# flash4242/Promptable-Counterfactual-GAN

Hardware: AMD Instinct MI355X
Metric: images/sec (G+D step) MNIST-28 cDCGAN bs512 @1/2/4/8 MI355X; % MFMA roofline (higher is better)
Workload: dtype f32

## Files before the change

include/pcgan_hip.h:

```cpp
#ifndef PCGAN_HIP_H
#define PCGAN_HIP_H

#include <stddef.h>
#include <stdint.h>

#ifdef __cplusplus
extern "C" {
#endif

typedef void* pcg_stream_t;

typedef enum pcg_status {
  PCG_OK = 0,
  PCG_ERR_INVALID = -1,
  PCG_ERR_WORKSPACE = -2,
  PCG_ERR_LAUNCH = -3,
  PCG_ERR_UNSUPPORTED = -4
} pcg_status;

typedef enum pcg_act {
  PCG_ACT_NONE = 0,
  PCG_ACT_RELU = 1,
  PCG_ACT_LRELU = 2,
  PCG_ACT_TANH = 3,
// ... 408 lines not shown
  int32_t B;
  const float* const* w_stored;
  const float* a1; const float* a2; const float* a3; const float* a4;
  float* dx;
} pcg_house_cls_bwd_args;
int pcg_house_classifier_fwd(const pcg_house_cls_fwd_args* args, const pcg_sn_bwd_batch* rider , pcg_stream_t stream);
int pcg_house_classifier_bwd(const pcg_house_cls_bwd_args* args, const pcg_sn_fwd_batch* rider , pcg_stream_t stream);

typedef struct pcg_house_cf_eval_args {
  int64_t N; int32_t T, group, clamp_cls, mask_rows;
  const float* g_flat; int32_t nG;
  const float* bn_mean[10]; const float* bn_var[10];
  float bn_eps, tau, res_scale;
  int32_t col_src[17];
  const float* norm_vals;
  const float* const* c_w_kmajor; const float* const* c_bias;
  const float* x; const int64_t* y;
  const int64_t* target; const float* mask; const float* noise;
  float* cont; float* logits; int32_t* chosen;
  float* masked; float* x_cf; float* x_cf_raw;
  float* logits_cf; float* logits_x;
  int64_t* pred_cf; int64_t* pred_x;
  float* gain;
  float* tile_sums; float* class_sums; float* class_counts;
} pcg_house_cf_eval_args;
int pcg_house_cf_eval(const pcg_house_g_desc* desc, const pcg_house_cf_eval_args* args, pcg_stream_t stream);

enum { PCG_MASK_SHARED = 0,
       PCG_MASK_PER_ROW = 1,
       PCG_MASK_PER_QUERY = 2 };

typedef struct pcg_patch_mask_bits_args {
  const uint64_t* bits;
  float* mask;
  int32_t n, H, W, ps;
} pcg_patch_mask_bits_args;
int pcg_patch_mask_bits(const pcg_patch_mask_bits_args* args, pcg_stream_t stream);

typedef struct pcg_mnist_cf_entry_args {
  const float* x;
  const float* table;
  const float* mask;
  const int64_t* target;
  float* out;
  int32_t B, T, HW, K, mask_mode, q0, nq;
} pcg_mnist_cf_entry_args;
int pcg_mnist_cf_entry(const pcg_mnist_cf_entry_args* args, pcg_stream_t stream);

typedef struct pcg_mnist_cf_tail_args {
  const float* c;
  const float* x;
  const float* mask;
  float* x_cf;
  float* raw; float* masked;
  float* sums;
  float scale;
  int32_t B, T, HW, mask_mode, q0, nq;
} pcg_mnist_cf_tail_args;
int pcg_mnist_cf_tail(const pcg_mnist_cf_tail_args* args, pcg_stream_t stream);

#define PCG_MNIST_CF_GROUP_SUMS 8
typedef struct pcg_mnist_cf_score_args {
  const float* logits_cf;
  const float* logits_orig;
  const int64_t* target;
  const int64_t* y_true;
  const float* tail_sums;
  int64_t* pred; float* conf; float* p_target; float* p_true; float* p_orig_true; float* flip;
  float* group_sums;
  int32_t B, T, K, ld, group_rows, q0, nq;
} pcg_mnist_cf_score_args;
int pcg_mnist_cf_score(const pcg_mnist_cf_score_args* args, pcg_stream_t stream);

int pcg_house_losses(const float* d_real, const float* d_fake, const float* d_fake_g, int64_t n, const float* g_cls, const float* am,
                     const float* pen, float lambda_cls, float w_reg, float lambda_mask, float w_reg_log, float* out5, pcg_stream_t stream);

typedef struct pcg_house_res_fwd_args {
  const float* cont; int32_t ncont;
  const float* samples; const int32_t* seg_dev; int32_t T;
  const float* norm; const float* x; const float* mask;
  const int32_t* col_src;
  int32_t D, B;
  float* res; float* masked; float* x_cf; float* partial512; int32_t* ticket; float* pen_out; float* am_out;
} pcg_house_res_fwd_args;
typedef struct pcg_house_res_bwd_args {
  const float* res; const float* masked; const float* mask; const float* gx_a; const float* gx_b;
  float w_pen, w_am;
  int32_t ncont; const int32_t* cont_idx_dev; const int32_t* seg_dev; int32_t S, T;
  const int32_t* cat_idx_dev; const float* norm;
  int32_t D, B;
  float* dcont; float* dsamples;
} pcg_house_res_bwd_args;
typedef struct pcg_house_loss_args {
  const float* d_real; const float* d_fake; const float* d_fake_g; int32_t n;
  const float* g_cls;
  const float* am; const float* pen;
  float lambda_cls, w_reg, lambda_mask, w_reg_log;
  const float* ce_row_loss;
  int32_t n_ce;
  float* out6;
} pcg_house_loss_args;
typedef struct pcg_house_diag_args {
  const float* logits_cf; const float* logits_orig;
  const int64_t* src_rows;
  const int64_t* target_y; const float* masked;
  int32_t B, nc, D;
  float eps;
  float* out4;
  double* acc;
} pcg_house_diag_args;
int pcg_house_residual_fwd(const pcg_house_res_fwd_args* args, const pcg_sn_fwd_batch* rider , pcg_stream_t stream);
int pcg_house_residual_bwd(const pcg_house_res_bwd_args* args, const pcg_house_loss_args* losses ,
                           const pcg_house_diag_args* diag , pcg_stream_t stream);
int pcg_house_diag(const pcg_house_diag_args* args, pcg_stream_t stream);
int pcg_house_draws(int64_t* target_y, int32_t B, int32_t num_classes, const int64_t* y, uint64_t offset_target, float* mask, int32_t D,
                    const int32_t* zero_cols, int32_t n_zero_cols, uint64_t offset_mask, float* noise, int32_t T, uint64_t offset_noise,
                    uint64_t seed, float* onehot_target, float* onehot_y, pcg_stream_t stream);
int pcg_house_draws_counter(int64_t* target_y, int32_t B, int32_t num_classes, const int64_t* y, float* mask, int32_t D,
                            const int32_t* zero_cols, int32_t n_zero_cols, float* noise, int32_t T, uint64_t seed, float* onehot_target,
                            float* onehot_y, uint64_t* counter, pcg_stream_t stream);
int pcg_house_batch_draws_counter(int64_t* target_y, int32_t B, int32_t num_classes, const float* X, const int64_t* Y,
                                  const int64_t* perm, int64_t n_perm, int64_t n_rows, float* x_out, int64_t* y_out,
                                  int64_t* src_out , float* mask, int32_t D, const int32_t* zero_cols, int32_t n_zero_cols,
                                  float* noise, int32_t T, uint64_t seed, float* onehot_target , float* onehot_y ,
                                  uint64_t* counter, pcg_stream_t stream);

int pcg_dp_barrier(pcg_stream_t stream);
int32_t pcg_dp_rccl_version(void);

#define PCG_DP_UNIQUE_ID_BYTES 128
int pcg_dp_unique_id(void* id_out );
int pcg_dp_init(const void* id , int32_t rank, int32_t world);
int32_t pcg_dp_world(void);
int32_t pcg_dp_rank(void);
pcg_stream_t pcg_dp_side_stream(void);
int pcg_dp_allreduce(float* buf, int64_t n, pcg_stream_t stream);
int pcg_dp_allreduce_begin(float* buf, int64_t n, int32_t slot, pcg_stream_t producer_stream);
int pcg_dp_record(int32_t slot);
int pcg_dp_allreduce_wait(int32_t slot, pcg_stream_t consumer_stream);
int pcg_dp_allreduce_sum_f64(double* buf, int64_t n, pcg_stream_t stream);
int pcg_dp_broadcast(void* buf, int64_t nbytes, int32_t root, pcg_stream_t stream);
int pcg_dp_sync_batchnorm(int32_t enable);
int pcg_dp_shutdown(void);

int pcg_tune_set(const char* name, int32_t value);

int pcg_conv_plan_describe(const pcg_conv_geom* g, int32_t op, int32_t assume_scratch, char* out, size_t out_bytes);
size_t pcg_conv_scratch_parts_bytes(void);
size_t pcg_conv_scratch_arrivals_bytes(void);
int pcg_conv_set_scratch(pcg_stream_t stream, void* parts, size_t parts_bytes, void* arrivals, size_t arrivals_bytes);
int pcg_conv_reset_scratch(pcg_stream_t stream);
size_t pcg_conv_pixtab_bytes(const pcg_conv_geom* g);
int pcg_conv_pixtab_register(const pcg_conv_geom* g, void* host_out, size_t bytes, const void* device_table);
int pcg_debug_stamp_buffer(void* buf, int64_t bytes);

typedef struct pcg_moons_cf_desc {
  int32_t hidden, clf_hidden, B, N;
  int32_t nG, nD, nC, nG_adam, nD_adam;
  int32_t g_off[14], d_off[8], c_off[6];
  double lr_G, lr_D, beta1, beta2, adam_eps;
  float bn_eps, bn_momentum, sn_eps, slope;
  float lambda_cls, lambda_l1, lambda_l2, lambda_mask;
} pcg_moons_cf_desc;

typedef struct pcg_moons_cf_train_args {
  const float* X; const int64_t* Y;
  const int64_t* rows;
  const int64_t* target_y;
  const float* mask;
  float* g_flat; float* d_flat; const float* c_flat;
  float* g_exp_avg; float* g_exp_avg_sq; int64_t* g_step;
  float* d_exp_avg; float* d_exp_avg_sq; int64_t* d_step;
  float* bn_mean[3]; float* bn_var[3]; int64_t* bn_nbt[3];
  float* sn_u[4]; float* sn_v[4];
  float* logs;
  float* scratch; size_t scratch_bytes;
} pcg_moons_cf_train_args;

size_t pcg_moons_cf_scratch_bytes(const pcg_moons_cf_desc* desc, int32_t forward);
int pcg_moons_cf_train_steps(const pcg_moons_cf_desc* desc, const pcg_moons_cf_train_args* args, int32_t n_steps, pcg_stream_t stream);

typedef struct pcg_moons_cf_fwd_args {
  int32_t which, train, B;
  const float* x; const float* onehot; const float* mask;
  float* params;
  float* bn_mean[3]; float* bn_var[3]; int64_t* bn_nbt[3];
  float* sn_u[4]; float* sn_v[4];
  float* out0; float* out1;
  float* scratch; size_t scratch_bytes;
} pcg_moons_cf_fwd_args;
int pcg_moons_cf_forward(const pcg_moons_cf_desc* desc, const pcg_moons_cf_fwd_args* args, pcg_stream_t stream);

typedef struct pcg_moons_cf_eval_args {
  int64_t N; int32_t M, T, group;
  const float* x; const int64_t* y;
  const float* masks;
  const int64_t* target; const float* row_mask;
  const float* g_flat; const float* c_flat;
  const float* bn_mean[3]; const float* bn_var[3];
  float* raw; float* masked; float* x_cf;
  float* logits_cf; float* logits_x;
  int64_t* pred_cf; int64_t* pred_x;
  float* gain;
  float* sums;
} pcg_moons_cf_eval_args;
int pcg_moons_cf_eval(const pcg_moons_cf_desc* desc, const pcg_moons_cf_eval_args* args, pcg_stream_t stream);

typedef struct {
  const float* gamma;
  const float* beta;
  float* running_mean;
  float* running_var;
  int64_t* num_batches_tracked;
  float* save_mean;
  float* save_invstd;
  float* xhat;
  float eps;
  float momentum;
  int32_t training;
} pcg_dense_bn;
typedef struct {
  const float* xhat;
  const float* gamma;
  const float* invstd;
  float* dgamma;
  float* dbeta;
  int32_t accumulate;
} pcg_dense_bn_bwd;
int pcg_dense_rows_fwd(const float* x, const float* W, const float* bias , int32_t R, int32_t I, int32_t O,
                       const pcg_dense_bn* bn , int act, float slope, float* y, pcg_stream_t stream);
int pcg_dense_rows_dgrad(const float* dz, const float* W, int32_t R, int32_t O, int32_t I, int below_act, float below_slope,
                         const float* y_below , const pcg_dense_bn_bwd* bn , float* dx,
                         pcg_stream_t stream);
int pcg_dense_rows_wgrad(const float* dz, const float* x, int32_t R, int32_t O, int32_t I, float* dW, float* db ,
                         int accumulate, pcg_stream_t stream);

typedef struct pcg_moons_gan_desc {
  int32_t hidden, z_dim, label_dim, B, N;
  int32_t nG, nD, nG_adam, nD_adam;
  int32_t g_off[4], d_off[4];
  double lr_G, lr_D, beta1, beta2, adam_eps;
} pcg_moons_gan_desc;

typedef struct pcg_moons_gan_train_args {
  const float* X; const int64_t* Y;
  const int64_t* rows;
  const float* z;
  const int64_t* labels;
  float* g_flat; float* d_flat;
  float* g_exp_avg; float* g_exp_avg_sq; int64_t* g_step;
  float* d_exp_avg; float* d_exp_avg_sq; int64_t* d_step;
  float* logs;
  float* scratch; size_t scratch_bytes;
} pcg_moons_gan_train_args;

size_t pcg_moons_gan_scratch_bytes(const pcg_moons_gan_desc* desc);
int pcg_moons_gan_train_steps(const pcg_moons_gan_desc* desc, const pcg_moons_gan_train_args* args, int32_t n_steps, pcg_stream_t stream);

typedef struct pcg_moons_gan_fwd_args {
  int32_t which; int64_t R;
  const float* x; const float* onehot; const float* params;
  float* out;
} pcg_moons_gan_fwd_args;
int pcg_moons_gan_forward(const pcg_moons_gan_desc* desc, const pcg_moons_gan_fwd_args* args, pcg_stream_t stream);

int32_t pcg_calib_mfma_blocks(int32_t rounds);
size_t pcg_calib_mfma_workspace_bytes(int32_t rounds);
int pcg_calib_mfma(int32_t iters, int32_t rounds, void* workspace, size_t workspace_bytes, double* flop_out ,
                   uint64_t** stamps_out , pcg_stream_t stream);
int pcg_calib_copy(const void* src, void* dst, int64_t nbytes, pcg_stream_t stream);

#ifdef __cplusplus
}
#endif
#endif
```

promptable-counterfactual-gan_amd/_lib.py:

```python
import ctypes
import os

import torch

_HERE = os.path.dirname(os.path.abspath(__file__))
LIB_PATH = os.environ.get("PCG_LIB") or os.path.join(_HERE, "libpcgan_hip.so")

PCG_OK = 0
ACT_NONE, ACT_RELU, ACT_LRELU, ACT_TANH, ACT_SIGMOID = 0, 1, 2, 3, 4


class PcgError(RuntimeError):
    pass


class ConvGeom(ctypes.Structure):

    _fields_ = [(n, ctypes.c_int32) for n in ("B", "IH", "IW", "Cin", "OH", "OW", "Cout", "KH", "KW", "stride", "pad")]

    def key(self):
        return tuple(getattr(self, n) for n, _ in self._fields_)


_I, _P = ctypes.c_int32, ctypes.c_void_p
# ... 45 lines not shown


class MoonsCfFwdArgs(ctypes.Structure):
    _fields_ = ([(n, _I) for n in ("which", "train", "B")] + [(n, _P) for n in ("x", "onehot", "mask", "params")] +
                [("bn_mean", _P * 3), ("bn_var", _P * 3), ("bn_nbt", _P * 3), ("sn_u", _P * 4), ("sn_v", _P * 4)] +
                [("out0", _P), ("out1", _P), ("scratch", _P), ("scratch_bytes", ctypes.c_size_t)])


class MoonsCfEvalArgs(ctypes.Structure):
    _fields_ = ([("N", ctypes.c_int64), ("M", _I), ("T", _I), ("group", _I)] +
                [(n, _P) for n in ("x", "y", "masks", "target", "row_mask", "g_flat", "c_flat")] + [("bn_mean", _P * 3), ("bn_var", _P * 3)] +
                [(n, _P) for n in ("raw", "masked", "x_cf", "logits_cf", "logits_x", "pred_cf", "pred_x", "gain", "sums")])


class HouseCfEvalArgs(ctypes.Structure):
    _fields_ = ([("N", ctypes.c_int64)] + [(n, _I) for n in ("T", "group", "clamp_cls", "mask_rows")] + [("g_flat", _P), ("nG", _I)] +
                [("bn_mean", _P * 10), ("bn_var", _P * 10)] + [(n, ctypes.c_float) for n in ("bn_eps", "tau", "res_scale")] +
                [("col_src", _I * 17), ("norm_vals", _P), ("c_w_kmajor", ctypes.POINTER(ctypes.c_void_p)), ("c_bias", ctypes.POINTER(ctypes.c_void_p))] +
                [(n, _P) for n in ("x", "y", "target", "mask", "noise", "cont", "logits", "chosen", "masked", "x_cf", "x_cf_raw", "logits_cf",
                                   "logits_x", "pred_cf", "pred_x", "gain", "tile_sums", "class_sums", "class_counts")])


class PatchMaskBitsArgs(ctypes.Structure):
    _fields_ = [("bits", _P), ("mask", _P)] + [(n, _I) for n in ("n", "H", "W", "ps")]


class MnistCfEntryArgs(ctypes.Structure):
    _fields_ = [(n, _P) for n in ("x", "table", "mask", "target", "out")] + [(n, _I) for n in ("B", "T", "HW", "K", "mask_mode", "q0", "nq")]


class MnistCfTailArgs(ctypes.Structure):
    _fields_ = ([(n, _P) for n in ("c", "x", "mask", "x_cf", "raw", "masked", "sums")] + [("scale", ctypes.c_float)] +
                [(n, _I) for n in ("B", "T", "HW", "mask_mode", "q0", "nq")])


class MnistCfScoreArgs(ctypes.Structure):
    _fields_ = ([(n, _P) for n in ("logits_cf", "logits_orig", "target", "y_true", "tail_sums", "pred", "conf", "p_target", "p_true",
                                   "p_orig_true", "flip", "group_sums")] + [(n, _I) for n in ("B", "T", "K", "ld", "group_rows", "q0", "nq")])


MASK_SHARED, MASK_PER_ROW, MASK_PER_QUERY = 0, 1, 2
MNIST_CF_GROUP_SUMS = 8


class MoonsGanDesc(ctypes.Structure):
    _fields_ = ([(n, _I) for n in ("hidden", "z_dim", "label_dim", "B", "N", "nG", "nD", "nG_adam", "nD_adam")] +
                [("g_off", _I * 4), ("d_off", _I * 4)] + [(n, ctypes.c_double) for n in ("lr_G", "lr_D", "beta1", "beta2", "adam_eps")])


class MoonsGanTrainArgs(ctypes.Structure):
    _fields_ = ([(n, _P) for n in ("X", "Y", "rows", "z", "labels", "g_flat", "d_flat", "g_exp_avg", "g_exp_avg_sq", "g_step",
                                   "d_exp_avg", "d_exp_avg_sq", "d_step", "logs", "scratch")] + [("scratch_bytes", ctypes.c_size_t)])


class MoonsGanFwdArgs(ctypes.Structure):
    _fields_ = [("which", _I), ("R", ctypes.c_int64)] + [(n, _P) for n in ("x", "onehot", "params", "out")]


class DenseBn(ctypes.Structure):
    _fields_ = ([(n, _P) for n in ("gamma", "beta", "running_mean", "running_var", "num_batches_tracked", "save_mean", "save_invstd", "xhat")] +
                [("eps", ctypes.c_float), ("momentum", ctypes.c_float), ("training", _I)])


class DenseBnBwd(ctypes.Structure):
    _fields_ = [(n, _P) for n in ("xhat", "gamma", "invstd", "dgamma", "dbeta")] + [("accumulate", _I)]


_PP, _PI, _F = ctypes.POINTER(ctypes.c_void_p), ctypes.POINTER(ctypes.c_int32), ctypes.c_float


class SnFwdBatch(ctypes.Structure):
    _fields_ = ([("n", _I), ("reps", _I), ("power_iteration", _I), ("eps", _F), ("w_orig", _PP), ("out_features", _PI), ("in_features", _PI)] +
                [(n, _PP) for n in ("u", "v", "w_bar", "sigma", "u_used", "v_used")])


class SnBwdBatch(ctypes.Structure):
    _fields_ = [("n", _I), ("passes", _I), ("dw_bar", _PP), ("w_bar", _PP), ("out_features", _PI), ("in_features", _PI), ("u", _PP), ("v", _PP),
                ("sigma", _PP), ("dw_orig", _PP), ("accumulate", _PI), ("db_dst", _PP), ("db_src", _PP)]


class HouseCriticFwdArgs(ctypes.Structure):
    _fields_ = ([(n, _I) for n in ("n_pass", "B", "D", "NC")] + [("slope", _F)] +
                [(n, _PP) for n in ("x", "onehot", "w_bar", "bias", "a0", "a1", "a2", "a3", "out")])


class HouseCriticBwdArgs(ctypes.Structure):
    _fields_ = ([(n, _I) for n in ("n_pass", "B", "D")] + [("slope", _F)] +
                [(n, _PP) for n in ("dout", "w_bar", "a1", "a2", "a3", "d3", "d2", "d1", "dx")])


class HouseClsFwdArgs(ctypes.Structure):
    _fields_ = ([("x", _P), ("B", _I), ("w_kmajor", _PP), ("bias", _PP)] + [(n, _P) for n in ("a1", "a2", "a3", "a4", "logits", "ce_target")] +
                [("ce_grad_scale", _F), ("ce_dlogits", _P), ("ce_row_loss", _P)])


class HouseClsBwdArgs(ctypes.Structure):
    _fields_ = [("dlogits", _P), ("B", _I), ("w_stored", _PP)] + [(n, _P) for n in ("a1", "a2", "a3", "a4", "dx")]


class HouseResFwdArgs(ctypes.Structure):
    _fields_ = ([("cont", _P), ("ncont", _I), ("samples", _P), ("seg_dev", _P), ("T", _I), ("norm", _P), ("x", _P), ("mask", _P), ("col_src", _PI),
                 ("D", _I), ("B", _I)] + [(n, _P) for n in ("res", "masked", "x_cf", "partial512", "ticket", "pen_out", "am_out")])


class HouseResBwdArgs(ctypes.Structure):
    _fields_ = ([(n, _P) for n in ("res", "masked", "mask", "gx_a", "gx_b")] + [("w_pen", _F), ("w_am", _F), ("ncont", _I), ("cont_idx_dev", _P),
                ("seg_dev", _P), ("S", _I), ("T", _I), ("cat_idx_dev", _P), ("norm", _P), ("D", _I), ("B", _I), ("dcont", _P), ("dsamples", _P)])


class HouseLossArgs(ctypes.Structure):
    _fields_ = ([("d_real", _P), ("d_fake", _P), ("d_fake_g", _P), ("n", _I), ("g_cls", _P), ("am", _P), ("pen", _P)] +
                [(n, _F) for n in ("lambda_cls", "w_reg", "lambda_mask", "w_reg_log")] + [("ce_row_loss", _P), ("n_ce", _I), ("out6", _P)])


class HouseDiagArgs(ctypes.Structure):
    _fields_ = ([(n, _P) for n in ("logits_cf", "logits_orig", "src_rows", "target_y", "masked")] + [("B", _I), ("nc", _I), ("D", _I), ("eps", _F),
                ("out4", _P), ("acc", _P)])


STRUCTS = {"pcg_conv_geom": ConvGeom, "pcg_in_xform": InXform, "pcg_wgrad_item": WgradItem, "pcg_sn_fwd_batch": SnFwdBatch,
           "pcg_sn_bwd_batch": SnBwdBatch, "pcg_house_g_desc": HouseGDesc, "pcg_house_g_fwd_args": HouseGFwdArgs,
           "pcg_house_g_bwd_args": HouseGBwdArgs, "pcg_house_critic_fwd_args": HouseCriticFwdArgs,
           "pcg_house_critic_bwd_args": HouseCriticBwdArgs, "pcg_house_cls_fwd_args": HouseClsFwdArgs, "pcg_house_cls_bwd_args": HouseClsBwdArgs,
           "pcg_house_res_fwd_args": HouseResFwdArgs, "pcg_house_res_bwd_args": HouseResBwdArgs, "pcg_house_loss_args": HouseLossArgs,
           "pcg_house_diag_args": HouseDiagArgs, "pcg_moons_cf_desc": MoonsCfDesc, "pcg_moons_cf_train_args": MoonsCfTrainArgs,
           "pcg_moons_cf_fwd_args": MoonsCfFwdArgs, "pcg_moons_cf_eval_args": MoonsCfEvalArgs,
           "pcg_house_cf_eval_args": HouseCfEvalArgs, "pcg_patch_mask_bits_args": PatchMaskBitsArgs,
           "pcg_mnist_cf_entry_args": MnistCfEntryArgs, "pcg_mnist_cf_tail_args": MnistCfTailArgs,
           "pcg_mnist_cf_score_args": MnistCfScoreArgs, "pcg_dense_bn": DenseBn,
           "pcg_dense_bn_bwd": DenseBnBwd, "pcg_moons_gan_desc": MoonsGanDesc, "pcg_moons_gan_train_args": MoonsGanTrainArgs,
           "pcg_moons_gan_fwd_args": MoonsGanFwdArgs}

_c = ctypes
_vp, _f, _i, _i64, _sz = _c.c_void_p, _c.c_float, _c.c_int, _c.c_int64, _c.c_size_t
_d = _c.c_double
_i32 = _c.c_int32
_gp = _c.POINTER(ConvGeom)
_xp = _c.POINTER(InXform)

PROTOTYPES = {
    "pcg_abi_version": (_i, []),
    "pcg_abi_struct_bytes": (_sz, [_c.c_char_p]),
    "pcg_last_error": (_c.c_char_p, []),
    "pcg_target_arch": (_c.c_char_p, []),
    "pcg_tune_set": (_i, [_c.c_char_p, _i32]),
    "pcg_debug_stamp_buffer": (_i, [_vp, _i64]),
    "pcg_conv_plan_describe": (_i, [_c.POINTER(ConvGeom), _i32, _i32, _c.c_char_p, _sz]),
    "pcg_conv_scratch_parts_bytes": (_sz, []),
    "pcg_conv_scratch_arrivals_bytes": (_sz, []),
    "pcg_conv_set_scratch": (_i, [_vp, _vp, _sz, _vp, _sz]),
    "pcg_conv_reset_scratch": (_i, [_vp]),
    "pcg_conv_pixtab_bytes": (_sz, [_gp]),
    "pcg_conv_pixtab_register": (_i, [_gp, _vp, _sz, _vp]),
    "pcg_conv2d_fwd_bn_g": (_i, [_gp, _vp, _vp, _vp, _vp, _f, _f, _vp, _vp, _vp, _vp, _vp, _i32, _vp, _sz, _vp]),
    "pcg_bn_apply_act_g": (_i, [_vp, _i64, _i32, _vp, _vp, _vp, _vp, _i, _f, _vp, _i32, _vp]),
    "pcg_conv2d_dgrad_bn_phases": (_i32, [_gp]),
    "pcg_conv2d_dgrad_bnbwd_g": (_i, [_gp, _vp, _vp, _vp, _vp, _vp, _vp, _vp, _i, _f, _vp, _vp, _sz, _i32, _vp]),
    "pcg_bn_bwd_partial_g_workspace_bytes": (_sz, [_i32, _i32]),
    "pcg_bn_bwd_partial_g": (_i, [_vp, _vp, _i64, _i32, _vp, _vp, _vp, _vp, _i32, _i32, _vp, _vp, _vp, _i, _i32, _vp, _sz, _vp]),
    "pcg_bn_act_bwd_g_workspace_bytes": (_sz, [_i64, _i32, _i32]),
    "pcg_bn_act_bwd_premask_g": (_i, [_vp, _vp, _i64, _i32, _vp, _vp, _vp, _vp, _i, _f, _vp, _vp, _vp, _i, _i32, _vp, _sz, _vp]),
    "pcg_bce_pair": (_i, [_vp, _i64, _f, _f, _vp, _vp, _vp, _vp, _vp, _vp]),
    "pcg_conv2d_fwd_bnbwd_thin_ok": (_i32, [_gp]),
    "pcg_conv2d_fwd_bnbwd_thin_workspace_bytes": (_sz, [_gp]),
    "pcg_conv2d_fwd_bnbwd_thin": (_i, [_gp, _vp, _vp, _vp, _vp, _vp, _vp, _vp, _i, _f, _vp, _vp, _vp, _i, _vp, _sz, _vp]),
    "pcg_conv2d_bnin_full_ok": (_i32, [_gp, _i32]),
    "pcg_conv2d_fwd_bnin_full": (_i, [_gp, _vp, _vp, _vp, _vp, _vp, _i, _f, _i32, _vp, _vp, _i, _f, _vp, _vp]),
    "pcg_conv2d_wgrad_bnin_full": (_i, [_gp, _vp, _vp, _vp, _vp, _vp, _i, _f, _i32, _vp, _vp, _i, _vp, _sz, _vp]),
    "pcg_conv_precision_set": (_i, [_i32]),
    "pcg_conv_precision_get": (_i32, []),
    "pcg_slab_defer_begin": (_i, [_vp]),
    "pcg_slab_defer_flush": (_i, [_vp]),
    "pcg_slab_defer_pending": (_i32, []),
    "pcg_conv2d_dgrad_bnbwd_full_ok": (_i32, [_gp, _i32]),
    "pcg_conv2d_dgrad_bnbwd_full_workspace_bytes": (_sz, [_gp, _i32]),
    "pcg_conv2d_dgrad_bnbwd_full": (_i, [_gp, _vp, _vp, _vp, _vp, _vp, _vp, _vp, _i, _f, _vp, _vp, _vp, _i, _i32, _vp, _sz, _vp]),
    "pcg_calib_mfma_blocks": (_i32, [_i32]),
    "pcg_calib_mfma_workspace_bytes": (_sz, [_i32]),
    "pcg_calib_mfma": (_i, [_i32, _i32, _vp, _sz, _c.POINTER(_d), _c.POINTER(_c.c_uint64), _vp]),
    "pcg_calib_copy": (_i, [_vp, _vp, _i64, _vp]),
    "pcg_conv2d_fwd_workspace_bytes": (_sz, [_gp]),
    "pcg_conv2d_dgrad_workspace_bytes": (_sz, [_gp]),
    "pcg_conv2d_fwd": (_i, [_gp, _vp, _vp, _vp, _vp, _vp, _sz, _vp]),
    "pcg_conv2d_dgrad": (_i, [_gp, _vp, _vp, _vp, _vp, _vp, _sz, _vp]),
    "pcg_conv2d_fwd_act": (_i, [_gp, _vp, _vp, _vp, _i, _f, _vp, _vp, _sz, _vp]),
    "pcg_conv2d_dgrad_act": (_i, [_gp, _vp, _vp, _vp, _i, _f, _vp, _vp, _sz, _vp]),
    "pcg_conv2d_fwd_bn_workspace_bytes": (_sz, [_gp]),
    "pcg_conv2d_dgrad_bn_workspace_bytes": (_sz, [_gp]),
    "pcg_conv2d_fwd_bn": (_i, [_gp, _vp, _vp, _vp, _vp, _f, _f, _vp, _vp, _vp, _vp, _vp, _vp, _sz, _vp]),
    "pcg_conv2d_dgrad_bn": (_i, [_gp, _vp, _vp, _vp, _vp, _f, _f, _vp, _vp, _vp, _vp, _vp, _vp, _sz, _vp]),
    "pcg_conv2d_dgrad_mask": (_i, [_gp, _vp, _vp, _vp, _i, _f, _vp, _vp, _sz, _vp]),
    "pcg_conv2d_dgrad_mask_thin_ok": (_i32, [_gp]),
    "pcg_conv2d_xf_thin_ok": (_i32, [_gp]),
    "pcg_conv2d_fwd_add_mask": (_i, [_gp, _vp, _vp, _vp, _vp, _i, _f, _vp, _vp]),
    "pcg_conv2d_dgrad_add_mask": (_i, [_gp, _vp, _vp, _vp, _vp, _i, _f, _vp, _vp]),
    "pcg_conv2d_fwd_mask": (_i, [_gp, _vp, _vp, _vp, _i, _f, _vp, _vp, _sz, _vp]),
    "pcg_conv2d_dgrad_bnbwd": (_i, [_gp, _vp, _vp, _vp, _vp, _vp, _vp, _vp, _i, _f, _vp, _vp, _sz, _vp]),
    "pcg_conv2d_fwd_bnbwd": (_i, [_gp, _vp, _vp, _vp, _vp, _vp, _vp, _vp, _i, _f, _vp, _vp, _sz, _vp]),
    "pcg_conv2d_dgrad_add": (_i, [_gp, _vp, _vp, _vp, _vp, _vp, _sz, _vp]),
    "pcg_conv2d_fwd_bn_partial_rows": (_c.c_int32, [_gp]),
    "pcg_conv2d_dgrad_bn_partial_rows": (_c.c_int32, [_gp]),
    "pcg_bn_bwd_partial_workspace_bytes": (_sz, [_c.c_int32]),
    "pcg_bn_bwd_partial": (_i, [_vp, _vp, _i64, _c.c_int32, _vp, _vp, _vp, _vp, _c.c_int32, _vp, _vp, _vp, _i, _vp, _sz, _vp]),
    "pcg_conv2d_fwd_bn_xf": (_i, [_gp, _vp, _xp, _vp, _vp, _vp, _f, _f, _vp, _vp, _vp, _vp, _vp, _vp, _vp, _vp, _vp, _sz, _vp]),
    "pcg_conv2d_dgrad_bn_xf": (_i, [_gp, _vp, _xp, _vp, _vp, _vp, _f, _f, _vp, _vp, _vp, _vp, _vp, _vp, _vp, _vp, _vp, _sz, _vp]),
    "pcg_conv2d_fwd_xf": (_i, [_gp, _vp, _xp, _vp, _vp, _i, _f, _vp, _vp, _sz, _vp]),
    "pcg_conv2d_dgrad_xf": (_i, [_gp, _vp, _xp, _vp, _vp, _i, _f, _vp, _vp, _sz, _vp]),
    "pcg_conv2d_wgrad_xf": (_i, [_gp, _vp, _xp, _vp, _xp, _vp, _i, _vp, _sz, _vp]),
    "pcg_bn_train_stats_coef": (_i, [_vp, _i64, _c.c_int32, _f, _f, _vp, _vp, _vp, _vp, _vp, _vp, _vp, _vp, _vp, _sz, _vp]),
    "pcg_bn_db_workspace_bytes": (_sz, [_i64, _c.c_int32]),
    "pcg_bn_act_bwd_db": (_i, [_vp, _vp, _vp, _i64, _c.c_int32, _vp, _vp, _vp, _vp, _i, _f, _f, _vp, _vp, _vp, _i, _vp, _i, _vp, _sz, _vp]),
    "pcg_bn_bwd_partial_db_workspace_bytes": (_sz, [_c.c_int32]),
    "pcg_bn_bwd_partial_db": (_i, [_vp, _vp, _i64, _c.c_int32, _vp, _vp, _vp, _vp, _c.c_int32, _f, _vp, _vp, _vp, _i, _vp, _i, _vp, _sz, _vp]),
    "pcg_conv2d_dgrad_add_bnsum": (_i, [_gp, _vp, _vp, _vp, _vp, _vp, _vp, _f, _vp, _vp, _sz, _vp]),
    "pcg_conv2d_fwd_add": (_i, [_gp, _vp, _vp, _vp, _vp, _vp, _sz, _vp]),
    "pcg_conv2d_fwd_add_bnsum": (_i, [_gp, _vp, _vp, _vp, _vp, _vp, _vp, _f, _vp, _vp, _sz, _vp]),
    "pcg_conv_weight_adjoint": (_i, [_vp, _vp, _i32, _i32, _i32, _i32, _vp]),
    "pcg_conv_weight_adjoint_many": (_i, [_vp, _vp, _i32, _i32, _i32, _i32, _i32, _vp]),
    "pcg_house_losses": (_i, [_vp, _vp, _vp, _i64, _vp, _vp, _vp, _f, _f, _f, _f, _vp, _vp]),
    "pcg_dp_unique_id": (_i, [_vp]),
    "pcg_dp_init": (_i, [_vp, _i32, _i32]),
    "pcg_dp_world": (_i32, []),
    "pcg_dp_rank": (_i32, []),
    "pcg_dp_side_stream": (_vp, []),
    "pcg_dp_allreduce": (_i, [_vp, _i64, _vp]),
    "pcg_dp_allreduce_begin": (_i, [_vp, _i64, _i32, _vp]),
    "pcg_dp_record": (_i, [_i32]),
    "pcg_dp_allreduce_wait": (_i, [_i32, _vp]),
    "pcg_dp_allreduce_sum_f64": (_i, [_vp, _i64, _vp]),
    "pcg_dp_broadcast": (_i, [_vp, _i64, _i32, _vp]),
    "pcg_dp_sync_batchnorm": (_i, [_i32]),
    "pcg_dp_barrier": (_i, [_vp]),
    "pcg_dp_rccl_version": (_i32, []),
    "pcg_dp_shutdown": (_i, []),
    "pcg_conv2d_wgrad_workspace_bytes": (_sz, [_gp]),
    "pcg_conv2d_wgrad": (_i, [_gp, _vp, _vp, _vp, _i, _vp, _sz, _vp]),
    "pcg_colsum_workspace_bytes": (_sz, [_i64, _c.c_int32]),
    "pcg_colsum": (_i, [_vp, _i64, _c.c_int32, _vp, _i, _vp, _sz, _vp]),
    "pcg_bn_workspace_bytes": (_sz, [_i64, _c.c_int32]),
    "pcg_bn_train_stats": (_i, [_vp, _i64, _c.c_int32, _f, _f, _vp, _vp, _vp, _vp, _vp, _vp, _sz, _vp]),
    "pcg_bn_apply_act": (_i, [_vp, _i64, _c.c_int32, _vp, _vp, _f, _vp, _vp, _i, _f, _vp, _f, _vp, _vp]),
    "pcg_bn_act_bwd": (_i, [_vp, _vp, _vp, _i64, _c.c_int32, _vp, _vp, _vp, _i, _f, _f, _vp, _vp, _vp, _i, _vp, _sz, _vp]),
    "pcg_bn_act_bwd_premask": (_i, [_vp, _vp, _i64, _c.c_int32, _vp, _vp, _vp, _vp, _i, _f, _f, _vp, _vp, _vp, _i, _vp, _sz, _vp]),
    "pcg_embed_concat_fwd": (_i, [_vp, _vp, _vp, _vp, _vp, _c.c_int32, _c.c_int32, _c.c_int32, _c.c_int32, _vp]),
    "pcg_embed_concat_bwd": (_i, [_vp, _vp, _vp, _vp, _c.c_int32, _c.c_int32, _c.c_int32, _c.c_int32, _i, _vp]),
    "pcg_embed_table_grad": (_i, [_vp, _vp, _vp, _i32, _i32, _i32, _i32, _i32, _i, _vp]),
    "pcg_gather_channel": (_i, [_vp, _vp, _i32, _i32, _i32, _vp]),
    "pcg_axpby": (_i, [_vp, _f, _vp, _f, _vp, _i64, _vp]),
    "pcg_scale_mask_fwd": (_i, [_vp, _vp, _f, _vp, _vp, _i64, _vp]),
    "pcg_scale_mask_bwd": (_i, [_vp, _vp, _vp, _f, _vp, _i64, _vp]),
    "pcg_clamp_add_fwd": (_i, [_vp, _vp, _f, _f, _vp, _i64, _vp]),
    "pcg_clamp_add_bwd": (_i, [_vp, _vp, _vp, _f, _f, _vp, _i64, _vp]),
    "pcg_abs_mean_workspace_bytes": (_sz, []),
    "pcg_abs_mean_fwd": (_i, [_vp, _vp, _i, _i64, _vp, _vp, _sz, _vp]),
    "pcg_abs_mean_bwd": (_i, [_vp, _vp, _i, _i64, _vp, _f, _vp, _i, _vp]),
    "pcg_avgpool_fwd": (_i, [_vp, _vp, _c.c_int32, _c.c_int32, _c.c_int32, _vp]),
    "pcg_avgpool_bwd": (_i, [_vp, _vp, _c.c_int32, _c.c_int32, _c.c_int32, _vp]),
    "pcg_cross_entropy_fwd_bwd": (_i, [_vp, _vp, _c.c_int32, _c.c_int32, _f, _vp, _vp, _vp, _vp]),
    "pcg_act_fwd": (_i, [_vp, _i64, _i, _f, _vp, _vp]),
    "pcg_act_bwd": (_i, [_vp, _vp, _i64, _i, _f, _vp, _vp]),
    "pcg_bce_fwd_bwd": (_i, [_vp, _vp, _f, _i64, _f, _vp, _vp, _vp, _vp]),
    "pcg_bce_logits_fwd_bwd": (_i, [_vp, _f, _i64, _f, _vp, _vp, _vp, _vp]),
    "pcg_adam_step": (_i, [_vp, _vp, _vp, _vp, _i64, _d, _d, _d, _d, _d, _i, _i64, _vp]),
    "pcg_adam_step_capturable": (_i, [_vp, _vp, _vp, _vp, _i64, _d, _d, _d, _d, _d, _i, _vp, _vp, _vp]),
    "pcg_patch_mask": (_i, [_vp, _c.c_int32, _c.c_int32, _c.c_int32, _c.c_int32, _c.c_int32, _c.c_uint64, _c.c_uint64, _vp]),
    "pcg_randint": (_i, [_vp, _i64, _c.c_int32, _c.c_int32, _vp, _c.c_uint64, _c.c_uint64, _vp]),
    "pcg_randn": (_i, [_vp, _i64, _f, _f, _c.c_uint64, _c.c_uint64, _vp]),
    "pcg_fill": (_i, [_vp, _i64, _f, _vp]),
    "pcg_add_bias_rows": (_i, [_vp, _i64, _i32, _vp, _vp]),
    "pcg_sumsq": (_i, [_vp, _i64, _vp, _i, _vp]),
    "pcg_norm_sum": (_i, [_vp, _vp, _i32, _vp, _vp]),
    "pcg_instnorm_fwd": (_i, [_vp, _i32, _i32, _i32, _vp, _vp, _f, _i, _f, _vp, _vp, _vp, _vp]),
    "pcg_instnorm_bwd": (_i, [_vp, _vp, _i32, _i32, _i32, _vp, _vp, _vp, _vp, _vp, _vp, _vp]),
    "pcg_instnorm_bwd_bwd": (_i, [_vp, _vp, _vp, _i32, _i32, _i32, _vp, _vp, _vp, _vp, _vp, _vp, _vp]),
    "pcg_instnorm_bwd_fused": (_i, [_vp, _vp, _f, _vp, _i32, _i32, _i32, _vp, _vp, _vp, _vp, _vp, _vp, _vp, _vp, _vp, _vp]),
    "pcg_instnorm_bwd_bwd_act": (_i, [_vp, _vp, _vp, _i32, _i32, _i32, _vp, _vp, _vp, _vp, _f, _vp, _vp, _vp, _vp]),
    "pcg_rowsum3": (_i, [_i32, _vp, _vp, _i, _vp, _vp, _i, _vp, _vp, _i, _i32, _i32, _vp]),
    "pcg_nhwc_to_nchw_flat": (_i, [_vp, _vp, _i32, _i32, _i32, _i, _vp]),
    "pcg_interpolate": (_i, [_vp, _vp, _vp, _vp, _i32, _i32, _vp]),
    "pcg_interpolate_stack": (_i, [_vp, _vp, _vp, _vp, _i32, _i32, _vp]),
    "pcg_gradient_penalty_fwd": (_i, [_vp, _i32, _i32, _f, _vp, _vp, _vp]),
    "pcg_gradient_penalty_bwd": (_i, [_vp, _vp, _vp, _i32, _i32, _f, _vp, _vp]),
    "pcg_rand_uniform": (_i, [_vp, _i64, _c.c_uint64, _c.c_uint64, _vp]),
    "pcg_cross_entropy_weighted_fwd_bwd": (_i, [_vp, _vp, _vp, _i32, _i32, _f, _vp, _vp, _vp, _vp]),
    "pcg_dropout_apply": (_i, [_vp, _vp, _i64, _i32, _i32, _f, _vp, _vp]),
    "pcg_rand_bernoulli": (_i, [_vp, _i64, _f, _c.c_uint64, _c.c_uint64, _vp]),
    "pcg_resize8_normalize": (_i, [_vp, _i32, _i32, _i32, _i32, _i32, _vp, _vp, _i32, _vp, _vp, _i32, _f, _f, _vp, _vp]),
    "pcg_house_g_fwd": (_i, [_c.POINTER(HouseGDesc), _c.POINTER(HouseGFwdArgs), _vp]),
    "pcg_house_g_bwd": (_i, [_c.POINTER(HouseGDesc), _c.POINTER(HouseGBwdArgs), _vp]),
    "pcg_weighted_sum_fwd": (_i, [_i32, _vp, _vp, _vp, _vp]),
    "pcg_weighted_sum_bwd": (_i, [_i32, _vp, _vp, _vp, _vp]),
    "pcg_cf_metrics": (_i, [_vp, _vp, _vp, _vp, _i32, _i32, _vp, _vp]),
    "pcg_gemm": (_i, [_i, _i, _i32, _i32, _i32, _vp, _i32, _vp, _i32, _vp, _i32, _vp, _i, _vp]),
    "pcg_linear_wgrad_workspace_bytes": (_sz, [_i32, _i32, _i32]),
    "pcg_linear_wgrad_ticket_count": (_i32, []),
    "pcg_linear_wgrad": (_i, [_vp, _i32, _vp, _i32, _i32, _i32, _i32, _vp, _vp, _i, _i, _vp, _sz, _vp, _vp]),
    "pcg_spectral_norm_fwd_batched": (_i, [_c.POINTER(SnFwdBatch), _vp]),
    "pcg_spectral_norm_bwd_batched": (_i, [_c.POINTER(SnBwdBatch), _vp]),
    "pcg_house_critic_fwd": (_i, [_c.POINTER(HouseCriticFwdArgs), _vp]),
    "pcg_house_critic_bwd": (_i, [_c.POINTER(HouseCriticBwdArgs), _vp]),
    "pcg_house_classifier_fwd": (_i, [_c.POINTER(HouseClsFwdArgs), _c.POINTER(SnBwdBatch), _vp]),
    "pcg_house_classifier_bwd": (_i, [_c.POINTER(HouseClsBwdArgs), _c.POINTER(SnFwdBatch), _vp]),
    "pcg_house_cf_eval": (_i, [_c.POINTER(HouseGDesc), _c.POINTER(HouseCfEvalArgs), _vp]),
    "pcg_patch_mask_bits": (_i, [_c.POINTER(PatchMaskBitsArgs), _vp]),
    "pcg_mnist_cf_entry": (_i, [_c.POINTER(MnistCfEntryArgs), _vp]),
    "pcg_mnist_cf_tail": (_i, [_c.POINTER(MnistCfTailArgs), _vp]),
# ... 75 lines not shown
```

promptable-counterfactual-gan_amd/csrc/conv_igemm.hip:

```cpp
#include <string.h>
#include <mutex>
#include "conv_loaders.h"
#include "conv_pixtab.h"
#include "thin_conv.h"

namespace pcg {
namespace {

__device__ __forceinline__ int wave_id() { return __builtin_amdgcn_readfirstlane((int)(threadIdx.x >> 6)); }

__device__ __forceinline__ void prio_entry(const ConvP& p) { if (p.edge_prio & 1) __builtin_amdgcn_s_setprio(3); }
__device__ __forceinline__ void prio_epilogue(const ConvP& p) { if (p.edge_prio & 2) __builtin_amdgcn_s_setprio(3); }

__device__ __forceinline__ int epi_group_off(const ConvP& p, int m_block) {
  return p.epi.group_rows > 0 ? __builtin_amdgcn_readfirstlane(m_block / p.epi.group_rows) * p.N : 0;
}

template <class Cfg, bool XF>
__global__ void __launch_bounds__(IG_THREADS, Cfg::MINW) conv_fwd_kernel(ConvP p) {
  extern __shared__ __attribute__((aligned(16))) float smem[];
  prio_entry(p);
  const uint32_t tile = xcd_remap(blockIdx.x, gridDim.x);
  const int mt = tile / p.tilesN, nt = tile % p.tilesN;
  const int m_block = mt * Cfg::BM, n_block = nt * Cfg::BN;
  const int kt_begin = blockIdx.y * p.ktiles_per_split;
  int ktiles = p.ktiles - kt_begin;
  if (ktiles > p.ktiles_per_split) ktiles = p.ktiles_per_split;

  if (wave_id() >= 4) {
    const int tid = threadIdx.x - IG_LOADERS;
    FwdALoader<Cfg::BM, XF> la(p, m_block, tid);
    FwdBLoader<Cfg::BN> lb(p, n_block, tid);
    if (kt_begin) { la.seek(kt_begin); lb.seek(kt_begin); }
    igemm_produce<Cfg>(la, lb, ktiles, smem, tid, ClockStamp{p.stamps, p.stamp_slots});
    return;
  }
  f32x16 acc[Cfg::TM][Cfg::TN];
  ClockStamp cs{p.stamps, p.stamp_slots};
  cs.phase(0);
  igemm_consume<Cfg, true, true>(ktiles, acc, smem, cs);
  prio_epilogue(p);
  float* out = p.out + (size_t)blockIdx.y * (size_t)p.M * (size_t)p.N;
#ifdef PCG_ABL_NO_EPILOGUE
  if (acc[0][0][0] == 12345.678f) out[0] = acc[0][0][1];
  return;
#endif
  igemm_store_tile<Cfg>(acc, smem, n_block, p.N, blockIdx.y == 0 ? p.bias : nullptr, [&](int row) -> float* {
    const int m = m_block + row;
    return m < p.M ? out + (size_t)m * p.N + n_block : nullptr;
  }, p.stat_partial ? p.stat_partial + (size_t)mt * Cfg::WAVES_M * 2 * p.N : nullptr, p.act, p.slope, &p.epi, epi_group_off(p, m_block));
  cs.phase(3);
}

template <class Cfg, bool XF>
__global__ void __launch_bounds__(IG_THREADS, Cfg::MINW) conv_dgrad_kernel(ConvP p, DgradPhases phases) {
  extern __shared__ __attribute__((aligned(16))) float smem[];
  __shared__ int rowpix[Cfg::BM];
  prio_entry(p);
  uint32_t bx = blockIdx.x, py = blockIdx.y;
  if (phases.interleave) {
    const uint32_t l = xcd_remap(blockIdx.x, gridDim.x);
    py = l % (uint32_t)phases.interleave; bx = l / (uint32_t)phases.interleave;
  }
  const PhaseInfo& f = phases.p[py];
  const int tilesM = (f.Mp + Cfg::BM - 1) / Cfg::BM;
  const uint32_t ntiles = (uint32_t)tilesM * p.tilesN;
  if (bx >= ntiles) return;
  const uint32_t tile = phases.interleave ? bx : xcd_remap(bx, ntiles);
  const int mt = tile / p.tilesN, nt = tile % p.tilesN;
  const int m_block = mt * Cfg::BM, n_block = nt * Cfg::BN;
  const int ktiles = f.nth * f.ntw * ((p.Cout + IG_BK - 1) / IG_BK);

  if (wave_id() >= 4) {
    const int tid = threadIdx.x - IG_LOADERS;
    for (int r = tid; r < Cfg::BM; r += IG_LOADERS) {
      const int m = m_block + r;
      int pix = -1;
      if (m < f.Mp) {
        uint32_t t, cc, b, aa;
        f.dPHw.divmod((uint32_t)m, t, cc);
        f.dPHh.divmod(t, b, aa);
        pix = ((int)b * p.IH + (int)aa * p.stride + f.ph) * p.IW + (int)cc * p.stride + f.pw;
      }
      rowpix[r] = pix;
    }
    DgradALoader<Cfg::BM, XF> la(p, f, m_block, tid);
    DgradBLoader<Cfg::BN> lb(p, f, n_block, tid);
    igemm_produce<Cfg>(la, lb, ktiles, smem, tid, ClockStamp{p.stamps, p.stamp_slots});
    return;
  }
  f32x16 acc[Cfg::TM][Cfg::TN];
  ClockStamp cs{p.stamps, p.stamp_slots};
  cs.phase(0);
  igemm_consume<Cfg, true, false>(ktiles, acc, smem, cs);
  prio_epilogue(p);
  igemm_store_tile<Cfg>(acc, smem, n_block, p.N, p.bias, [&](int row) -> float* {
    const int pix = rowpix[row];
    return pix >= 0 ? p.out + (size_t)pix * p.Cin + n_block : nullptr;
  }, p.stat_partial ? p.stat_partial + (size_t)(f.prow0 + mt * Cfg::WAVES_M) * 2 * p.N : nullptr, p.act, p.slope, &p.epi, epi_group_off(p, m_block));
  cs.phase(3);
}

struct SkPlan {
  int dp_tiles, sk_tiles, sk_blocks, ktiles;
  float* parts;
  int* arrivals;
};
struct SkSeg { int tile, kt_begin, nkt, nparts, first_block; };

__device__ __forceinline__ int sk_start(int g, const SkPlan& sk) {
  return __builtin_amdgcn_readfirstlane((int)((uint32_t)g * (uint32_t)(sk.sk_tiles * sk.ktiles) / (uint32_t)sk.sk_blocks));
}
__device__ __forceinline__ int sk_owner(int x, const SkPlan& sk) {
  return __builtin_amdgcn_readfirstlane((int)((((uint32_t)x + 1u) * (uint32_t)sk.sk_blocks - 1u) / (uint32_t)(sk.sk_tiles * sk.ktiles)));
}
__device__ __forceinline__ int sk_segments(const SkPlan& sk, SkSeg& s0, SkSeg& s1) {
  const int b = blockIdx.x;
  if (b < sk.dp_tiles) { s0 = SkSeg{(int)xcd_remap((uint32_t)b, (uint32_t)sk.dp_tiles), 0, sk.ktiles, 1, 0}; return 1; }
  const int g = (int)xcd_remap((uint32_t)(b - sk.dp_tiles), (uint32_t)sk.sk_blocks), KT = sk.ktiles;
  const int it0 = sk_start(g, sk), it1 = sk_start(g + 1, sk);
  const int j0 = __builtin_amdgcn_readfirstlane(it0 / KT), e0 = it1 < (j0 + 1) * KT ? it1 : (j0 + 1) * KT;
  auto fill = [&](SkSeg& sg, int j, int from, int to) {
    const int f = sk_owner(j * KT, sk), l = sk_owner((j + 1) * KT - 1, sk);
    sg = SkSeg{sk.dp_tiles + j, from - j * KT, to - from, l - f + 1, f};
  };
  fill(s0, j0, it0, e0);
  if (it1 <= e0) return 1;
  fill(s1, j0 + 1, e0, it1);
  return 2;
}
#if defined(__HIP_DEVICE_COMPILE__) && !defined(__gfx950__)
#error "stream-K partial-tile exchange (sc1 stores + relaxed agent-scope counters) is written for gfx950 only"
#endif
__device__ __forceinline__ void sk_store4(rsrc_t r, uint32_t off, float a, float b, float c, float d) {
  const u32x4 v = {__float_as_uint(a), __float_as_uint(b), __float_as_uint(c), __float_as_uint(d)};
  __builtin_amdgcn_raw_buffer_store_b128(v, r, off, 0, 16);
}
__device__ __forceinline__ float4 sk_load4(rsrc_t r, uint32_t off) {
  const u32x4 v = __builtin_amdgcn_raw_buffer_load_b128(r, off, 0, 16);
  return make_float4(__uint_as_float(v.x), __uint_as_float(v.y), __uint_as_float(v.z), __uint_as_float(v.w));
}
template <class Cfg, class FirstOf>
__device__ __forceinline__ bool sk_combine_core(float* parts, int* arrivals, int nblocks, int g, int j, int nparts, int first_block,
                                                FirstOf first_of, f32x16 (&acc)[Cfg::TM][Cfg::TN]) {
  if (nparts == 1) return true;
  constexpr uint32_t TILE_BYTES = Cfg::BM * Cfg::BN * 4;
  auto slot_of = [&](int blk) { return (uint32_t)(2 * blk + (first_of(blk) ? 0 : 1)); };
  const rsrc_t rs = make_rsrc(parts, (uint32_t)(2 * nblocks) * TILE_BYTES);
  const uint32_t toff = threadIdx.x * 16u;
  const uint32_t mine = slot_of(g) * TILE_BYTES + toff;
#pragma unroll
  for (int i = 0; i < Cfg::TM; ++i)
#pragma unroll
    for (int jj = 0; jj < Cfg::TN; ++jj)
#pragma unroll
      for (int q = 0; q < 4; ++q)
        sk_store4(rs, mine + (uint32_t)(((i * Cfg::TN + jj) * 4 + q) * IG_LOADERS * 16),
                  acc[i][jj][4 * q], acc[i][jj][4 * q + 1], acc[i][jj][4 * q + 2], acc[i][jj][4 * q + 3]);
  asm volatile("s_waitcnt vmcnt(0)" ::: "memory");
  int* cnt = arrivals + j * 4 + (int)(threadIdx.x >> 6);
  int old = 0;
  if ((threadIdx.x & 63) == 0) old = __hip_atomic_fetch_add(cnt, 1, __ATOMIC_RELAXED, __HIP_MEMORY_SCOPE_AGENT);
  old = __builtin_amdgcn_readfirstlane(old);
  if (old != nparts - 1) return false;
  if ((threadIdx.x & 63) == 0) __hip_atomic_store(cnt, 0, __ATOMIC_RELAXED, __HIP_MEMORY_SCOPE_AGENT);
#pragma unroll
  for (int i = 0; i < Cfg::TM; ++i)
#pragma unroll
    for (int jj = 0; jj < Cfg::TN; ++jj)
#pragma unroll
      for (int r = 0; r < 16; ++r) acc[i][jj][r] = 0.f;
  for (int k = 0; k < nparts; ++k) {
    const uint32_t src = slot_of(first_block + k) * TILE_BYTES + toff;
#pragma unroll
    for (int i = 0; i < Cfg::TM; ++i)
#pragma unroll
      for (int jj = 0; jj < Cfg::TN; ++jj)
#pragma unroll
        for (int q = 0; q < 4; ++q) {
          const float4 v = sk_load4(rs, src + (uint32_t)(((i * Cfg::TN + jj) * 4 + q) * IG_LOADERS * 16));
          acc[i][jj][4 * q] += v.x; acc[i][jj][4 * q + 1] += v.y; acc[i][jj][4 * q + 2] += v.z; acc[i][jj][4 * q + 3] += v.w;
        }
  }
  return true;
}
template <class Cfg>
__device__ __forceinline__ bool sk_combine(const SkPlan& sk, const SkSeg& sg, f32x16 (&acc)[Cfg::TM][Cfg::TN]) {
  const int g = (int)xcd_remap((uint32_t)((int)blockIdx.x - sk.dp_tiles), (uint32_t)sk.sk_blocks), j = sg.tile - sk.dp_tiles, KT = sk.ktiles;
  return sk_combine_core<Cfg>(sk.parts, sk.arrivals, sk.sk_blocks, g, j, sg.nparts, sg.first_block,
                              [&](int blk) { return sk_start(blk, sk) >= j * KT; }, acc);
}

template <class Cfg, bool XF>
__device__ __forceinline__ void fwd_sk_segment(const ConvP& p, const SkPlan& sk, const SkSeg& sg, float* smem) {
  const int mt = __builtin_amdgcn_readfirstlane(sg.tile / p.tilesN), nt = sg.tile - mt * p.tilesN;
  const int m_block = mt * Cfg::BM, n_block = nt * Cfg::BN;
  if (wave_id() >= 4) {
    const int tid = threadIdx.x - IG_LOADERS;
    FwdALoader<Cfg::BM, XF> la(p, m_block, tid);
    FwdBLoader<Cfg::BN> lb(p, n_block, tid);
    if (sg.kt_begin) { la.seek(sg.kt_begin); lb.seek(sg.kt_begin); }
    igemm_produce<Cfg>(la, lb, sg.nkt, smem, tid, ClockStamp{nullptr, 0});
    return;
  }
  f32x16 acc[Cfg::TM][Cfg::TN];
  igemm_consume<Cfg, true, true>(sg.nkt, acc, smem);
  if (sk_combine<Cfg>(sk, sg, acc))
    igemm_store_tile<Cfg>(acc, smem, n_block, p.N, p.bias, [&](int row) -> float* {
      const int m = m_block + row;
      return m < p.M ? p.out + (size_t)m * p.N + n_block : nullptr;
    }, p.stat_partial ? p.stat_partial + (size_t)mt * Cfg::WAVES_M * 2 * p.N : nullptr, p.act, p.slope, &p.epi, epi_group_off(p, m_block));
// ... 121 lines not shown
}
template <class Cfg, bool XF>
__global__ void __launch_bounds__(IG_THREADS, Cfg::MINW) conv_dgrad_skn_kernel(ConvP p, DgradPhases phases, SkNPlan sk) {
  extern __shared__ __attribute__((aligned(16))) float smem[];
  __shared__ int rowpix[Cfg::BM];
  const int g = (int)xcd_remap(blockIdx.x, (uint32_t)sk.blocks);
  const int it1 = skn_start(g + 1, sk);
  if (wave_id() >= 4) {
    const int tid = threadIdx.x - IG_LOADERS;
#pragma unroll 1
    for (int it = skn_start(g, sk); it < it1;) {
      const SkNSeg sg = skn_segment(it, it1, sk, p.tilesN);
      const PhaseInfo& f = phases.p[sg.py];
      const int m_block = sg.mt * Cfg::BM, n_block = sg.nt * Cfg::BN;
      for (int r = tid; r < Cfg::BM; r += IG_LOADERS) {
        const int m = m_block + r;
        int pix = -1;
        if (m < f.Mp) {
          uint32_t t, cc, b, aa;
          f.dPHw.divmod((uint32_t)m, t, cc);
          f.dPHh.divmod(t, b, aa);
          pix = ((int)b * p.IH + (int)aa * p.stride + f.ph) * p.IW + (int)cc * p.stride + f.pw;
        }
        rowpix[r] = pix;
      }
      DgradALoader<Cfg::BM, XF> la(p, f, m_block, tid);
      DgradBLoader<Cfg::BN> lb(p, f, n_block, tid);
      if (sg.kt_begin) { la.seek(sg.kt_begin); lb.seek(sg.kt_begin); }
      igemm_produce<Cfg>(la, lb, sg.nkt, smem, tid, ClockStamp{nullptr, 0});
      it = sg.e;
      if (it < it1) lds_barrier();
    }
    return;
  }
#pragma unroll 1
  for (int it = skn_start(g, sk); it < it1;) {
    const SkNSeg sg = skn_segment(it, it1, sk, p.tilesN);
    const PhaseInfo& f = phases.p[sg.py];
    const int m_block = sg.mt * Cfg::BM, n_block = sg.nt * Cfg::BN;
    {
      f32x16 acc[Cfg::TM][Cfg::TN];
      igemm_consume<Cfg, true, false>(sg.nkt, acc, smem);
      const int t_begin = sg.t_begin;
      if (sk_combine_core<Cfg>(sk.parts, sk.arrivals, sk.blocks, g, sk.tile0[sg.py] + sg.tin, sg.nparts, sg.fb,
                               [&](int blk) { return skn_start(blk, sk) >= t_begin; }, acc))
        igemm_store_tile<Cfg>(acc, smem, n_block, p.N, p.bias, [&](int row) -> float* {
          const int pix = rowpix[row];
          return pix >= 0 ? p.out + (size_t)pix * p.Cin + n_block : nullptr;
        }, p.stat_partial ? p.stat_partial + (size_t)(f.prow0 + sg.mt * Cfg::WAVES_M) * 2 * p.N : nullptr, p.act, p.slope, &p.epi, epi_group_off(p, m_block));
    }
    it = sg.e;
    if (it < it1) lds_barrier();
  }
}

template <class Cfg, bool XFA, bool XFB, bool TAB>
__device__ __forceinline__ void wgrad_sk_segment(const ConvP& p, const SkPlan& sk, const SkSeg& sg, float* smem) {
  const int mt = __builtin_amdgcn_readfirstlane(sg.tile / p.tilesN), nt = sg.tile - mt * p.tilesN;
  const int m_block = mt * Cfg::BM, n_block = nt * Cfg::BN;
  if (wave_id() >= 4) {
    const int tid = threadIdx.x - IG_LOADERS;
    WgradALoader<Cfg::BM, XFA> la(p, m_block, sg.kt_begin, tid);
    WgradBLoader<Cfg::BN, XFB, TAB> lb(p, n_block, sg.kt_begin, tid);
    igemm_produce<Cfg>(la, lb, sg.nkt, smem, tid, ClockStamp{nullptr, 0});
    return;
  }
  f32x16 acc[Cfg::TM][Cfg::TN];
  igemm_consume<Cfg, false, false>(sg.nkt, acc, smem);
  if (sk_combine<Cfg>(sk, sg, acc))
    igemm_store_tile<Cfg>(acc, smem, n_block, p.N, nullptr, [&](int row) -> float* {
      const int m = m_block + row;
      return m < p.M ? p.out + (size_t)m * p.N + n_block : nullptr;
    }, nullptr, PCG_ACT_NONE, 0.f, &p.epi);
}
template <class Cfg, bool XFA, bool XFB, bool TAB = false>
__global__ void __launch_bounds__(IG_THREADS, 4) conv_wgrad_sk_kernel(ConvP p, SkPlan sk) {
  extern __shared__ __attribute__((aligned(16))) float smem[];
  SkSeg s0, s1{};
  const int nseg = sk_segments(sk, s0, s1);
  wgrad_sk_segment<Cfg, XFA, XFB, TAB>(p, sk, s0, smem);
  if (nseg == 1) return;
  lds_barrier();
  wgrad_sk_segment<Cfg, XFA, XFB, TAB>(p, sk, s1, smem);
}

using Cfg64x192 = TileCfg<64, 192, 2, 2>;
template <class Cfg, bool TAB = false>
__global__ void __launch_bounds__(IG_THREADS, 4) conv_wgrad192_kernel(ConvP p, int ktiles_total, int ktiles_per_split, int tiles,
                                                                      int slice_major) {
  static_assert(Cfg::BM == 64 && Cfg::BN == 192, "the 192-column weight-gradient tile");
  extern __shared__ __attribute__((aligned(16))) float smem[];
  prio_entry(p);
  uint32_t tile, split;
  if (slice_major) {
    const uint32_t l = xcd_remap(blockIdx.x, gridDim.x);
    split = l / (uint32_t)tiles; tile = l - split * (uint32_t)tiles;
  } else {
    tile = xcd_remap(blockIdx.x, gridDim.x); split = blockIdx.y;
  }
  const int mt = tile / p.tilesN, nt = tile % p.tilesN;
  const int m_block = mt * Cfg::BM, n_block = nt * Cfg::BN;
  const int kt_begin = split * ktiles_per_split;
  int ktiles = ktiles_total - kt_begin;
  if (ktiles > ktiles_per_split) ktiles = ktiles_per_split;
  if (wave_id() >= 4) {
    const int tid = threadIdx.x - IG_LOADERS;
    WgradALoader<Cfg::BM, false> la(p, m_block, kt_begin, tid);
    WgradBLoader192<TAB> lb(p, n_block, kt_begin, tid);
    igemm_produce<Cfg>(la, lb, ktiles, smem, tid);
    return;
  }
  f32x16 acc[Cfg::TM][Cfg::TN];
  igemm_consume<Cfg, false, false>(ktiles, acc, smem, ClockStamp{p.stamps, p.stamp_slots});
  prio_epilogue(p);
  float* slab = p.out + (size_t)split * (size_t)p.M * (size_t)p.N;
  igemm_store_tile<Cfg>(acc, smem, n_block, p.N, nullptr, [&](int row) -> float* {
    const int m = m_block + row;
    return m < p.M ? slab + (size_t)m * p.N + n_block : nullptr;
  });
}

__global__ void __launch_bounds__(256) col2im_kernel(const float4* __restrict__ dcol, float4* __restrict__ dx, const float* __restrict__ bias,
                                                     int B, int IH, int IW, int CQ, int OH, int OW, int KH, int KW, int stride, int pad,
                                                     FastDiv dCQ, FastDiv dIW, FastDiv dIH, int act, float neg) {
  const uint32_t total = (uint32_t)B * IH * IW * CQ;
  for (uint32_t idx = blockIdx.x * 256u + threadIdx.x; idx < total; idx += gridDim.x * 256u) {
    uint32_t pix, cq, t, iw, b, ih;
    dCQ.divmod(idx, pix, cq);
    dIW.divmod(pix, t, iw);
    dIH.divmod(t, b, ih);
    float4 acc = bias ? *reinterpret_cast<const float4*>(bias + 4 * cq) : make_float4(0.f, 0.f, 0.f, 0.f);
    for (int kh = 0; kh < KH; ++kh) {
      const int th = (int)ih + pad - kh;
      if (th < 0 || th % stride) continue;
      const int oh = th / stride;
      if (oh >= OH) continue;
      for (int kw = 0; kw < KW; ++kw) {
        const int tw = (int)iw + pad - kw;
        if (tw < 0 || tw % stride) continue;
        const int ow = tw / stride;
        if (ow >= OW) continue;
        const float4 v = dcol[((size_t)(((int)b * OH + oh) * OW + ow) * (KH * KW) + (kh * KW + kw)) * CQ + cq];
        acc.x += v.x; acc.y += v.y; acc.z += v.z; acc.w += v.w;
      }
    }
    if (act != PCG_ACT_NONE) {
      acc.x = act_neg_scale(acc.x, neg); acc.y = act_neg_scale(acc.y, neg); acc.z = act_neg_scale(acc.z, neg); acc.w = act_neg_scale(acc.w, neg);
    }
    dx[idx] = acc;
  }
}

using Cfg128x128 = TileCfg<128, 128, 2, 2>;
#ifndef PCG_TILE64_SWZ
#define PCG_TILE64_SWZ 1
#endif
using Cfg128x64P = TileCfg<128, 64, 2, 2>;
#if PCG_TILE64_SWZ
using Cfg128x64 = TileCfg<128, 64, 2, 2, true, 6, 1>;
#else
using Cfg128x64 = Cfg128x64P;
#endif

template <class C>
using Bf16Twin = TileCfg<C::BM, C::BN, C::WAVES_M, C::WAVES_N, false, C::MINW, C::PF, true>;


int check_geom(const pcg_conv_geom* g) {
  PCG_REQUIRE(g != nullptr, "conv geometry is null");
  PCG_REQUIRE(g->B > 0 && g->IH > 0 && g->IW > 0 && g->Cin > 0 && g->OH > 0 && g->OW > 0 && g->Cout > 0,
              "conv geometry: non-positive extent");
  PCG_REQUIRE(g->KH > 0 && g->KW > 0 && g->stride > 0 && g->pad >= 0, "conv geometry: bad kernel/stride/pad");
  PCG_REQUIRE(g->OH == (g->IH + 2 * g->pad - g->KH) / g->stride + 1 && g->OW == (g->IW + 2 * g->pad - g->KW) / g->stride + 1,
              "conv geometry: OH/OW inconsistent with IH/IW, kernel %dx%d stride %d pad %d", g->KH, g->KW, g->stride, g->pad);
  PCG_REQUIRE((int64_t)g->B * g->IH * g->IW * g->Cin * 4 < (1ll << 31) && (int64_t)g->B * g->OH * g->OW * g->Cout * 4 < (1ll << 31) &&
                  (int64_t)g->Cout * g->KH * g->KW * g->Cin * 4 < (1ll << 31),
              "conv geometry: an operand tensor reaches 2 GiB (32-bit buffer offsets); split the batch");
  PCG_REQUIRE(g->KH * g->KW <= 32, "conv geometry: more than 32 taps (%dx%d) unsupported", g->KH, g->KW);
  return PCG_OK;
}

struct Tune { int edge_prio = -1, dgrad_swz3 = -1, wgrad_rounds = -1, korder = -1, wgrad_order = -1, dgrad_interleave = -1, fwd_splits = -1, stream_k = -1, sk_blocks = -1, dgrad_gemm = -1, t64 = -1, wgrad_pixtab = -1; unsigned long long* stamps = nullptr; int stamp_slots = 0; };
Tune g_tune;

ConvP make_params(const pcg_conv_geom* g) {
  ConvP p{};
  static const int korder_env = getenv("PCG_KORDER") ? atoi(getenv("PCG_KORDER")) : 1;
  p.korder = g_tune.korder >= 0 ? g_tune.korder : korder_env;
  static const int edge_env = getenv("PCG_EDGE_PRIO") ? atoi(getenv("PCG_EDGE_PRIO")) : 2;
  p.edge_prio = g_tune.edge_prio >= 0 ? g_tune.edge_prio : edge_env;
  p.stamps = g_tune.stamps; p.stamp_slots = g_tune.stamp_slots;
  p.B = g->B; p.IH = g->IH; p.IW = g->IW; p.Cin = g->Cin; p.OH = g->OH; p.OW = g->OW; p.Cout = g->Cout;
  p.KH = g->KH; p.KW = g->KW; p.stride = g->stride; p.pad = g->pad;
  p.dOW = FastDiv((uint32_t)g->OW);
  p.dOH = FastDiv((uint32_t)g->OH);
  p.dOHW = FastDiv((uint32_t)(g->OH * g->OW));
  p.x_bytes = (uint32_t)((int64_t)g->B * g->IH * g->IW * g->Cin * 4);
  p.dy_bytes = (uint32_t)((int64_t)g->B * g->OH * g->OW * g->Cout * 4);
  p.w_bytes = (uint32_t)((int64_t)g->Cout * g->KH * g->KW * g->Cin * 4);
  return p;
}

int set_xform(const char* who, const pcg_in_xform* xf, int C, ConvP* p) {
  if (!xf || !xf->scale) return PCG_OK;
  PCG_REQUIRE(xf->shift != nullptr, "%s: input transform without shift", who);
  PCG_REQUIRE(xf->act == PCG_ACT_NONE || xf->act == PCG_ACT_RELU || xf->act == PCG_ACT_LRELU,
              "%s: input transform activation %d is not none / ReLU / LeakyReLU", who, xf->act);
  PCG_REQUIRE(C % 4 == 0 && (((uintptr_t)xf->scale | (uintptr_t)xf->shift) & 15) == 0,
              "%s: input transform needs a channel count %% 4 == 0 and 16-byte aligned scale / shift", who);
  p->in_sc = xf->scale; p->in_sh = xf->shift; p->in_neg = act_neg_of(xf->act, xf->slope); p->in_c_bytes = (uint32_t)C * 4u;
  return PCG_OK;
}

template <class Cfg, bool AK, bool BK_>
constexpr size_t smem_bytes() {
  constexpr int a = igemm_smem_floats<Cfg, AK, BK_>(), b = epilogue_smem_floats<Cfg>();
  return sizeof(float) * (size_t)(a > b ? a : b);
}

template <class K>
int set_smem(K kernel, size_t bytes) {
  hipError_t e = hipFuncSetAttribute(reinterpret_cast<const void*>(kernel), hipFuncAttributeMaxDynamicSharedMemorySize, (int)bytes);
  if (e != hipSuccess) { set_error("hipFuncSetAttribute(max dynamic LDS=%zu): %s", bytes, hipGetErrorString(e)); return PCG_ERR_LAUNCH; }
  return PCG_OK;
}

constexpr int SK_MAX_BLOCKS = 512, SK_MAX_TILES = 4096;
constexpr size_t SK_PARTS_BYTES = (size_t)2 * SK_MAX_BLOCKS * 128 * 128 * sizeof(float);
constexpr size_t SK_ARRIVALS_BYTES = (size_t)SK_MAX_TILES * 4 * sizeof(int);
struct SkScratch { int device; hipStream_t stream; float* parts; int* arrivals; };
SkScratch g_sk_scratch[64];
int g_sk_scratch_n = 0;
std::mutex g_sk_mutex;
int current_device() { int d = 0; return hipGetDevice(&d) == hipSuccess ? d : 0; }
bool sk_scratch_of(hipStream_t s, SkPlan* sk) {
  const int dev = current_device();
  std::lock_guard<std::mutex> lock(g_sk_mutex);
  for (int i = 0; i < g_sk_scratch_n; ++i)
    if (g_sk_scratch[i].stream == s && g_sk_scratch[i].device == dev) {
      if (sk) { sk->parts = g_sk_scratch[i].parts; sk->arrivals = g_sk_scratch[i].arrivals; }
      return true;
    }
  return false;
}
struct PixTabReg { int device, IH, IW, OH, OW, stride, pad, KH, KW, Cin; const uint32_t* tab; };
constexpr int PIXTAB_MAX = 256;
PixTabReg g_pixtab[PIXTAB_MAX];
int g_pixtab_n = 0;
std::mutex g_pixtab_mutex;
bool pixtab_same(const PixTabReg& r, int dev, const pcg_conv_geom* g) {
  return r.device == dev && r.IH == g->IH && r.IW == g->IW && r.OH == g->OH && r.OW == g->OW && r.stride == g->stride && r.pad == g->pad &&
         r.KH == g->KH && r.KW == g->KW && r.Cin == g->Cin;
}
const uint32_t* pixtab_of(const pcg_conv_geom* g) {
  static const int env = getenv("PCG_WGRAD_PIXTAB") ? atoi(getenv("PCG_WGRAD_PIXTAB")) : 1;
  if (!(g_tune.wgrad_pixtab >= 0 ? g_tune.wgrad_pixtab : env)) return nullptr;
  std::lock_guard<std::mutex> lock(g_pixtab_mutex);
  if (g_pixtab_n == 0) return nullptr;
  const int dev = current_device();
  for (int i = 0; i < g_pixtab_n; ++i)
    if (pixtab_same(g_pixtab[i], dev, g)) return g_pixtab[i].tab;
  return nullptr;
}
int sk_mode() {
  static const int env = getenv("PCG_STREAM_K") ? atoi(getenv("PCG_STREAM_K")) : 1;
  return g_tune.stream_k >= 0 ? g_tune.stream_k : env;
}
bool plan_sk_shape(int tiles, int ktiles, SkPlan* sk) {
  const int mode = sk_mode();
  if (mode == 3) {
    sk->dp_tiles = tiles; sk->sk_tiles = 0; sk->sk_blocks = 0; sk->ktiles = ktiles;
    return true;
  }
  if (mode == 0 || ktiles < 8) return false;
  const int dp = tiles / 512 * 512, r = tiles - dp;
  if (r == 0 || r > SK_MAX_TILES || (int64_t)r * ktiles * 512 >= (1ll << 31)) return false;
  const double t_dp = (r <= 256 ? 2.2 : 3.5) * ktiles + 6.0;
  double best = 1e30;
  int bg = 0;
  for (int G = 512; G >= 64; G >>= 1) {
    if (g_tune.sk_blocks > 0 && G != g_tune.sk_blocks) continue;
    if (G < r) break;
    const int it = ceil_div(r * ktiles, G);
    if (it < 4) continue;
    const int parts = ceil_div(ktiles, it) + 1;
    if (parts > 8) continue;
    const double t = it * (G == 512 ? 3.5 : 2.2) + 2 * 12.0 + 3.0 + 1.5 * parts;
    if (t < best) { best = t; bg = G; }
  }
  if (!bg || (mode == 1 && best > 0.9 * t_dp)) return false;
  sk->dp_tiles = dp; sk->sk_tiles = r; sk->sk_blocks = bg; sk->ktiles = ktiles;
  return true;
}
bool plan_sk(int tiles, int ktiles, hipStream_t s, SkPlan* sk) { return plan_sk_shape(tiles, ktiles, sk) && sk_scratch_of(s, sk); }
bool have_sk_scratch() {
  if (sk_mode() == 0) return false;
  const int dev = current_device();
  std::lock_guard<std::mutex> lock(g_sk_mutex);
  for (int i = 0; i < g_sk_scratch_n; ++i) if (g_sk_scratch[i].device == dev) return true;
  return false;
}
int stream_has_sk(hipStream_t s) { return sk_mode() != 0 && sk_scratch_of(s, nullptr) ? 1 : 0; }

template <class Cfg, bool XF>
int launch_fwd_x(ConvP p, int splits, hipStream_t s) {
  p.tilesN = ceil_div(p.N, Cfg::BN);
  const int tilesM = ceil_div(p.M, Cfg::BM);
  constexpr size_t smem = smem_bytes<Cfg, true, true>();
  if constexpr (Cfg::BM == 128 && Cfg::BN == 128) {
    SkPlan sk{};
    if (splits == 1 && plan_sk(tilesM * p.tilesN, p.ktiles, s, &sk)) {
      static int once_sk = set_smem(conv_fwd_sk_kernel<Cfg, XF>, smem);
      if (once_sk != PCG_OK) return once_sk;
      hipLaunchKernelGGL((conv_fwd_sk_kernel<Cfg, XF>), dim3((unsigned)(sk.dp_tiles + sk.sk_blocks)), dim3(IG_THREADS), smem, s, p, sk);
      return launch_status("conv_fwd_sk_kernel");
    }
  }
  static int once = set_smem(conv_fwd_kernel<Cfg, XF>, smem);
  if (once != PCG_OK) return once;
  hipLaunchKernelGGL((conv_fwd_kernel<Cfg, XF>), dim3((unsigned)tilesM * p.tilesN, splits), dim3(IG_THREADS), smem, s, p);
  return launch_status("conv_fwd_kernel");
}
template <class Cfg>
int launch_fwd(const ConvP& p, int splits, hipStream_t s) {
  if (conv_bf16()) return p.in_sc ? launch_fwd_x<Bf16Twin<Cfg>, true>(p, splits, s) : launch_fwd_x<Bf16Twin<Cfg>, false>(p, splits, s);
  return p.in_sc ? launch_fwd_x<Cfg, true>(p, splits, s) : launch_fwd_x<Cfg, false>(p, splits, s);
}

struct FwdPlan { int splits, ktiles_per_split; };
FwdPlan plan_fwd(const pcg_conv_geom* g, int have_sk = -1) {
  if (have_sk < 0) have_sk = have_sk_scratch() ? 1 : 0;
  const int M = g->B * g->OH * g->OW, N = g->Cout;
  const int tiles = ceil_div(M, 128) * ceil_div(N, N > 64 ? 128 : 64);
  const int ktiles = g->KH * g->KW * ceil_div(g->Cin, IG_BK);
  FwdPlan f{1, ktiles};
  if (g_tune.fwd_splits > 0) {
    f.ktiles_per_split = ceil_div(ktiles, g_tune.fwd_splits);
    f.splits = ceil_div(ktiles, f.ktiles_per_split);
    return f;
  }
  if (tiles > 256 && tiles < 448 && ktiles >= 32 && !have_sk) {
    int best = 1;
    double bc = 2.0;
    for (int s = 2; s <= 4; ++s) {
      const double c = (double)ceil_div(tiles * s, 256) / s + 0.1 * s;
      if (c < bc - 1e-9) { bc = c; best = s; }
    }
    f.ktiles_per_split = ceil_div(ktiles, best);
    f.splits = ceil_div(ktiles, f.ktiles_per_split);
    return f;
  }
  if (tiles > 96 || ktiles < 32) return f;
  int splits = ceil_div(tiles >= 48 ? 512 : 384, tiles);
  if (splits > ktiles / 8) splits = ktiles / 8;
  if (splits < 2) return f;
  f.ktiles_per_split = ceil_div(ktiles, splits);
  f.splits = ceil_div(ktiles, f.ktiles_per_split);
  return f;
}

bool plan_skn_shape(const DgradPhases& ph, int nphases, int BM, int tilesN, int Cout, SkNPlan* sn) {
  if (sk_mode() == 0 || nphases < 2) return false;
  sn->nph = nphases;
  bool ok = true;
  int tiles = 0, total = 0, ktmax = 0;
  for (int i = 0; i < nphases && ok; ++i) {
    const int kt = ph.p[i].nth * ph.p[i].ntw * ceil_div(Cout, IG_BK), t = ceil_div(ph.p[i].Mp, BM) * tilesN;
    ok = ph.p[i].nth > 0 && ph.p[i].ntw > 0 && ph.p[i].Mp > 0 && kt > 0;
    sn->tile0[i] = tiles; sn->it0[i] = total; sn->kt[i] = kt;
    tiles += t; total += t * kt;
    if (kt > ktmax) ktmax = kt;
  }
  sn->tile0[nphases] = tiles; sn->it0[nphases] = total;
  int blocks = total / 512 >= 16 ? 512 : 256;
  if (g_tune.sk_blocks > 0) blocks = g_tune.sk_blocks;
  ok = ok && tiles <= SK_MAX_TILES && blocks <= SK_MAX_BLOCKS && total / blocks >= 8 && (int64_t)total * blocks < (1ll << 31) &&
       ktmax <= 8 * (total / blocks) && (sk_mode() == 2 || g_tune.sk_blocks > 0 || total >= 48 * tiles);
  sn->blocks = blocks; sn->total = total;
  return ok;
}

template <class Cfg, bool XF>
int launch_dgrad_x(ConvP p, const DgradPhases& ph, int nphases, int maxMp, hipStream_t s) {
  p.tilesN = ceil_div(p.N, Cfg::BN);
  const int tilesM = ceil_div(maxMp, Cfg::BM);
  constexpr size_t smem = smem_bytes<Cfg, true, false>();
  if constexpr (Cfg::BM == 128 && Cfg::BN == 128) {
    bool uniform = true;
    for (int i = 0; i < nphases; ++i)
      uniform = uniform && ph.p[i].Mp == ph.p[0].Mp && ph.p[i].nth * ph.p[i].ntw == ph.p[0].nth * ph.p[0].ntw && ph.p[i].nth > 0 && ph.p[i].ntw > 0;
    if (!uniform && nphases > 1 && sk_mode() != 0) {
      SkNPlan sn{};
      SkPlan scratch{};
      if (plan_skn_shape(ph, nphases, Cfg::BM, p.tilesN, p.Cout, &sn) && sk_scratch_of(s, &scratch)) {
        sn.parts = scratch.parts; sn.arrivals = scratch.arrivals;
        static int once_sn = set_smem(conv_dgrad_skn_kernel<Cfg, XF>, smem);
        if (once_sn != PCG_OK) return once_sn;
        DgradPhases phs = ph;
        phs.interleave = 0;
        hipLaunchKernelGGL((conv_dgrad_skn_kernel<Cfg, XF>), dim3((unsigned)sn.blocks), dim3(IG_THREADS), smem, s, p, phs, sn);
        return launch_status("conv_dgrad_skn_kernel");
      }
    }
    SkPlan sk{};
    const int tpp = tilesM * p.tilesN;
    if (uniform && plan_sk(tpp * nphases, ph.p[0].nth * ph.p[0].ntw * ceil_div(p.Cout, IG_BK), s, &sk)) {
      static int once_sk = set_smem(conv_dgrad_sk_kernel<Cfg, XF>, smem);
      if (once_sk != PCG_OK) return once_sk;
      DgradPhases phs = ph;
      phs.interleave = 0;
      hipLaunchKernelGGL((conv_dgrad_sk_kernel<Cfg, XF>), dim3((unsigned)(sk.dp_tiles + sk.sk_blocks)), dim3(IG_THREADS), smem, s, p, phs, sk, tpp);
      return launch_status("conv_dgrad_sk_kernel");
    }
  }
  static int once = set_smem(conv_dgrad_kernel<Cfg, XF>, smem);
  if (once != PCG_OK) return once;
  static const int il_env0 = getenv("PCG_DGRAD_INTERLEAVE") ? atoi(getenv("PCG_DGRAD_INTERLEAVE")) : 1;
  const int il_env = g_tune.dgrad_interleave >= 0 ? g_tune.dgrad_interleave : il_env0;
  DgradPhases phl = ph;
  bool same = nphases > 1 && il_env && p.w_bytes <= (1u << 20);
  for (int i = 1; i < nphases; ++i) same = same && ph.p[i].Mp == ph.p[0].Mp;
  phl.interleave = same ? nphases : 0;
  if (same)
    hipLaunchKernelGGL((conv_dgrad_kernel<Cfg, XF>), dim3((unsigned)tilesM * p.tilesN * nphases), dim3(IG_THREADS), smem, s, p, phl);
  else
    hipLaunchKernelGGL((conv_dgrad_kernel<Cfg, XF>), dim3((unsigned)tilesM * p.tilesN, nphases), dim3(IG_THREADS), smem, s, p, phl);
  return launch_status("conv_dgrad_kernel");
}
template <class Cfg>
int launch_dgrad(const ConvP& p, const DgradPhases& ph, int nphases, int maxMp, hipStream_t s) {
  if (conv_bf16())
    return p.in_sc ? launch_dgrad_x<Bf16Twin<Cfg>, true>(p, ph, nphases, maxMp, s) : launch_dgrad_x<Bf16Twin<Cfg>, false>(p, ph, nphases, maxMp, s);
  return p.in_sc ? launch_dgrad_x<Cfg, true>(p, ph, nphases, maxMp, s) : launch_dgrad_x<Cfg, false>(p, ph, nphases, maxMp, s);
}

struct WgradPlan { int splits, ktiles_total, ktiles_per_split, tiles; bool narrow, wide192; };

WgradPlan plan_wgrad(const pcg_conv_geom* g) {
  WgradPlan w{};
  const int M = g->Cout, N = g->KH * g->KW * g->Cin;
  w.narrow = (M <= 64);
  static const int t192_env = getenv("PCG_WGRAD_192") ? atoi(getenv("PCG_WGRAD_192")) : 1;
  w.wide192 = w.narrow && t192_env && N % 192 == 0 && (N % 128) != 0;
  const int BM = w.narrow ? 64 : 128;
  w.tiles = ceil_div(M, BM) * (w.wide192 ? N / 192 : ceil_div(N, 128));
  const int64_t K = (int64_t)g->B * g->OH * g->OW;
  w.ktiles_total = (int)ceil_div64(K, IG_BK);
  const int slots = 512 * (g_tune.wgrad_rounds > 0 ? g_tune.wgrad_rounds : 1);
  int splits = w.tiles <= slots ? slots / w.tiles : 1;
  const int max_splits = w.ktiles_total / 8 > 0 ? w.ktiles_total / 8 : 1;
  if (splits > max_splits) splits = max_splits;
  if (splits < 1) splits = 1;
  auto cost = [&](int s, int* s_eff) {
    const int kps = ceil_div(w.ktiles_total, s), se = ceil_div(w.ktiles_total, kps);
    const int n = ceil_div(w.tiles * se, 256);
    *s_eff = se;
    return (double)n * kps * (w.wide192 ? 1.5 : w.narrow ? 1.0 : 1.95) * (n == 1 ? 1.2 : 1.0) + (double)se * M * N * 8.0 / 4.0e6;
  };
  int se = 0;
  const double c0 = cost(splits, &se);
  double cb = c0;
  int sb = splits;
  for (int s = 1; s <= max_splits && s <= 64; ++s) {
    const double c = cost(s, &se);
    if (se == s && c < cb * 0.98) { cb = c; sb = s; }
  }
  if (cb < 0.95 * c0) splits = sb;
  w.ktiles_per_split = ceil_div(w.ktiles_total, splits);
  w.splits = ceil_div(w.ktiles_total, w.ktiles_per_split);
  return w;
}

}
}

using namespace pcg;

extern "C" size_t pcg_conv2d_fwd_workspace_bytes(const pcg_conv_geom* g) {
  if (check_geom(g) != PCG_OK) return 0;
  if (thin_is_cin(g) || thin_is_cout(g)) return thin_conv_fwd_workspace_bytes(g);
  const FwdPlan f = plan_fwd(g);
  return f.splits > 1 ? (size_t)f.splits * g->B * g->OH * g->OW * g->Cout * sizeof(float) : 0;
}
static bool dgrad_as_gemm(const pcg_conv_geom* g, int have_sk = -1) {
  if (have_sk < 0) have_sk = have_sk_scratch() ? 1 : 0;
  if (thin_is_cin(g) || thin_is_cout(g)) return false;
  if (g_tune.dgrad_gemm == 0) return false;
  if (g_tune.dgrad_gemm < 0 && have_sk && g->stride == 2) {
    int64_t phase_macs = 0;
    for (int a = 0; a < 2; ++a)
      for (int b = 0; b < 2; ++b) {
        const int PHh = a < g->IH ? (g->IH - a + 1) / 2 : 0, PHw = b < g->IW ? (g->IW - b + 1) / 2 : 0;
        const int kh0 = (a + g->pad) % 2, kw0 = (b + g->pad) % 2;
        const int nth = kh0 < g->KH ? (g->KH - kh0 + 1) / 2 : 0, ntw = kw0 < g->KW ? (g->KW - kw0 + 1) / 2 : 0;
        phase_macs += (int64_t)PHh * PHw * nth * ntw;
      }
    if (phase_macs * 20 <= (int64_t)g->OH * g->OW * g->KH * g->KW * 19) return false;
  }
  if (g->stride < 2 || (g->KH % g->stride == 0 && g->KW % g->stride == 0)) return false;
  if (g->Cout < 512 || g->Cin % 4 || g->Cout % 4) return false;
  const int64_t bytes = (int64_t)g->B * g->OH * g->OW * g->KH * g->KW * g->Cin * 4;
  return bytes < (1ll << 31);
}
static size_t dgrad_gemm_bytes(const pcg_conv_geom* g) { return (size_t)g->B * g->OH * g->OW * g->KH * g->KW * g->Cin * sizeof(float); }

extern "C" size_t pcg_conv_scratch_parts_bytes(void) { return pcg::SK_PARTS_BYTES; }
extern "C" size_t pcg_conv_scratch_arrivals_bytes(void) { return pcg::SK_ARRIVALS_BYTES; }
extern "C" int pcg_conv_set_scratch(pcg_stream_t stream, void* parts, size_t parts_bytes, void* arrivals, size_t arrivals_bytes) {
  using namespace pcg;
  hipStream_t s = (hipStream_t)stream;
  const int dev = current_device();
  std::lock_guard<std::mutex> lock(g_sk_mutex);
  int at = -1;
  for (int i = 0; i < g_sk_scratch_n; ++i) if (g_sk_scratch[i].stream == s && g_sk_scratch[i].device == dev) at = i;
  if (!parts) {
    if (at >= 0) g_sk_scratch[at] = g_sk_scratch[--g_sk_scratch_n];
    return PCG_OK;
  }
  PCG_REQUIRE(arrivals != nullptr && parts_bytes >= SK_PARTS_BYTES && arrivals_bytes >= SK_ARRIVALS_BYTES,
              "pcg_conv_set_scratch: parts %zu B (need %zu), arrivals %zu B (need %zu)", parts_bytes, SK_PARTS_BYTES, arrivals_bytes, SK_ARRIVALS_BYTES);
  PCG_REQUIRE((((uintptr_t)parts) & 15) == 0 && (((uintptr_t)arrivals) & 3) == 0, "pcg_conv_set_scratch: misaligned scratch");
  if (at < 0) {
    PCG_REQUIRE(g_sk_scratch_n < 64, "pcg_conv_set_scratch: more than 64 streams with scratch");
    at = g_sk_scratch_n++;
  }
  g_sk_scratch[at] = SkScratch{dev, s, (float*)parts, (int*)arrivals};
  return PCG_OK;
}
extern "C" int pcg_conv_reset_scratch(pcg_stream_t stream) {
  using namespace pcg;
  SkPlan sk{};
  if (!sk_scratch_of((hipStream_t)stream, &sk)) return PCG_OK;
  hipError_t e = hipMemsetAsync(sk.arrivals, 0, SK_ARRIVALS_BYTES, (hipStream_t)stream);
  if (e != hipSuccess) { set_error("pcg_conv_reset_scratch: %s", hipGetErrorString(e)); return PCG_ERR_LAUNCH; }
  return PCG_OK;
}

extern "C" size_t pcg_conv_pixtab_bytes(const pcg_conv_geom* g) {
  if (check_geom(g) != PCG_OK) return 0;
  return pcg::pixtab_entries(g->OH, g->OW) * 2 * sizeof(uint32_t);
}
extern "C" int pcg_conv_pixtab_register(const pcg_conv_geom* g, void* host_out, size_t bytes, const void* device_table) {
  using namespace pcg;
  if (int e = check_geom(g)) return e;
  if (host_out) {
    PCG_REQUIRE(bytes >= pcg_conv_pixtab_bytes(g) && (((uintptr_t)host_out) & 3) == 0, "pcg_conv_pixtab_register: host buffer %zu B (need %zu), 4-byte aligned",
                bytes, pcg_conv_pixtab_bytes(g));
    pixtab_build(g->IH, g->IW, g->OH, g->OW, g->stride, g->pad, g->KH, g->KW, g->Cin, static_cast<uint32_t*>(host_out));
    if (!device_table) return PCG_OK;
  }
  PCG_REQUIRE((((uintptr_t)device_table) & 7) == 0, "pcg_conv_pixtab_register: misaligned table");
  const int dev = current_device();
  std::lock_guard<std::mutex> lock(g_pixtab_mutex);
  int at = -1;
  for (int i = 0; i < g_pixtab_n; ++i) if (pixtab_same(g_pixtab[i], dev, g)) at = i;
  if (!device_table) {
    if (at >= 0) g_pixtab[at] = g_pixtab[--g_pixtab_n];
    return PCG_OK;
  }
  if (at < 0) {
    PCG_REQUIRE(g_pixtab_n < PIXTAB_MAX, "pcg_conv_pixtab_register: more than %d geometries with a table", PIXTAB_MAX);
    at = g_pixtab_n++;
  }
  g_pixtab[at] = PixTabReg{dev, g->IH, g->IW, g->OH, g->OW, g->stride, g->pad, g->KH, g->KW, g->Cin, static_cast<const uint32_t*>(device_table)};
  return PCG_OK;
}

extern "C" size_t pcg_conv2d_dgrad_workspace_bytes(const pcg_conv_geom* g) {
  if (check_geom(g) != PCG_OK) return 0;
  if (thin_is_cin(g) || thin_is_cout(g)) return thin_conv_dgrad_workspace_bytes(g);
  return dgrad_as_gemm(g) ? dgrad_gemm_bytes(g) : 0;
}

namespace pcg {
int launch_bn_stats_finalize(const double* partial, int nparts, int64_t rows, int C, float eps, float momentum, float* save_mean,
                             float* save_invstd, float* running_mean, float* running_var, int64_t* nbt, hipStream_t s,
                             bool has_presum_tail, const float* gamma = nullptr, const float* beta = nullptr, float* coef = nullptr);
size_t bn_partial_buffer_bytes(int nparts, int C);
int launch_bn_stats_finalize_g(const double* partial, int nparts, int nphases, int groups, int64_t rows_per_group, int C, float eps,
                               float momentum, float* save_mean, float* save_invstd, float* running_mean, float* running_var,
                               int64_t* nbt, hipStream_t s);
}

static bool mfma_layer(const pcg_conv_geom* g) { return !(thin_is_cin(g) || thin_is_cout(g)); }
static int fwd_stat_rows(const pcg_conv_geom* g) { return ceil_div(g->B * g->OH * g->OW, 128) * 2; }
static int dgrad_stat_rows(const pcg_conv_geom* g) {
  int rows = 0;
  const int s = g->stride;
  for (int a = 0; a < s; ++a)
    for (int b = 0; b < s; ++b) {
      const int PHh = a < g->IH ? (g->IH - a + s - 1) / s : 0, PHw = b < g->IW ? (g->IW - b + s - 1) / s : 0;
      rows += ceil_div(g->B * PHh * PHw, 128) * 2;
    }
  return rows;
}

static bool fwd_use_t64(int M, int N, int splits) {
  const int tiles128 = ceil_div(M, 128) * ceil_div(N, 128);
  return g_tune.t64 != 0 && N > 64 && splits == 1 && tiles128 > 224 && tiles128 <= 256 && M % 128 == 0;
}
static int conv2d_fwd_impl(const pcg_conv_geom* g, const float* x, const float* w, const float* bias, float* y,
                           double* stat_partial, void* workspace, size_t workspace_bytes, pcg_stream_t stream, int act = PCG_ACT_NONE,
                           float slope = 0.f, const EpiAux* epi = nullptr, const pcg_in_xform* xf = nullptr) {
  if (int e = check_geom(g)) return e;
  PCG_REQUIRE(x && w && y, "pcg_conv2d_fwd: null pointer");
  PCG_REQUIRE(act >= PCG_ACT_NONE && act <= PCG_ACT_SIGMOID, "pcg_conv2d_fwd: unknown activation %d", act);
  if (thin_is_cin(g) || thin_is_cout(g)) {
    PCG_REQUIRE(!(xf && xf->scale), "pcg_conv2d_fwd: input transforms are only implemented on the MFMA path (Cin > 3 and Cout > 3)");
    return thin_conv_fwd(g, x, w, bias, y, workspace, workspace_bytes, (hipStream_t)stream, act, slope);
  }
  PCG_REQUIRE(g->Cin % 4 == 0, "pcg_conv2d_fwd: Cin=%d must be a multiple of 4 for the MFMA path (1..3-channel layers take the thin path)", g->Cin);
  ConvP p = make_params(g);
  p.x = x; p.w = w; p.bias = bias; p.out = y; p.stat_partial = stat_partial;
  if (epi) p.epi = *epi;
  if (int e = set_xform("pcg_conv2d_fwd", xf, g->Cin, &p)) return e;
  p.M = g->B * g->OH * g->OW; p.N = g->Cout;
  p.ktiles = g->KH * g->KW * ceil_div(g->Cin, IG_BK);
  p.ktiles_per_split = p.ktiles;
  hipStream_t s = (hipStream_t)stream;
  FwdPlan f = plan_fwd(g, stream_has_sk(s));
  const size_t need = (size_t)f.splits * p.M * p.N * sizeof(float);
  if (f.splits > 1 && (stat_partial || epi || !workspace || workspace_bytes < need || ((uintptr_t)workspace & 15) || ((uintptr_t)y & 15) || (p.M * (size_t)p.N) % 4))
    f = FwdPlan{1, p.ktiles};
  const bool fuse = act_is_cheap(act) && f.splits == 1;
  p.act = fuse ? act : PCG_ACT_NONE; p.slope = act_neg_of(p.act, slope);
  if (f.splits > 1) { p.out = (float*)workspace; p.ktiles_per_split = f.ktiles_per_split; }
  const bool t64 = fwd_use_t64(p.M, p.N, f.splits);
  if (int e = t64 ? launch_fwd<TileCfg<64, 128, 1, 4>>(p, f.splits, s)
                  : p.N > 64 ? launch_fwd<Cfg128x128>(p, f.splits, s)
                       : launch_fwd<Cfg128x64>(p, f.splits, s)) return e;
  if (f.splits > 1) {
    const size_t n = (size_t)p.M * p.N;
    if (int e = launch_slab_reduce((const float*)workspace, y, n, n, f.splits, 0, s)) return e;
  }
  return (fuse || act == PCG_ACT_NONE) ? PCG_OK : pcg_act_fwd(y, (int64_t)p.M * p.N, act, slope, y, stream);
}

extern "C" int pcg_conv2d_fwd(const pcg_conv_geom* g, const float* x, const float* w, const float* bias, float* y,
                              void* workspace, size_t workspace_bytes, pcg_stream_t stream) {
  return conv2d_fwd_impl(g, x, w, bias, y, nullptr, workspace, workspace_bytes, stream);
}
extern "C" int pcg_conv2d_fwd_act(const pcg_conv_geom* g, const float* x, const float* w, const float* bias, int act, float slope,
                                  float* y, void* workspace, size_t workspace_bytes, pcg_stream_t stream) {
  return conv2d_fwd_impl(g, x, w, bias, y, nullptr, workspace, workspace_bytes, stream, act, slope);
}

extern "C" size_t pcg_conv2d_fwd_bn_workspace_bytes(const pcg_conv_geom* g) {
  if (check_geom(g) != PCG_OK || !mfma_layer(g) || g->Cout % 4) return 0;
  return bn_partial_buffer_bytes(fwd_stat_rows(g), g->Cout);
}
extern "C" size_t pcg_conv2d_dgrad_bn_workspace_bytes(const pcg_conv_geom* g) {
  if (check_geom(g) != PCG_OK || !mfma_layer(g) || g->stride > 2 || g->Cin % 4) return 0;
  return bn_partial_buffer_bytes(dgrad_stat_rows(g), g->Cin);
}

extern "C" int pcg_conv2d_fwd_bn_xf(const pcg_conv_geom* g, const float* x, const pcg_in_xform* xf, const float* w, const float* bias,
                                    float* y, float eps, float momentum, float* save_mean, float* save_invstd, float* running_mean,
                                    float* running_var, int64_t* num_batches_tracked, const float* gamma, const float* beta,
                                    float* coef_out, void* workspace, size_t workspace_bytes, pcg_stream_t stream) {
  const size_t need = pcg_conv2d_fwd_bn_workspace_bytes(g);
  PCG_REQUIRE(need > 0, "pcg_conv2d_fwd_bn: only MFMA layers (Cin > 3, Cout > 3, Cout %% 4 == 0); use pcg_conv2d_fwd + pcg_bn_train_stats");
  PCG_REQUIRE(save_mean && save_invstd, "pcg_conv2d_fwd_bn: null statistics output");
  PCG_REQUIRE(!coef_out || (gamma && beta), "pcg_conv2d_fwd_bn_xf: coef_out needs gamma and beta");
  if (!workspace || workspace_bytes < need) { set_error("pcg_conv2d_fwd_bn: workspace %zu B < required %zu B", workspace_bytes, need); return PCG_ERR_WORKSPACE; }
  if (int e = conv2d_fwd_impl(g, x, w, bias, y, (double*)workspace, nullptr, 0, stream, PCG_ACT_NONE, 0.f, nullptr, xf)) return e;
  return launch_bn_stats_finalize((const double*)workspace, fwd_stat_rows(g), (int64_t)g->B * g->OH * g->OW, g->Cout, eps, momentum,
                                  save_mean, save_invstd, running_mean, running_var, num_batches_tracked, (hipStream_t)stream, true,
                                  gamma, beta, coef_out);
}
extern "C" int pcg_conv2d_fwd_bn(const pcg_conv_geom* g, const float* x, const float* w, const float* bias, float* y, float eps,
                                 float momentum, float* save_mean, float* save_invstd, float* running_mean, float* running_var,
                                 int64_t* num_batches_tracked, void* workspace, size_t workspace_bytes, pcg_stream_t stream) {
  return pcg_conv2d_fwd_bn_xf(g, x, nullptr, w, bias, y, eps, momentum, save_mean, save_invstd, running_mean, running_var,
                              num_batches_tracked, nullptr, nullptr, nullptr, workspace, workspace_bytes, stream);
}
extern "C" int pcg_conv2d_fwd_bn_g(const pcg_conv_geom* g, const float* x, const float* w, const float* bias, float* y, float eps,
                                   float momentum, float* save_mean, float* save_invstd, float* running_mean, float* running_var,
                                   int64_t* num_batches_tracked, int32_t groups, void* workspace, size_t workspace_bytes,
                                   pcg_stream_t stream) {
  const size_t need = pcg_conv2d_fwd_bn_workspace_bytes(g);
  PCG_REQUIRE(need > 0, "pcg_conv2d_fwd_bn_g: only MFMA layers (Cin > 3, Cout > 3, Cout %% 4 == 0)");
  PCG_REQUIRE(save_mean && save_invstd, "pcg_conv2d_fwd_bn_g: null statistics output");
  PCG_REQUIRE(groups >= 1 && groups <= 8 && g->B % groups == 0 && ((int64_t)(g->B / groups) * g->OH * g->OW) % 128 == 0,
              "pcg_conv2d_fwd_bn_g: %d images do not split into %d groups of whole 128-row tiles (%d x %d output)", g->B, groups, g->OH, g->OW);
  if (!workspace || workspace_bytes < need) { set_error("pcg_conv2d_fwd_bn_g: workspace %zu B < required %zu B", workspace_bytes, need); return PCG_ERR_WORKSPACE; }
  if (int e = conv2d_fwd_impl(g, x, w, bias, y, (double*)workspace, nullptr, 0, stream)) return e;
  return launch_bn_stats_finalize_g((const double*)workspace, fwd_stat_rows(g), 1, groups, (int64_t)(g->B / groups) * g->OH * g->OW, g->Cout,
                                    eps, momentum, save_mean, save_invstd, running_mean, running_var, num_batches_tracked, (hipStream_t)stream);
}
extern "C" int pcg_conv2d_fwd_xf(const pcg_conv_geom* g, const float* x, const pcg_in_xform* xf, const float* w, const float* bias,
                                 int act, float slope, float* y, void* workspace, size_t workspace_bytes, pcg_stream_t stream) {
  return conv2d_fwd_impl(g, x, w, bias, y, nullptr, workspace, workspace_bytes, stream, act, slope, nullptr, xf);
}

static int build_phases(const pcg_conv_geom* g, DgradPhases* php, int* maxMp_out) {
  DgradPhases& ph = *php;
  int nph = 0, maxMp = 0, prow = 0;
  const int s = g->stride;
  for (int a = 0; a < s; ++a)
    for (int b = 0; b < s; ++b) {
      PhaseInfo& f = ph.p[nph];
      f.ph = a; f.pw = b;
      f.PHh = a < g->IH ? (g->IH - a + s - 1) / s : 0;
      f.PHw = b < g->IW ? (g->IW - b + s - 1) / s : 0;
      f.Mp = g->B * f.PHh * f.PHw;
      if (f.Mp == 0) continue;
      f.kh0 = (a + g->pad) % s; f.kw0 = (b + g->pad) % s;
      f.nth = f.kh0 < g->KH ? (g->KH - f.kh0 + s - 1) / s : 0;
      f.ntw = f.kw0 < g->KW ? (g->KW - f.kw0 + s - 1) / s : 0;
      if (f.nth == 0 || f.ntw == 0) { f.nth = 0; f.ntw = 1; }
      f.dh0 = (a + g->pad - f.kh0) / s; f.dw0 = (b + g->pad - f.kw0) / s;
      f.dPHw = FastDiv((uint32_t)f.PHw); f.dPHh = FastDiv((uint32_t)f.PHh);
      if (f.Mp > maxMp) maxMp = f.Mp;
      f.prow0 = prow; prow += ceil_div(f.Mp, 128) * 2;
      ++nph;
    }
  *maxMp_out = maxMp;
  return nph;
}

static int conv2d_dgrad_impl(const pcg_conv_geom* g, const float* dy, const float* w, const float* bias_x, float* dx,
                             double* stat_partial, void* workspace, size_t workspace_bytes, pcg_stream_t stream, int act = PCG_ACT_NONE,
                             float slope = 0.f, const EpiAux* epi = nullptr, const pcg_in_xform* xf = nullptr) {
  if (int e = check_geom(g)) return e;
  PCG_REQUIRE(dy && w && dx, "pcg_conv2d_dgrad: null pointer");
  PCG_REQUIRE(act >= PCG_ACT_NONE && act <= PCG_ACT_SIGMOID, "pcg_conv2d_dgrad: unknown activation %d", act);
  const bool has_xf = xf && xf->scale;
  if (thin_is_cin(g) || thin_is_cout(g)) {
    PCG_REQUIRE(!has_xf || thin_conv_xf_ok(g), "pcg_conv2d_dgrad: input transforms on the MFMA path (Cin > 3 and Cout > 3) and on the thin forms of pcg_conv2d_xf_thin_ok only");
    PCG_REQUIRE(!has_xf || (xf->act == PCG_ACT_NONE || xf->act == PCG_ACT_RELU || xf->act == PCG_ACT_LRELU), "pcg_conv2d_dgrad: transform activation %d", has_xf ? xf->act : 0);
    const ThinXf tx{has_xf ? xf->scale : nullptr, has_xf ? xf->shift : nullptr, has_xf ? act_neg_of(xf->act, xf->slope) : 1.f};
    return thin_conv_dgrad(g, dy, w, bias_x, dx, workspace, workspace_bytes, (hipStream_t)stream, act, slope, &tx);
  }
  PCG_REQUIRE(g->Cin % 4 == 0 && g->Cout % 4 == 0, "pcg_conv2d_dgrad: Cin=%d and Cout=%d must be multiples of 4", g->Cin, g->Cout);
  PCG_REQUIRE(g->stride <= 2, "pcg_conv2d_dgrad: stride %d > 2 unsupported", g->stride);
  if (!epi && !stat_partial && !has_xf && dgrad_as_gemm(g, stream_has_sk((hipStream_t)stream)) && workspace && workspace_bytes >= dgrad_gemm_bytes(g) &&
      (((uintptr_t)workspace | (uintptr_t)dx) & 15) == 0) {
    pcg_conv_geom g1 = {g->B, g->OH, g->OW, g->KH * g->KW * g->Cin, g->OH, g->OW, g->Cout, 1, 1, 1, 0};
    float* dcol = (float*)workspace;
    if (int e = conv2d_dgrad_impl(&g1, dy, w, nullptr, dcol, nullptr, nullptr, 0, stream)) return e;
    const bool fuse_act = act_is_cheap(act);
    const int CQ = g->Cin / 4;
    const uint64_t total = (uint64_t)g->B * g->IH * g->IW * CQ;
    unsigned blocks = (unsigned)((total + 255) / 256);
    if (blocks > 8192) blocks = 8192;
    hipLaunchKernelGGL(col2im_kernel, dim3(blocks), dim3(256), 0, (hipStream_t)stream, reinterpret_cast<const float4*>(dcol),
                       reinterpret_cast<float4*>(dx), bias_x, g->B, g->IH, g->IW, CQ, g->OH, g->OW, g->KH, g->KW, g->stride, g->pad,
                       FastDiv((uint32_t)CQ), FastDiv((uint32_t)g->IW), FastDiv((uint32_t)g->IH), fuse_act ? act : PCG_ACT_NONE,
                       act_neg_of(fuse_act ? act : PCG_ACT_NONE, slope));
    if (int e = launch_status("col2im_kernel")) return e;
    return fuse_act ? PCG_OK : pcg_act_fwd(dx, (int64_t)g->B * g->IH * g->IW * g->Cin, act, slope, dx, stream);
  }
  ConvP p = make_params(g);
  const bool fuse = act_is_cheap(act);
  p.dy = dy; p.w = w; p.bias = bias_x; p.out = dx; p.stat_partial = stat_partial;
  if (epi) p.epi = *epi;
  if (int e = set_xform("pcg_conv2d_dgrad", xf, g->Cout, &p)) return e;
  p.act = fuse ? act : PCG_ACT_NONE; p.slope = act_neg_of(p.act, slope);
  p.N = g->Cin;
  DgradPhases ph{};
  int maxMp = 0;
  const int nph = build_phases(g, &ph, &maxMp);
  PCG_REQUIRE(nph > 0, "pcg_conv2d_dgrad: empty problem");
  hipStream_t st = (hipStream_t)stream;
  if (int e = p.N > 64 ? launch_dgrad<Cfg128x128>(p, ph, nph, maxMp, st)
                       : (nph > 1 && g_tune.dgrad_swz3 == 0) ? launch_dgrad<Cfg128x64P>(p, ph, nph, maxMp, st)
                                                             : launch_dgrad<Cfg128x64>(p, ph, nph, maxMp, st)) return e;
  return fuse ? PCG_OK : pcg_act_fwd(dx, (int64_t)g->B * g->IH * g->IW * g->Cin, act, slope, dx, stream);
}

extern "C" int pcg_conv2d_dgrad(const pcg_conv_geom* g, const float* dy, const float* w, const float* bias_x, float* dx,
                                void* workspace, size_t workspace_bytes, pcg_stream_t stream) {
  return conv2d_dgrad_impl(g, dy, w, bias_x, dx, nullptr, workspace, workspace_bytes, stream);
}
extern "C" int pcg_conv2d_dgrad_act(const pcg_conv_geom* g, const float* dy, const float* w, const float* bias_x, int act, float slope,
                                    float* dx, void* workspace, size_t workspace_bytes, pcg_stream_t stream) {
  return conv2d_dgrad_impl(g, dy, w, bias_x, dx, nullptr, workspace, workspace_bytes, stream, act, slope);
}

extern "C" int pcg_conv2d_dgrad_bn_xf(const pcg_conv_geom* g, const float* dy, const pcg_in_xform* xf, const float* w, const float* bias_x,
                                      float* dx, float eps, float momentum, float* save_mean, float* save_invstd, float* running_mean,
                                      float* running_var, int64_t* num_batches_tracked, const float* gamma, const float* beta,
                                      float* coef_out, void* workspace, size_t workspace_bytes, pcg_stream_t stream) {
  const size_t need = pcg_conv2d_dgrad_bn_workspace_bytes(g);
  PCG_REQUIRE(need > 0, "pcg_conv2d_dgrad_bn: only MFMA layers with stride <= 2; use pcg_conv2d_dgrad + pcg_bn_train_stats");
  PCG_REQUIRE(save_mean && save_invstd, "pcg_conv2d_dgrad_bn: null statistics output");
  PCG_REQUIRE(!coef_out || (gamma && beta), "pcg_conv2d_dgrad_bn_xf: coef_out needs gamma and beta");
  if (!workspace || workspace_bytes < need) { set_error("pcg_conv2d_dgrad_bn: workspace %zu B < required %zu B", workspace_bytes, need); return PCG_ERR_WORKSPACE; }
  if (int e = conv2d_dgrad_impl(g, dy, w, bias_x, dx, (double*)workspace, nullptr, 0, stream, PCG_ACT_NONE, 0.f, nullptr, xf)) return e;
  return launch_bn_stats_finalize((const double*)workspace, dgrad_stat_rows(g), (int64_t)g->B * g->IH * g->IW, g->Cin, eps, momentum,
                                  save_mean, save_invstd, running_mean, running_var, num_batches_tracked, (hipStream_t)stream, true,
                                  gamma, beta, coef_out);
}
extern "C" int pcg_conv2d_dgrad_bn(const pcg_conv_geom* g, const float* dy, const float* w, const float* bias_x, float* dx, float eps,
                                   float momentum, float* save_mean, float* save_invstd, float* running_mean, float* running_var,
                                   int64_t* num_batches_tracked, void* workspace, size_t workspace_bytes, pcg_stream_t stream) {
  return pcg_conv2d_dgrad_bn_xf(g, dy, nullptr, w, bias_x, dx, eps, momentum, save_mean, save_invstd, running_mean, running_var,
                                num_batches_tracked, nullptr, nullptr, nullptr, workspace, workspace_bytes, stream);
}
extern "C" int pcg_conv2d_dgrad_xf(const pcg_conv_geom* g, const float* dy, const pcg_in_xform* xf, const float* w, const float* bias_x,
                                   int act, float slope, float* dx, void* workspace, size_t workspace_bytes, pcg_stream_t stream) {
  return conv2d_dgrad_impl(g, dy, w, bias_x, dx, nullptr, workspace, workspace_bytes, stream, act, slope, nullptr, xf);
}

static int epi_common(const char* who, const pcg_conv_geom* g, const float* out, const float* aux, int act, float slope, EpiAux* e) {
  PCG_REQUIRE(mfma_layer(g), "%s: only MFMA layers (Cin > 3 and Cout > 3); use the unfused calls", who);
  PCG_REQUIRE(aux && out, "%s: null pointer", who);
  PCG_REQUIRE(act == PCG_ACT_NONE || act == PCG_ACT_RELU || act == PCG_ACT_LRELU, "%s: activation %d is not none / ReLU / LeakyReLU", who, act);
  PCG_REQUIRE((((uintptr_t)aux | (uintptr_t)out) & 15) == 0, "%s: tensors must be 16-byte aligned", who);
  e->neg = act_neg_of(act, slope);
  e->delta_bytes = (int64_t)((intptr_t)aux - (intptr_t)out);
  return PCG_OK;
}

extern "C" int32_t pcg_conv2d_xf_thin_ok(const pcg_conv_geom* g) { return check_geom(g) == PCG_OK && thin_conv_xf_ok(g) ? 1 : 0; }
extern "C" int32_t pcg_conv2d_dgrad_mask_thin_ok(const pcg_conv_geom* g) { return check_geom(g) == PCG_OK && thin_conv_dgrad_mask_ok(g) && g->Cin % 4 == 0 ? 1 : 0; }
extern "C" int pcg_conv2d_dgrad_mask(const pcg_conv_geom* g, const float* dy, const float* w, const float* a_below, int act, float slope,
                                     float* dx, void* workspace, size_t workspace_bytes, pcg_stream_t stream) {
  EpiAux e{};
  e.mode = EPI_MASK;
  if (int rc = check_geom(g)) return rc;
  if (pcg_conv2d_dgrad_mask_thin_ok(g)) {
    PCG_REQUIRE(dy && w && a_below && dx && (((uintptr_t)a_below | (uintptr_t)dx) & 15) == 0, "pcg_conv2d_dgrad_mask: null or misaligned tensor");
    PCG_REQUIRE(act == PCG_ACT_NONE || act == PCG_ACT_RELU || act == PCG_ACT_LRELU, "pcg_conv2d_dgrad_mask: activation %d is not none / ReLU / LeakyReLU", act);
    return thin_conv_dgrad_mask(g, dy, w, a_below, act, slope, dx, (hipStream_t)stream);
  }
  if (int rc = epi_common("pcg_conv2d_dgrad_mask", g, dx, a_below, act, slope, &e)) return rc;
  return conv2d_dgrad_impl(g, dy, w, nullptr, dx, nullptr, workspace, workspace_bytes, stream, PCG_ACT_NONE, 0.f, &e);
}
extern "C" int pcg_conv2d_fwd_mask(const pcg_conv_geom* g, const float* x, const float* w, const float* a_below, int act, float slope,
                                   float* y, void* workspace, size_t workspace_bytes, pcg_stream_t stream) {
  EpiAux e{};
  e.mode = EPI_MASK;
  if (int rc = check_geom(g)) return rc;
  if (int rc = epi_common("pcg_conv2d_fwd_mask", g, y, a_below, act, slope, &e)) return rc;
  return conv2d_fwd_impl(g, x, w, nullptr, y, nullptr, workspace, workspace_bytes, stream, PCG_ACT_NONE, 0.f, &e);
}

extern "C" int pcg_conv2d_dgrad_add(const pcg_conv_geom* g, const float* dy, const float* w, const float* addend, float* dx,
                                    void* workspace, size_t workspace_bytes, pcg_stream_t stream) {
  EpiAux e{};
  e.mode = EPI_ADD;
  if (int rc = check_geom(g)) return rc;
  if (int rc = epi_common("pcg_conv2d_dgrad_add", g, dx, addend, PCG_ACT_NONE, 0.f, &e)) return rc;
  return conv2d_dgrad_impl(g, dy, w, nullptr, dx, nullptr, workspace, workspace_bytes, stream, PCG_ACT_NONE, 0.f, &e);
}

extern "C" int pcg_conv2d_fwd_add(const pcg_conv_geom* g, const float* x, const float* w, const float* addend, float* y,
                                  void* workspace, size_t workspace_bytes, pcg_stream_t stream) {
  EpiAux e{};
  e.mode = EPI_ADD;
  if (int rc = check_geom(g)) return rc;
  if (int rc = epi_common("pcg_conv2d_fwd_add", g, y, addend, PCG_ACT_NONE, 0.f, &e)) return rc;
  return conv2d_fwd_impl(g, x, w, nullptr, y, nullptr, workspace, workspace_bytes, stream, PCG_ACT_NONE, 0.f, &e);
}
static int add_mask_epi(const char* who, const pcg_conv_geom* g, const float* out, const float* addend, const float* a_below, int act,
                        float slope, EpiAux* e) {
  e->mode = EPI_ADD;
  if (int rc = check_geom(g)) return rc;
  if (int rc = epi_common(who, g, out, addend, act, slope, e)) return rc;
  PCG_REQUIRE(a_below && a_below != out && (((uintptr_t)a_below) & 15) == 0, "%s: a_below must be a 16-byte aligned tensor other than the output", who);
  e->delta2_bytes = (int64_t)((intptr_t)a_below - (intptr_t)out);
  return PCG_OK;
}
extern "C" int pcg_conv2d_fwd_add_mask(const pcg_conv_geom* g, const float* x, const float* w, const float* addend, const float* a_below,
                                       int act, float slope, float* y, pcg_stream_t stream) {
  EpiAux e{};
  if (int rc = add_mask_epi("pcg_conv2d_fwd_add_mask", g, y, addend, a_below, act, slope, &e)) return rc;
  return conv2d_fwd_impl(g, x, w, nullptr, y, nullptr, nullptr, 0, stream, PCG_ACT_NONE, 0.f, &e);
}
extern "C" int pcg_conv2d_dgrad_add_mask(const pcg_conv_geom* g, const float* dy, const float* w, const float* addend, const float* a_below,
                                         int act, float slope, float* dx, pcg_stream_t stream) {
  EpiAux e{};
  if (int rc = add_mask_epi("pcg_conv2d_dgrad_add_mask", g, dx, addend, a_below, act, slope, &e)) return rc;
  return conv2d_dgrad_impl(g, dy, w, nullptr, dx, nullptr, nullptr, 0, stream, PCG_ACT_NONE, 0.f, &e);
}
extern "C" int pcg_conv2d_fwd_add_bnsum(const pcg_conv_geom* g, const float* x, const float* w, const float* addend, const float* z_next,
                                        const float* mean, const float* invstd, float sum_scale, float* y, void* partial,
                                        size_t partial_bytes, pcg_stream_t stream) {
  EpiAux e{};
  e.mode = EPI_ADDSUM;
  if (int rc = check_geom(g)) return rc;
  e.no_addend = addend == nullptr;
  if (int rc = epi_common("pcg_conv2d_fwd_add_bnsum", g, y, addend ? addend : y, PCG_ACT_NONE, 0.f, &e)) return rc;
  const size_t need = pcg_conv2d_fwd_bn_workspace_bytes(g);
  PCG_REQUIRE(need > 0, "pcg_conv2d_fwd_add_bnsum: layer not eligible (MFMA layers, channel count %% 4 == 0)");
  PCG_REQUIRE(z_next && mean && invstd && (((uintptr_t)z_next | (uintptr_t)mean | (uintptr_t)invstd) & 15) == 0,
              "pcg_conv2d_fwd_add_bnsum: z_next / mean / invstd must be non-null and 16-byte aligned");
  if (!partial || partial_bytes < need) { set_error("pcg_conv2d_fwd_add_bnsum: partial-sum buffer %zu B < required %zu B", partial_bytes, need); return PCG_ERR_WORKSPACE; }
  e.neg = sum_scale;
  e.delta2_bytes = (int64_t)((intptr_t)z_next - (intptr_t)y);
  e.mean = mean; e.invstd = invstd;
  return conv2d_fwd_impl(g, x, w, nullptr, y, (double*)partial, nullptr, 0, stream, PCG_ACT_NONE, 0.f, &e);
}

namespace pcg { namespace {
__global__ void __launch_bounds__(256) weight_adjoint_kernel(const float* __restrict__ w, float* __restrict__ wa, int Cout, int KHW, int Cin) {
  const int total = Cout * KHW * Cin;
  for (int o = blockIdx.x * 256 + threadIdx.x; o < total; o += gridDim.x * 256) {
    const int co = o % Cout, t = o / Cout;
    const int tapr = t % KHW, ci = t / KHW;
    wa[o] = w[((size_t)co * KHW + (KHW - 1 - tapr)) * Cin + ci];
  }
}
} }
namespace pcg { namespace {
struct AdjMany { const float* w[16]; float* wa[16]; };
__global__ void __launch_bounds__(256) weight_adjoint_many_kernel(AdjMany a, int Cout, int KHW, int Cin) {
  const float* __restrict__ w = a.w[blockIdx.y];
  float* __restrict__ wa = a.wa[blockIdx.y];
  const int total = Cout * KHW * Cin;
  for (int o = blockIdx.x * 256 + threadIdx.x; o < total; o += gridDim.x * 256) {
    const int co = o % Cout, t = o / Cout;
    const int tapr = t % KHW, ci = t / KHW;
    wa[o] = w[((size_t)co * KHW + (KHW - 1 - tapr)) * Cin + ci];
  }
}
// ... 189 lines not shown
  }
  if constexpr (!TAB) {
    if (p.pixtab) return launch_wgrad_sk_x<Cfg, XFA, XFB, true>(p, sk, s);
  }
  constexpr size_t smem = smem_bytes<Cfg, false, false>();
  static int once = set_smem(conv_wgrad_sk_kernel<Cfg, XFA, XFB, TAB>, smem);
  if (once != PCG_OK) return once;
  hipLaunchKernelGGL((conv_wgrad_sk_kernel<Cfg, XFA, XFB, TAB>), dim3((unsigned)(sk.dp_tiles + sk.sk_blocks)), dim3(IG_THREADS), smem, s, p, sk);
  return launch_status("conv_wgrad_sk_kernel");
}
template <class Cfg, bool TAB = false>
static int launch_wgrad192(const ConvP& p, const WgradPlan& wp, int slice_major, hipStream_t s) {
  if constexpr (!TAB) {
    if (p.pixtab) return launch_wgrad192<Cfg, true>(p, wp, slice_major, s);
  }
  constexpr size_t smem = smem_bytes<Cfg, false, false>();
  static int once = set_smem(conv_wgrad192_kernel<Cfg, TAB>, smem);
  if (once != PCG_OK) return once;
  hipLaunchKernelGGL((conv_wgrad192_kernel<Cfg, TAB>), slice_major ? dim3((unsigned)wp.tiles * wp.splits) : dim3((unsigned)wp.tiles, wp.splits),
                     dim3(IG_THREADS), smem, s, p, wp.ktiles_total, wp.ktiles_per_split, wp.tiles, slice_major);
  return launch_status("conv_wgrad192_kernel");
}
template <class Cfg>
static int launch_wgrad(const ConvP& p, const WgradPlan& wp, int slice_major, int xf_side, hipStream_t s) {
  if constexpr (!Cfg::BF16) {
    if (conv_bf16()) return launch_wgrad<Bf16Twin<Cfg>>(p, wp, slice_major, xf_side, s);
  }
  if (xf_side == 1) return launch_wgrad_x<Cfg, false, true>(p, wp, slice_major, s);
  if (xf_side == 2) return launch_wgrad_x<Cfg, true, false>(p, wp, slice_major, s);
  return launch_wgrad_x<Cfg, false, false>(p, wp, slice_major, s);
}

extern "C" int pcg_conv2d_wgrad_xf(const pcg_conv_geom* g, const float* x, const pcg_in_xform* xf_x, const float* dy,
                                   const pcg_in_xform* xf_dy, float* dw, int accumulate, void* workspace, size_t workspace_bytes,
                                   pcg_stream_t stream) {
  if (int e = check_geom(g)) return e;
  PCG_REQUIRE(x && dy && dw, "pcg_conv2d_wgrad: null pointer");
  const bool hx = xf_x && xf_x->scale, hy = xf_dy && xf_dy->scale;
  PCG_REQUIRE(!(hx && hy), "pcg_conv2d_wgrad_xf: at most one operand can carry an input transform");
  if (thin_is_cin(g) || thin_is_cout(g)) {
    PCG_REQUIRE(!hx && (!hy || thin_conv_xf_ok(g)), "pcg_conv2d_wgrad: input transforms on the MFMA path (Cin > 3 and Cout > 3) and, on the dy side, on the thin forms of pcg_conv2d_xf_thin_ok only");
    PCG_REQUIRE(!hy || (xf_dy->act == PCG_ACT_NONE || xf_dy->act == PCG_ACT_RELU || xf_dy->act == PCG_ACT_LRELU), "pcg_conv2d_wgrad: transform activation %d", hy ? xf_dy->act : 0);
    const ThinXf tx{hy ? xf_dy->scale : nullptr, hy ? xf_dy->shift : nullptr, hy ? act_neg_of(xf_dy->act, xf_dy->slope) : 1.f};
    return thin_conv_wgrad(g, x, dy, dw, accumulate, workspace, workspace_bytes, (hipStream_t)stream, &tx);
  }
  PCG_REQUIRE(g->Cin % 4 == 0 && g->Cout % 4 == 0, "pcg_conv2d_wgrad: Cin=%d and Cout=%d must be multiples of 4", g->Cin, g->Cout);
  const WgradPlan wp = plan_wgrad(g);
  const size_t need = pcg_conv2d_wgrad_workspace_bytes(g);
  if (workspace == nullptr || workspace_bytes < need) {
    set_error("pcg_conv2d_wgrad: workspace %zu B < required %zu B", workspace_bytes, need);
    return PCG_ERR_WORKSPACE;
  }
  PCG_REQUIRE(((uintptr_t)workspace & 15) == 0 && ((uintptr_t)dw & 15) == 0, "pcg_conv2d_wgrad: workspace/dw must be 16-byte aligned");
  ConvP p = make_params(g);
  p.x = x; p.dy = dy; p.out = (float*)workspace;
  p.M = g->Cout; p.N = g->KH * g->KW * g->Cin;
  p.tilesN = ceil_div(p.N, 128);
  p.pixtab = pixtab_of(g);
  if (int e = hx ? set_xform("pcg_conv2d_wgrad_xf", xf_x, g->Cin, &p) : set_xform("pcg_conv2d_wgrad_xf", xf_dy, g->Cout, &p)) return e;
  hipStream_t s = (hipStream_t)stream;
  static const int order_env0 = getenv("PCG_WGRAD_ORDER") ? atoi(getenv("PCG_WGRAD_ORDER")) : -1;
  const int order_env = g_tune.wgrad_order >= 0 ? g_tune.wgrad_order : order_env0;
  const int slice_major = order_env >= 0 ? order_env : (wp.tiles <= 8 ? 1 : 0);
  const int side = hx ? 1 : hy ? 2 : 0;
  if (!wp.narrow && !wp.wide192 && wp.tiles > 96 && sk_mode() != 0) {
    SkPlan sk{};
    bool take = plan_sk(wp.tiles, wp.ktiles_total, s, &sk);
    if (!take && wp.splits == 1) { sk = SkPlan{wp.tiles, 0, 0, wp.ktiles_total, nullptr, nullptr}; take = true; }
    if (take) {
      p.out = dw;
      if (accumulate) { p.epi.mode = EPI_ADD; p.epi.neg = 1.f; p.epi.delta_bytes = 0; }
      return side == 1 ? launch_wgrad_sk_x<Cfg128x128, false, true>(p, sk, s)
           : side == 2 ? launch_wgrad_sk_x<Cfg128x128, true, false>(p, sk, s) : launch_wgrad_sk_x<Cfg128x128, false, false>(p, sk, s);
    }
  }
  int rc;
  if (wp.wide192 && side == 0) {
    p.tilesN = p.N / 192;
    rc = conv_bf16() ? launch_wgrad192<Bf16Twin<Cfg64x192>>(p, wp, slice_major, s) : launch_wgrad192<Cfg64x192>(p, wp, slice_major, s);
  } else {
    WgradPlan wq = wp;
    if (wp.wide192) {
      wq.wide192 = false;
      wq.tiles = ceil_div(p.M, 64) * ceil_div(p.N, 128);
    }
    rc = wq.narrow ? launch_wgrad<TileCfg<64, 128, 1, 4>>(p, wq, slice_major, side, s) : launch_wgrad<Cfg128x128>(p, wq, slice_major, side, s);
  }
  if (rc != PCG_OK) return rc;
  const size_t n = (size_t)p.M * p.N;
  return launch_slab_reduce((const float*)workspace, dw, n, n, wp.splits, accumulate, s, true);
}

extern "C" int pcg_conv2d_wgrad(const pcg_conv_geom* g, const float* x, const float* dy, float* dw, int accumulate,
                                void* workspace, size_t workspace_bytes, pcg_stream_t stream) {
  return pcg_conv2d_wgrad_xf(g, x, nullptr, dy, nullptr, dw, accumulate, workspace, workspace_bytes, stream);
}

extern "C" int pcg_conv_plan_describe(const pcg_conv_geom* g, int32_t op, int32_t assume_scratch, char* out, size_t out_bytes) {
  if (int e = check_geom(g)) return e;
  PCG_REQUIRE(out && out_bytes > 0 && op >= 0 && op <= 2, "pcg_conv_plan_describe: bad arguments");
  const int have = assume_scratch ? (sk_mode() != 0 ? 1 : 0) : (have_sk_scratch() ? 1 : 0);
  char buf[512];
  buf[0] = 0;
  auto say = [&](const char* fmt, auto... a) { snprintf(buf + strlen(buf), sizeof(buf) - strlen(buf), fmt, a...); };
  if (thin_is_cin(g) || thin_is_cout(g)) {
    say("%s", "thin (Cin or Cout <= 3): no matrix-core launch");
  } else if (op == 0) {
    const int M = g->B * g->OH * g->OW, N = g->Cout, kt = g->KH * g->KW * ceil_div(g->Cin, IG_BK);
    const FwdPlan f = plan_fwd(g, have);
    SkPlan sk{};
    if (N <= 64) say("128x64 tiles: %d", ceil_div(M, 128));
    else if (fwd_use_t64(M, N, f.splits)) say("64x128 tiles: %d", ceil_div(M, 64) * ceil_div(N, 128));
    else if (f.splits == 1 && have && plan_sk_shape(ceil_div(M, 128) * ceil_div(N, 128), kt, &sk))
      say("stream-K: %d whole tiles + %d tiles x %d k-tiles over %d ranges", sk.dp_tiles, sk.sk_tiles, kt, sk.sk_blocks);
    else if (f.splits > 1) say("128x128 tiles: %d x %d K-slices of %d k-tiles (slabs)", ceil_div(M, 128) * ceil_div(N, 128), f.splits, f.ktiles_per_split);
    else say("128x128 tiles: %d", ceil_div(M, 128) * ceil_div(N, 128));
  } else if (op == 1) {
    if (dgrad_as_gemm(g, have)) {
      const int M = g->B * g->OH * g->OW, N = g->KH * g->KW * g->Cin, kt = ceil_div(g->Cout, IG_BK), tiles = ceil_div(M, 128) * ceil_div(N, 128);
      SkPlan sk{};
      say("%s", "GEMM + col2im: ");
      if (have && plan_sk_shape(tiles, kt, &sk)) say("stream-K: %d whole tiles + %d tiles x %d k-tiles over %d ranges", sk.dp_tiles, sk.sk_tiles, kt, sk.sk_blocks);
      else say("128x128 tiles: %d", tiles);
    } else {
      DgradPhases ph{};
      int maxMp = 0;
      const int nph = build_phases(g, &ph, &maxMp);
      const int N = g->Cin, tilesN = ceil_div(N, N > 64 ? 128 : 64);
      bool uniform = true;
      for (int i = 0; i < nph; ++i)
        uniform = uniform && ph.p[i].Mp == ph.p[0].Mp && ph.p[i].nth * ph.p[i].ntw == ph.p[0].nth * ph.p[0].ntw && ph.p[i].nth > 0 && ph.p[i].ntw > 0;
      SkNPlan sn{};
      SkPlan sk{};
      say("%d phase%s: ", nph, nph == 1 ? "" : "s");
      if (N > 64 && have && !uniform && plan_skn_shape(ph, nph, 128, tilesN, g->Cout, &sn))
        say("stream-K over unequal phases: %d tiles, %d k-tile iterations over %d ranges", sn.tile0[nph], sn.total, sn.blocks);
      else if (N > 64 && have && uniform && nph > 0 &&
               plan_sk_shape(ceil_div(maxMp, 128) * tilesN * nph, ph.p[0].nth * ph.p[0].ntw * ceil_div(g->Cout, IG_BK), &sk))
        say("stream-K: %d whole tiles + %d tiles over %d ranges", sk.dp_tiles, sk.sk_tiles, sk.sk_blocks);
      else say("%s tiles: %d per phase", N > 64 ? "128x128" : "128x64", ceil_div(maxMp, 128) * tilesN);
    }
  } else {
    const WgradPlan w = plan_wgrad(g);
    SkPlan sk{};
    if (!w.narrow && !w.wide192 && w.tiles > 96 && have && plan_sk_shape(w.tiles, w.ktiles_total, &sk))
      say("stream-K: %d whole tiles + %d tiles x %d k-tiles over %d ranges, dw written by the epilogue", sk.dp_tiles, sk.sk_tiles, w.ktiles_total, sk.sk_blocks);
    else if (!w.narrow && !w.wide192 && w.tiles > 96 && w.splits == 1 && sk_mode() != 0) say("128x128 tiles: %d, dw written by the epilogue", w.tiles);
    else say("%s tiles: %d x %d K-slices of %d k-tiles (slabs + slab_reduce)", w.wide192 ? "64x192" : w.narrow ? "64x128" : "128x128", w.tiles, w.splits, w.ktiles_per_split);
  }
  snprintf(out, out_bytes, "%s", buf);
  return PCG_OK;
}

extern "C" int pcg_tune_set(const char* name, int32_t value) {
  PCG_REQUIRE(name != nullptr, "pcg_tune_set: null name");
  if (!strcmp(name, "korder")) g_tune.korder = value;
  else if (!strcmp(name, "edge_prio")) g_tune.edge_prio = value;
  else if (!strcmp(name, "dgrad_swz3")) g_tune.dgrad_swz3 = value;
  else if (!strcmp(name, "wgrad_rounds")) g_tune.wgrad_rounds = value;
  else if (!strcmp(name, "wgrad_order")) g_tune.wgrad_order = value;
  else if (!strcmp(name, "dgrad_interleave")) g_tune.dgrad_interleave = value;
  else if (!strcmp(name, "fwd_splits")) g_tune.fwd_splits = value;
  else if (!strcmp(name, "stream_k")) g_tune.stream_k = value;
  else if (!strcmp(name, "sk_blocks")) g_tune.sk_blocks = value;
  else if (!strcmp(name, "dgrad_gemm")) g_tune.dgrad_gemm = value;
  else if (!strcmp(name, "t64")) g_tune.t64 = value;
  else if (!strcmp(name, "wgrad_pixtab")) g_tune.wgrad_pixtab = value;
  else {
    set_error("pcg_tune_set: unknown switch '%s' (korder, edge_prio, dgrad_swz3, wgrad_rounds, wgrad_order, dgrad_interleave, fwd_splits, "
              "stream_k, sk_blocks, dgrad_gemm, t64); the loader switch wgrad_pixtab is accepted as well", name);
    return PCG_ERR_INVALID;
  }
  return PCG_OK;
}

extern "C" int pcg_debug_stamp_buffer(void* buf, int64_t bytes) {
  g_tune.stamps = static_cast<unsigned long long*>(buf);
  g_tune.stamp_slots = buf ? (int)(bytes / 16) : 0;
#ifdef PCG_CLOCK_STAMP
  return 1;
#else
  return 0;
#endif
}
```

promptable-counterfactual-gan_amd/csrc/conv_loaders.h:

```cpp
#pragma once
#include "igemm_core.h"

namespace pcg {

__device__ __forceinline__ uint32_t tap_mask(int lo_h, int hi_h, int nh, int lo_w, int hi_w, int nw) {
  lo_h = lo_h < 0 ? 0 : lo_h; hi_h = hi_h > nh ? nh : hi_h;
  lo_w = lo_w < 0 ? 0 : lo_w; hi_w = hi_w > nw ? nw : hi_w;
  if (lo_h >= hi_h || lo_w >= hi_w) return 0u;
  const uint32_t rowbits = ((1u << (hi_w - lo_w)) - 1u) << lo_w;
  uint32_t m = 0;
  for (int a = lo_h; a < hi_h; ++a) m |= rowbits << (a * nw);
  return (hi_w - lo_w) >= 32 ? 0xFFFFFFFFu : m;
}

struct ConvP {
  const float* x;
  const float* w;
  const float* bias;
  float* out;
  const float* dy;
  double* stat_partial;
  int act; float slope;
  EpiAux epi;
  const float* in_sc; const float* in_sh; float in_neg; uint32_t in_c_bytes;
  uint32_t x_bytes, w_bytes, dy_bytes;
  int B, IH, IW, Cin, OH, OW, Cout, KH, KW, stride, pad;
  int M, N;
  int tilesN;
  int ktiles;
  int ktiles_per_split;
  int korder;
  int edge_prio;
  unsigned long long* stamps;
  int stamp_slots;
  FastDiv dOW, dOH;
  const uint32_t* pixtab;
  FastDiv dOHW;
};

struct FwdKIter {
  int KH, KW, Cin, S, mode;
  int ch, cw, jh, jw, ci0;
  __device__ __forceinline__ void init(const ConvP& p) {
    KH = p.KH; KW = p.KW; Cin = p.Cin; mode = p.korder; S = mode ? p.stride : 1;
    ch = cw = jh = jw = ci0 = 0;
  }
  __device__ __forceinline__ int kh() const { return ch + S * jh; }
  __device__ __forceinline__ int kw() const { return cw + S * jw; }
  __device__ __forceinline__ bool next_tap_in_class() {
    if (cw + S * (++jw) < KW) return true;
    jw = 0;
    if (ch + S * (++jh) < KH) return true;
    jh = 0;
    return false;
  }
  __device__ __forceinline__ void next_class() {
    if (++cw >= S || cw >= KW) { cw = 0; ++ch; }
  }
  __device__ __forceinline__ void advance() {
    if (mode == 0) {
      ci0 += IG_BK;
      if (ci0 < Cin) return;
      ci0 = 0;
      next_tap_in_class();
    } else {
      if (next_tap_in_class()) return;
      ci0 += IG_BK;
      if (ci0 < Cin) return;
      ci0 = 0;
      next_class();
    }
  }
  __device__ __forceinline__ void seek(int kt) {
    const int nchunks = (Cin + IG_BK - 1) / IG_BK;
    if (mode == 0) {
      const int tap = kt / nchunks;
      ci0 = (kt - tap * nchunks) * IG_BK;
      jh = tap / KW; jw = tap - jh * KW;
      return;
    }
    for (;;) {
      const int nh = (KH - ch + S - 1) / S, nw = (KW - cw + S - 1) / S, per = nh * nw;
      const int in_class = nchunks * per;
      if (kt < in_class || per <= 0) {
        const int c = per > 0 ? kt / per : 0, t = kt - c * per;
        ci0 = c * IG_BK;
        jh = t / nw; jw = t - jh * nw;
        return;
      }
      kt -= in_class;
      next_class();
    }
  }
};

struct PhaseInfo {
  int ph, pw;
  int PHh, PHw;
  int Mp;
  int kh0, kw0;
  int nth, ntw;
  int dh0, dw0;
  int prow0;
  FastDiv dPHw, dPHh;
};
struct DgradPhases { PhaseInfo p[4]; int interleave; };

struct XfK {
  rsrc_t rsc, rsh;
  float4 sc, sh;
  float neg;
  uint32_t ok;
  __device__ __forceinline__ void init(const ConvP& p) {
    rsc = make_rsrc(p.in_sc, p.in_c_bytes); rsh = make_rsrc(p.in_sh, p.in_c_bytes); neg = p.in_neg; ok = 0;
  }
  __device__ __forceinline__ void fetch(uint32_t c_off_bytes, bool kok) {
    sc = buf_load4(rsc, kok ? c_off_bytes : OOB_OFF);
    sh = buf_load4(rsh, kok ? c_off_bytes : OOB_OFF);
  }
};
__device__ __forceinline__ float4 xf_apply(float4 v, float4 sc, float4 sh, float neg, bool ok) {
  float4 t = make_float4(fmaf(v.x, sc.x, sh.x), fmaf(v.y, sc.y, sh.y), fmaf(v.z, sc.z, sh.z), fmaf(v.w, sc.w, sh.w));
  t.x = act_neg_scale(t.x, neg); t.y = act_neg_scale(t.y, neg); t.z = act_neg_scale(t.z, neg); t.w = act_neg_scale(t.w, neg);
  return ok ? t : make_float4(0.f, 0.f, 0.f, 0.f);
}

template <int ROWS_, bool XF = false>
struct FwdALoader {
  static constexpr bool KMAJOR = true, XFORM = XF;
  static constexpr int ROWS = ROWS_, NV = ROWS_ / 32;
  rsrc_t rs;
  uint32_t base[NV], mask[NV];
  int IW, Cin, KW, kq4;
  FwdKIter it;
  XfK xf;

  __device__ __forceinline__ FwdALoader(const ConvP& p, int m_block, int tid) {
    if constexpr (XF) xf.init(p);
    rs = make_rsrc(p.x, p.x_bytes);
    IW = p.IW; Cin = p.Cin; KW = p.KW;
    it.init(p);
    kq4 = (tid & 7) * 4;
    const int r0 = tid >> 3;
#pragma unroll
    for (int i = 0; i < NV; ++i) {
      const int m = m_block + r0 + 32 * i;
      uint32_t mk = 0, bs = OOB_OFF;
      if (m < p.M) {
        uint32_t t, ow, b, oh;
        p.dOW.divmod((uint32_t)m, t, ow);
        p.dOH.divmod(t, b, oh);
        const int ih0 = (int)oh * p.stride - p.pad, iw0 = (int)ow * p.stride - p.pad;
        bs = (uint32_t)(((((int)b * p.IH + ih0) * IW + iw0) * Cin + kq4) * 4);
        mk = tap_mask(-ih0, p.IH - ih0, p.KH, -iw0, IW - iw0, KW);
      }
      base[i] = bs; mask[i] = mk;
    }
  }
  __device__ __forceinline__ void seek(int kt) { it.seek(kt); }
  __device__ __forceinline__ void load_next(float4 (&v)[NV]) {
    const int kh = it.kh(), kw = it.kw(), ci0 = it.ci0;
    const int tap = kh * KW + kw;
    const uint32_t delta = (uint32_t)(((kh * IW + kw) * Cin + ci0) * 4);
    const bool kok = kq4 < Cin - ci0;
    uint32_t okbits = 0;
#pragma unroll
    for (int i = 0; i < NV; ++i) {
      const bool ok = kok && ((mask[i] >> tap) & 1u);
      v[i] = buf_load4(rs, ok ? base[i] + delta : OOB_OFF);
      if constexpr (XF) okbits |= (ok ? 1u : 0u) << i;
    }
    if constexpr (XF) { xf.ok = okbits; xf.fetch((uint32_t)((ci0 + kq4) * 4), kok); }
    it.advance();
  }
  __device__ __forceinline__ void transform(float4 (&v)[NV]) {
    if constexpr (XF) {
#pragma unroll
      for (int i = 0; i < NV; ++i) v[i] = xf_apply(v[i], xf.sc, xf.sh, xf.neg, (xf.ok >> i) & 1u);
    }
  }
};

template <int ROWS_>
struct FwdBLoader {
  static constexpr bool KMAJOR = true, XFORM = false;
  static constexpr int ROWS = ROWS_, NV = ROWS_ / 32;
  rsrc_t rs;
  uint32_t base[NV];
  int Cin, KW, kq4;
  FwdKIter it;

  __device__ __forceinline__ FwdBLoader(const ConvP& p, int n_block, int tid) {
    rs = make_rsrc(p.w, p.w_bytes);
    Cin = p.Cin; KW = p.KW; kq4 = (tid & 7) * 4;
    it.init(p);
    const int r0 = tid >> 3;
    const int Ktot = p.KH * p.KW * p.Cin;
#pragma unroll
    for (int i = 0; i < NV; ++i) {
      const int n = n_block + r0 + 32 * i;
      base[i] = n < p.N ? (uint32_t)((n * Ktot + kq4) * 4) : OOB_OFF;
    }
  }
  __device__ __forceinline__ void seek(int kt) { it.seek(kt); }
  __device__ __forceinline__ void load_next(float4 (&v)[NV]) {
    const int ci0 = it.ci0;
    const uint32_t delta = (uint32_t)(((it.kh() * KW + it.kw()) * Cin + ci0) * 4);
    const bool kok = kq4 < Cin - ci0;
#pragma unroll
    for (int i = 0; i < NV; ++i) v[i] = buf_load4(rs, kok ? base[i] + delta : OOB_OFF);
    it.advance();
  }
  __device__ __forceinline__ void transform(float4 (&)[NV]) {}
};

struct DgradTapIter {
  int Cout, nth, ntw, jw, co0, jh, mode;
  __device__ __forceinline__ void init(int Cout_, int nth_, int ntw_, int mode_) {
    Cout = Cout_; nth = nth_; ntw = ntw_; mode = mode_; jh = 0; jw = 0; co0 = 0;
  }
  __device__ __forceinline__ void advance() {
    if (mode == 0) {
      co0 += IG_BK;
      if (co0 >= Cout) { co0 = 0; if (++jw == ntw) { jw = 0; ++jh; } }
    } else {
      if (++jw < ntw) return;
      jw = 0;
      if (++jh < nth) return;
      jh = 0;
      co0 += IG_BK;
    }
  }
  __device__ __forceinline__ void seek(int kt) {
    const int ntaps = nth * ntw;
    int tap;
    if (mode == 0) {
      const int nchunks = (Cout + IG_BK - 1) / IG_BK;
      tap = kt / nchunks;
      co0 = (kt - tap * nchunks) * IG_BK;
    } else {
      const int c = kt / ntaps;
      tap = kt - c * ntaps;
      co0 = c * IG_BK;
    }
    jh = tap / ntw; jw = tap - jh * ntw;
  }
};

template <int ROWS_, bool XF = false>
struct DgradALoader {
  static constexpr bool KMAJOR = true, XFORM = XF;
  static constexpr int ROWS = ROWS_, NV = ROWS_ / 32;
  rsrc_t rs;
  uint32_t base[NV], mask[NV];
  int OW, Cout, kq4;
  DgradTapIter it;
  XfK xf;

  __device__ __forceinline__ DgradALoader(const ConvP& p, const PhaseInfo& f, int m_block, int tid) {
    if constexpr (XF) xf.init(p);
    rs = make_rsrc(p.dy, p.dy_bytes);
    OW = p.OW; Cout = p.Cout;
    kq4 = (tid & 7) * 4;
    const int r0 = tid >> 3;
#pragma unroll
    for (int i = 0; i < NV; ++i) {
      const int m = m_block + r0 + 32 * i;
      uint32_t mk = 0, bs = OOB_OFF;
      if (m < f.Mp) {
        uint32_t t, cc, b, aa;
        f.dPHw.divmod((uint32_t)m, t, cc);
        f.dPHh.divmod(t, b, aa);
        const int oh0 = (int)aa + f.dh0, ow0 = (int)cc + f.dw0;
        bs = (uint32_t)(((((int)b * p.OH + oh0) * OW + ow0) * Cout + kq4) * 4);
        mk = tap_mask(oh0 - p.OH + 1, oh0 + 1, f.nth, ow0 - OW + 1, ow0 + 1, f.ntw);
      }
      base[i] = bs; mask[i] = mk;
    }
    it.init(Cout, f.nth, f.ntw, p.korder);
  }
  __device__ __forceinline__ void seek(int kt) { it.seek(kt); }
  __device__ __forceinline__ void load_next(float4 (&v)[NV]) {
    const int tap = it.jh * it.ntw + it.jw;
    const uint32_t delta = (uint32_t)((it.co0 - (it.jh * OW + it.jw) * Cout) * 4);
    const bool kok = kq4 < Cout - it.co0;
    uint32_t okbits = 0;
#pragma unroll
    for (int i = 0; i < NV; ++i) {
      const bool ok = kok && ((mask[i] >> tap) & 1u);
      v[i] = buf_load4(rs, ok ? base[i] + delta : OOB_OFF);
      if constexpr (XF) okbits |= (ok ? 1u : 0u) << i;
    }
    if constexpr (XF) { xf.ok = okbits; xf.fetch((uint32_t)((it.co0 + kq4) * 4), kok); }
    it.advance();
  }
  __device__ __forceinline__ void transform(float4 (&v)[NV]) {
    if constexpr (XF) {
#pragma unroll
      for (int i = 0; i < NV; ++i) v[i] = xf_apply(v[i], xf.sc, xf.sh, xf.neg, (xf.ok >> i) & 1u);
    }
  }
};

template <int ROWS_>
struct DgradBLoader {
  static constexpr bool KMAJOR = false, XFORM = false;
  static constexpr int ROWS = ROWS_, NV = ROWS_ / 32;
  static constexpr int C4 = ROWS_ / 4, KR = IG_LOADERS / C4;
  rsrc_t rs;
  uint32_t base[NV];
  int Cin, KHKW, KW, stride, kh0, kw0, kr0;
  DgradTapIter it;

  __device__ __forceinline__ DgradBLoader(const ConvP& p, const PhaseInfo& f, int n_block, int tid) {
    rs = make_rsrc(p.w, p.w_bytes);
    Cin = p.Cin; KHKW = p.KH * p.KW; KW = p.KW; stride = p.stride; kh0 = f.kh0; kw0 = f.kw0;
    const int c4 = tid % C4;
    kr0 = tid / C4;
    const int n = n_block + 4 * c4;
#pragma unroll
    for (int i = 0; i < NV; ++i)
      base[i] = n < p.N ? (uint32_t)(((mn_krow<NV>(kr0, i) * KHKW) * Cin + n) * 4) : OOB_OFF;
    it.init(p.Cout, f.nth, f.ntw, p.korder);
  }
  __device__ __forceinline__ void seek(int kt) { it.seek(kt); }
  __device__ __forceinline__ void load_next(float4 (&v)[NV]) {
    const int tap = (kh0 + stride * it.jh) * KW + kw0 + stride * it.jw;
    const uint32_t delta = (uint32_t)(((it.co0 * KHKW + tap) * Cin) * 4);
    const int krem = it.Cout - it.co0;
#pragma unroll
    for (int i = 0; i < NV; ++i) v[i] = buf_load4(rs, mn_krow<NV>(kr0, i) < krem ? base[i] + delta : OOB_OFF);
    it.advance();
  }
  __device__ __forceinline__ void transform(float4 (&)[NV]) {}
};

template <int ROWS_, bool XF = false>
struct WgradALoader {
  static constexpr bool KMAJOR = false, XFORM = XF;
  static constexpr int ROWS = ROWS_, NV = ROWS_ / 32;
  static constexpr int C4 = ROWS_ / 4, KR = IG_LOADERS / C4;
  rsrc_t rs;
  uint32_t base[NV];
  int Cout, K, q0, kr0;
  float4 sc, sh; float neg; uint32_t okb; bool mok;

  __device__ __forceinline__ WgradALoader(const ConvP& p, int m_block, int kt_begin, int tid) {
    rs = make_rsrc(p.dy, p.dy_bytes);
    Cout = p.Cout; K = p.B * p.OH * p.OW;
    const int c4 = tid % C4;
    kr0 = tid / C4;
    const int m = m_block + 4 * c4;
    mok = m < p.M;
#pragma unroll
    for (int i = 0; i < NV; ++i) base[i] = mok ? (uint32_t)((mn_krow<NV>(kr0, i) * Cout + m) * 4) : OOB_OFF;
    q0 = kt_begin * IG_BK;
    if constexpr (XF) {
      neg = p.in_neg; okb = 0;
      sc = mok ? *reinterpret_cast<const float4*>(p.in_sc + m) : make_float4(0.f, 0.f, 0.f, 0.f);
      sh = mok ? *reinterpret_cast<const float4*>(p.in_sh + m) : make_float4(0.f, 0.f, 0.f, 0.f);
    }
  }
  __device__ __forceinline__ void load_next(float4 (&v)[NV]) {
    const uint32_t delta = (uint32_t)(q0 * Cout * 4);
    const int krem = K - q0;
    uint32_t okbits = 0;
#pragma unroll
    for (int i = 0; i < NV; ++i) {
      const bool ok = mn_krow<NV>(kr0, i) < krem;
      v[i] = buf_load4(rs, ok ? base[i] + delta : OOB_OFF);
      if constexpr (XF) okbits |= ((ok && mok) ? 1u : 0u) << i;
    }
    if constexpr (XF) okb = okbits;
    q0 += IG_BK;
  }
  __device__ __forceinline__ void transform(float4 (&v)[NV]) {
    if constexpr (XF) {
#pragma unroll
      for (int i = 0; i < NV; ++i) v[i] = xf_apply(v[i], sc, sh, neg, (okb >> i) & 1u);
    }
  }
};

typedef uint32_t u32x16 __attribute__((ext_vector_type(16)));
typedef u32x16 u32x16_dw __attribute__((aligned(4)));
struct PixDesc8 {
  struct Tile {
    u32x16 d; uint32_t base; int qd, K;
    __device__ __forceinline__ uint32_t off(int j) const { return base + d[2 * j]; }
    __device__ __forceinline__ uint32_t mask(int j) const { return qd + j < K ? d[2 * j + 1] : 0u; }
  };
  const __attribute__((address_space(4))) uint32_t* tab;
  FastDiv dOHW;
  uint32_t img_bytes;
  Tile t;
  __device__ __forceinline__ void init(const ConvP& p) {
    tab = (const __attribute__((address_space(4))) uint32_t*)p.pixtab;
    dOHW = p.dOHW; img_bytes = (uint32_t)(p.IH * p.IW * p.Cin * 4); t.K = p.B * p.OH * p.OW;
  }
  __device__ __forceinline__ void fetch(int qw) {
    qw = __builtin_amdgcn_readfirstlane(qw);
    uint32_t img, r;
    dOHW.divmod((uint32_t)qw, img, r);
    t.base = img * img_bytes; t.qd = qw;
    t.d = *reinterpret_cast<const __attribute__((address_space(4))) u32x16_dw*>(tab + 2 * r);
  }
  __device__ __forceinline__ static void landed() { __builtin_amdgcn_s_waitcnt(0xC07F); }
};
__device__ __forceinline__ uint32_t pick4(uint32_t a, uint32_t b, uint32_t c, uint32_t d, bool g1, bool g2) {
  return g2 ? (g1 ? d : c) : (g1 ? b : a);
}
__device__ __forceinline__ void pick_desc4(const PixDesc8::Tile& pd, int h, bool g1, bool g2, uint32_t& off, uint32_t& mask) {
  off = pick4(pd.off(h), pd.off(2 + h), pd.off(4 + h), pd.off(6 + h), g1, g2);
  mask = pick4(pd.mask(h), pd.mask(2 + h), pd.mask(4 + h), pd.mask(6 + h), g1, g2);
}

template <int ROWS_, bool XF = false, bool TAB = false>
struct WgradBLoader {
  static constexpr bool KMAJOR = false, XFORM = XF;
  static constexpr int ROWS = ROWS_, NV = ROWS_ / 32;
  static constexpr int C4 = ROWS_ / 4, KR = IG_LOADERS / C4;
  static constexpr bool SCALAR_PIX = C4 == 32;
  rsrc_t rs;
  int IH, IW, Cin, stride, K, q0, kr0, OH, OW, dh, dw, ci;
  int lane_off;
  bool nok;
  FastDiv dOW, dOH;
  float4 sc, sh; float neg; uint32_t okb;
  static_assert(!TAB || SCALAR_PIX, "the table loader is written for 128-column tiles");
  PixDesc8 pd;
  int qw0;
  uint32_t tab_off;
  uint32_t himask, tb_lo, tb_hi;

  __device__ __forceinline__ WgradBLoader(const ConvP& p, int n_block, int kt_begin, int tid) {
    rs = make_rsrc(p.x, p.x_bytes);
    IH = p.IH; IW = p.IW; Cin = p.Cin; stride = p.stride; K = p.B * p.OH * p.OW;
    dOW = p.dOW; dOH = p.dOH;
    const int c4 = tid % C4;
    const int n = n_block + 4 * c4;
    nok = n < p.N;
    const int tap = nok ? n / Cin : 0;
    ci = nok ? n - tap * Cin : 0;
    const int kh = tap / p.KW, kw = tap - kh * p.KW;
    dh = kh - p.pad; dw = kw - p.pad;
    lane_off = ((dh * IW + dw) * Cin + ci) * 4;
    q0 = kt_begin * IG_BK; kr0 = tid / C4; OH = p.OH; OW = p.OW;
    if constexpr (TAB) {
      pd.init(p);
      himask = (tid & 32) ? 0xFFFFFFFFu : 0u;
      const uint32_t tapbit = nok ? 1u << tap : 0u;
      tab_off = (uint32_t)(((kh * IW + kw) * Cin + ci) * 4);
      qw0 = __builtin_amdgcn_readfirstlane(8 * (tid >> 6));
      tb_lo = tapbit & ~himask; tb_hi = tapbit & himask;
      pd.fetch(q0 + qw0);
      PixDesc8::landed();
    }
    if constexpr (XF) {
      neg = p.in_neg; okb = 0;
      sc = nok ? *reinterpret_cast<const float4*>(p.in_sc + ci) : make_float4(0.f, 0.f, 0.f, 0.f);
      sh = nok ? *reinterpret_cast<const float4*>(p.in_sh + ci) : make_float4(0.f, 0.f, 0.f, 0.f);
    }
  }
  __device__ __forceinline__ void load_next(float4 (&v)[NV]) {
    uint32_t okbits = 0;
// ... 148 lines not shown
```

promptable-counterfactual-gan_amd/ops.py:

```python
import ctypes
import threading

import torch

from . import _lib
from ._lib import ACT_LRELU, ACT_NONE, ACT_RELU, ACT_SIGMOID, ACT_TANH, ConvGeom, check

_ws_cache = {}

_conv_hook = None


def set_conv_hook(hook):
    global _conv_hook
    _conv_hook = hook


def _conv_label(g, op):
    if g.Cin <= 3 or g.Cout <= 3:
        return f"thin_{op}"
    if op == "wgrad":
        n = g.KH * g.KW * g.Cin
        if g.Cout <= 64:
            return "conv_wgrad192_kernel<64x192>" if (n % 192 == 0 and n % 128 != 0) else "conv_wgrad_kernel<64x128>"
        return "conv_wgrad_kernel<128x128>"
    n = g.Cout if op == "fwd" else g.Cin
    if n > 64:
        return f"conv_{op}_kernel<128x128>"
    swz = op == "fwd" or g.stride == 1
    return f"conv_{op}_kernel<128x64{'/swz3' if swz else ''}>"


def _conv_flops(g):
    return 2.0 * g.B * g.OH * g.OW * g.Cout * g.KH * g.KW * g.Cin


class _Timed:
    def __init__(self, g, op):
        _conv_scratch()
        self.on = _conv_hook is not None
        if self.on:
            self.g, self.op = g, op
            self.t0 = torch.cuda.Event(enable_timing=True)
            self.t1 = torch.cuda.Event(enable_timing=True)

    def __enter__(self):
        if self.on:
            self.t0.record()
        return self

    def __exit__(self, *exc):
        if self.on:
            self.t1.record()
            _conv_hook(_conv_label(self.g, self.op), _conv_flops(self.g), self.t0, self.t1)
        return False


_sk_streams = {}
_sk_pool = {}
_sk_arrival_pool = _sk_pool
_SK_SPARES = 2
_sk_last = None


def _stream():
    return ctypes.c_void_p(torch.cuda.current_stream().cuda_stream)


def prepare_conv_scratch(device_index=None):
    if device_index is None:
        device_index = torch.cuda.current_device()
    if torch.cuda.is_current_stream_capturing():
        return
    lib = _lib.load()
    dev = torch.device("cuda", device_index)
    nparts, narr = lib.pcg_conv_scratch_parts_bytes(), lib.pcg_conv_scratch_arrivals_bytes()
    pool = _sk_pool.setdefault(device_index, [])
    while len(pool) < _SK_SPARES:
        pool.append((torch.empty(nparts, dtype=torch.uint8, device=dev), torch.zeros(narr, dtype=torch.uint8, device=dev)))


def _conv_scratch():
    global _sk_last
    s = torch.cuda.current_stream()
    key = (s.device_index, s.cuda_stream)
    if key == _sk_last:
        return
    if key not in _sk_streams:
        capturing = torch.cuda.is_current_stream_capturing()
        if not capturing:
            prepare_conv_scratch(s.device_index)
        pool = _sk_pool.setdefault(s.device_index, [])
        if not pool:
            raise _lib.PcgError("conv call on a new stream inside a HIP-graph capture with no spare stream-K scratch left: call "
                                "pcgan_amd.ops.prepare_conv_scratch() on this device before capturing (the scratch must not come "
                                "from the graph's private memory pool)")
        parts, arrivals = pool.pop()
        lib = _lib.load()
        if lib.pcg_conv_set_scratch(ctypes.c_void_p(s.cuda_stream), _p(parts), parts.numel(), _p(arrivals), arrivals.numel()) == 0:
            _sk_streams[key] = (parts, arrivals)
        else:
            pool.append((parts, arrivals))
            _sk_streams[key] = None
        if not capturing:
            prepare_conv_scratch(s.device_index)
    _sk_last = key


_pixtabs = {}


def _pixtab_key(g, device_index):
    return (device_index, g.IH, g.IW, g.OH, g.OW, g.stride, g.pad, g.KH, g.KW, g.Cin)


def prepare_conv_pixtab(g, device=None):
    device = torch.device("cuda", torch.cuda.current_device()) if device is None else device
    key = _pixtab_key(g, device.index)
    if key in _pixtabs or torch.cuda.is_current_stream_capturing():
        return _pixtabs.get(key)
    lib = _lib.load()
    n = lib.pcg_conv_pixtab_bytes(ctypes.byref(g))
    host = torch.empty(n, dtype=torch.uint8)
    check(lib.pcg_conv_pixtab_register(ctypes.byref(g), _p(host), n, None), "pcg_conv_pixtab_register")
    with torch.cuda.device(device):
        tab = host.to(device)
        check(lib.pcg_conv_pixtab_register(ctypes.byref(g), None, 0, _p(tab)), "pcg_conv_pixtab_register")
    _pixtabs[key] = tab
    return tab


def drop_conv_pixtab(g, device=None):
    device = torch.device("cuda", torch.cuda.current_device()) if device is None else device
    with torch.cuda.device(device):
        check(_lib.load().pcg_conv_pixtab_register(ctypes.byref(g), None, 0, None), "pcg_conv_pixtab_register")
    _pixtabs[_pixtab_key(g, device.index)] = None


def _p(t):
    return ctypes.c_void_p(t.data_ptr()) if t is not None else ctypes.c_void_p(0)


def _chk(t, name, dtype=torch.float32):
    if not t.is_cuda:
        raise _lib.PcgError(f"{name}: expected a tensor on the GPU (libpcgan_hip has no CPU path), got {t.device}")
    if t.dtype != dtype:
        raise _lib.PcgError(f"{name}: expected {dtype}, got {t.dtype}")
    if not t.is_contiguous():
        raise _lib.PcgError(f"{name}: expected a contiguous tensor, got strides {t.stride()} for shape {tuple(t.shape)}")
    return t


_ws_retired = []


def _scratch(kind, nbytes, device):
    stream = torch.cuda.current_stream(device).cuda_stream if device.type == "cuda" else 0
    key = (device.type, device.index, stream, kind)
    buf = _ws_cache.get(key)
    if buf is None or buf.numel() < nbytes:
        if buf is not None:
            _ws_retired.append(buf)
        buf = torch.empty(max(int(nbytes), 1 << 20), dtype=torch.uint8, device=device)
        _ws_cache[key] = buf
    return buf


def workspace(nbytes, device):
    return _scratch(0, nbytes, device)


def workspace2(nbytes, device):
    return _scratch(2, nbytes, device)


_ticket_pool = {}


def _ticket_buffer(device):
    stream = torch.cuda.current_stream(device).cuda_stream if device.type == "cuda" else 0
    key = (device.type, device.index, stream, "tickets")
    tk = _ws_cache.get(key)
    if tk is None:
        n = _lib.load().pcg_linear_wgrad_ticket_count()
        pool = _ticket_pool.setdefault((device.type, device.index), [])
        capturing = device.type == "cuda" and torch.cuda.is_current_stream_capturing()
        if not pool and not capturing:
            pool.extend(torch.zeros((8, n), dtype=torch.int32, device=device).unbind(0))
        tk = pool.pop() if pool else torch.zeros(n, dtype=torch.int32, device=device)
        _ws_cache[key] = tk
    return tk


def ohwi(w):
    v = w.permute(0, 2, 3, 1)
    if not v.is_contiguous():
        raise _lib.PcgError("conv weight is not in channels_last (OHWI) memory layout; FlatModule keeps it that way")
    return v


def conv_geom(B, IH, IW, Cin, Cout, KH, KW, stride, pad):
    OH = (IH + 2 * pad - KH) // stride + 1
    OW = (IW + 2 * pad - KW) // stride + 1
    return ConvGeom(B, IH, IW, Cin, OH, OW, Cout, KH, KW, stride, pad)


class InputXform:

    def __init__(self, coef, act, slope):
        C = coef.numel() // 2
        self.coef, self.act, self.slope, self.C = coef, int(act), float(slope), C
        self.c_struct = _lib.InXform(coef.data_ptr(), coef.data_ptr() + 4 * C, int(act), float(slope))

    def ref(self):
        return ctypes.byref(self.c_struct)


def xform_ok(g, operand):
    return g.Cin > 3 and g.Cout > 3 and g.Cin % 4 == 0 and g.Cout % 4 == 0 and g.stride <= 2


class BnInput:

    def __init__(self, mean, invstd, gamma, beta, act, slope, groups=1):
        self.mean, self.invstd, self.gamma, self.beta = mean, invstd, gamma, beta
        self.act, self.slope, self.groups = int(act), float(slope), int(groups)


def bnin_full_ok(g, groups=1):
    return bool(_lib.load().pcg_conv2d_bnin_full_ok(ctypes.byref(g), int(groups)))


def xform_thin_ok(g):
    return bool(_lib.load().pcg_conv2d_xf_thin_ok(ctypes.byref(g)))


def _xref(xf):
    return xf.ref() if xf is not None else None


def conv2d_fwd(g, x, w, bias=None, out=None, act=0, slope=0.0, xf=None):
    _chk(x, "x"); _chk(w, "w")
    assert x.numel() == g.B * g.IH * g.IW * g.Cin and w.numel() == g.Cout * g.KH * g.KW * g.Cin
    y = out if out is not None else torch.empty((g.B, g.OH, g.OW, g.Cout), dtype=torch.float32, device=x.device)
    lib = _lib.load()
    need = lib.pcg_conv2d_fwd_workspace_bytes(ctypes.byref(g))
    ws = workspace(need, x.device) if need else None
    with _Timed(g, "fwd"):
        if isinstance(xf, BnInput):
            check(lib.pcg_conv2d_fwd_bnin_full(ctypes.byref(g), _p(x), _p(xf.mean), _p(xf.invstd), _p(xf.gamma), _p(xf.beta), xf.act, xf.slope,
                                               xf.groups, _p(w), _p(bias), int(act), float(slope), _p(y), _stream()), "pcg_conv2d_fwd_bnin_full")
        elif xf is not None:
            assert xf.C == g.Cin
            check(lib.pcg_conv2d_fwd_xf(ctypes.byref(g), _p(x), xf.ref(), _p(w), _p(bias), int(act), float(slope), _p(y), _p(ws),
                                        ws.numel() if need else 0, _stream()), "pcg_conv2d_fwd_xf")
        else:
            check(lib.pcg_conv2d_fwd_act(ctypes.byref(g), _p(x), _p(w), _p(bias), int(act), float(slope), _p(y), _p(ws),
                                         ws.numel() if need else 0, _stream()), "pcg_conv2d_fwd_act")
    return y


def conv2d_dgrad(g, dy, w, bias_x=None, out=None, act=0, slope=0.0, xf=None):
    _chk(dy, "dy"); _chk(w, "w")
    assert dy.numel() == g.B * g.OH * g.OW * g.Cout and w.numel() == g.Cout * g.KH * g.KW * g.Cin
    dx = out if out is not None else torch.empty((g.B, g.IH, g.IW, g.Cin), dtype=torch.float32, device=dy.device)
    lib = _lib.load()
    need = lib.pcg_conv2d_dgrad_workspace_bytes(ctypes.byref(g))
    ws = workspace(need, dy.device) if need else None
    with _Timed(g, "dgrad"):
        if xf is not None:
            assert xf.C == g.Cout
            check(lib.pcg_conv2d_dgrad_xf(ctypes.byref(g), _p(dy), xf.ref(), _p(w), _p(bias_x), int(act), float(slope), _p(dx), _p(ws),
                                          ws.numel() if need else 0, _stream()), "pcg_conv2d_dgrad_xf")
        else:
            check(lib.pcg_conv2d_dgrad_act(ctypes.byref(g), _p(dy), _p(w), _p(bias_x), int(act), float(slope), _p(dx), _p(ws),
                                           ws.numel() if need else 0, _stream()), "pcg_conv2d_dgrad_act")
    return dx


def conv_bn_train(g, a, w, bias, transposed, eps, momentum, running_mean, running_var, num_batches_tracked, xf=None, gamma=None,
                  beta=None):
    _chk(a, "a"); _chk(w, "w")
    lib = _lib.load()
    C = g.Cin if transposed else g.Cout
    shape = (g.B, g.IH, g.IW, g.Cin) if transposed else (g.B, g.OH, g.OW, g.Cout)
    need = (lib.pcg_conv2d_dgrad_bn_workspace_bytes if transposed else lib.pcg_conv2d_fwd_bn_workspace_bytes)(ctypes.byref(g))
    want_coef = gamma is not None
    if need == 0:
        z = conv2d_dgrad(g, a, w, bias, xf=xf) if transposed else conv2d_fwd(g, a, w, bias, xf=xf)
# ... 1371 lines not shown
```

Before: 51810.

## Add pad-clipped conv tiles that skip zero-padding taps via position-major tiling

Adds a clipped variant of the forward and dgrad implicit-GEMM kernels for 4x4 stride-2 pad-1 convolutions. M tiles are regrouped so each block covers one output position across a batch slice, and the K loop then iterates only over kernel taps that fall inside the image. A host-side table of per-position tap ranges, sorted longest-first, plus a CU scheduling model decide at plan time whether clipping pays off and which tile order to use. The aim is to stop spending MFMA work on padding border taps, at the cost of uneven per-block work, extra host planning and a new table upload.

Result: faster. 52760 (median of 6 runs) (+1.8%).

```diff
diff --git a/include/pcgan_hip.h b/include/pcgan_hip.h
--- a/include/pcgan_hip.h
+++ b/include/pcgan_hip.h
@@ -584,6 +584,11 @@
 int pcg_conv_reset_scratch(pcg_stream_t stream);
 size_t pcg_conv_pixtab_bytes(const pcg_conv_geom* g);
 int pcg_conv_pixtab_register(const pcg_conv_geom* g, void* host_out, size_t bytes, const void* device_table);
+size_t pcg_conv_cliptab_bytes(const pcg_conv_geom* g);
+int pcg_conv_cliptab_register(const pcg_conv_geom* g, void* host_out, size_t bytes, const void* device_table);
+double pcg_conv_sched_model(const int32_t* ktiles, int32_t n);
+int pcg_conv_pad_clip_query(const pcg_conv_geom* g, int32_t op, int32_t groups, int32_t assume_scratch, int32_t* taken, int32_t* order,
+                            int32_t* tile_rows, double* predicted);
 int pcg_debug_stamp_buffer(void* buf, int64_t bytes);
 
 typedef struct pcg_moons_cf_desc {
diff --git a/promptable-counterfactual-gan_amd/_lib.py b/promptable-counterfactual-gan_amd/_lib.py
--- a/promptable-counterfactual-gan_amd/_lib.py
+++ b/promptable-counterfactual-gan_amd/_lib.py
@@ -221,6 +221,10 @@
     "pcg_conv_reset_scratch": (_i, [_vp]),
     "pcg_conv_pixtab_bytes": (_sz, [_gp]),
     "pcg_conv_pixtab_register": (_i, [_gp, _vp, _sz, _vp]),
+    "pcg_conv_cliptab_bytes": (_sz, [_gp]),
+    "pcg_conv_cliptab_register": (_i, [_gp, _vp, _sz, _vp]),
+    "pcg_conv_sched_model": (_d, [_vp, _i32]),
+    "pcg_conv_pad_clip_query": (_i, [_gp, _i32, _i32, _i32, _vp, _vp, _vp, _vp]),
     "pcg_conv2d_fwd_bn_g": (_i, [_gp, _vp, _vp, _vp, _vp, _f, _f, _vp, _vp, _vp, _vp, _vp, _i32, _vp, _sz, _vp]),
     "pcg_bn_apply_act_g": (_i, [_vp, _i64, _i32, _vp, _vp, _vp, _vp, _i, _f, _vp, _i32, _vp]),
     "pcg_conv2d_dgrad_bn_phases": (_i32, [_gp]),
diff --git a/promptable-counterfactual-gan_amd/csrc/conv_cliptab.h b/promptable-counterfactual-gan_amd/csrc/conv_cliptab.h
--- /dev/null
+++ b/promptable-counterfactual-gan_amd/csrc/conv_cliptab.h
@@ -0,0 +1,104 @@
+#pragma once
+#include <cstddef>
+#include <cstdint>
+#include <algorithm>
+#include <vector>
+
+#if defined(__HIPCC__)
+#define PCG_CLIP_HD __host__ __device__ __forceinline__
+#else
+#define PCG_CLIP_HD inline
+#endif
+
+namespace pcg {
+
+enum { CLIP_LONG_FIRST = 0, CLIP_SHORT_FIRST = 1, CLIP_PAIRS = 2 };
+
+PCG_CLIP_HD void clip_block_tile(uint32_t b, uint32_t per, uint32_t tilesM, int order, bool ygrid, uint32_t y, uint32_t& within, uint32_t& idx) {
+  const uint32_t q = b >> 3, x = b & 7u, r = q / per;
+  within = q - r * per;
+  const uint32_t mt = r * 8u + x, back = tilesM - 1u - mt;
+  idx = order == CLIP_LONG_FIRST ? mt : order == CLIP_SHORT_FIRST ? back : ygrid ? ((y & 1u) ? back : mt) : (mt & 1u) ? tilesM - 1u - (mt >> 1) : (mt >> 1);
+}
+
+inline bool clip_geom_ok(int IH, int IW, int OH, int OW, int stride, int pad, int KH, int KW) {
+  return stride == 2 && pad == 1 && KH == 4 && KW == 4 && IH == 2 * OH && IW == 2 * OW && OH >= 1 && OW >= 1 && OH * OW < 65536;
+}
+inline size_t cliptab_words(int OH, int OW) { return (size_t)5 * OH * OW; }
+
+inline uint32_t clip_desc(int pos, int h0, int nh, int w0, int nw) {
+  return (uint32_t)pos | (uint32_t)h0 << 16 | (uint32_t)nh << 20 | (uint32_t)w0 << 24 | (uint32_t)nw << 28;
+}
+PCG_CLIP_HD int clip_desc_taps(uint32_t d) { return (int)((d >> 20) & 15u) * (int)(d >> 28); }
+
+inline void cliptab_build(int OH, int OW, uint32_t* out) {
+  const int npos = OH * OW, IH = 2 * OH, IW = 2 * OW;
+  std::vector<uint32_t> d((size_t)npos);
+  auto sorted_out = [&](uint32_t* dst) {
+    std::stable_sort(d.begin(), d.end(), [](uint32_t a, uint32_t b) { return clip_desc_taps(a) > clip_desc_taps(b); });
+    std::copy(d.begin(), d.end(), dst);
+  };
+  auto range = [](int base, int sign, int n, int extent, int& lo, int& cnt) {
+    lo = n; cnt = 0;
+    for (int t = 0; t < n; ++t) {
+      const int v = base + sign * t;
+      if (v >= 0 && v < extent) { if (cnt == 0) lo = t; ++cnt; }
+    }
+  };
+  for (int oh = 0; oh < OH; ++oh)
+    for (int ow = 0; ow < OW; ++ow) {
+      int h0, nh, w0, nw;
+      range(oh * 2 - 1, 1, 4, IH, h0, nh);
+      range(ow * 2 - 1, 1, 4, IW, w0, nw);
+      d[(size_t)oh * OW + ow] = clip_desc(oh * OW + ow, h0, nh, w0, nw);
+    }
+  sorted_out(out);
+  for (int py = 0; py < 4; ++py) {
+    const int ph = py >> 1, pw = py & 1;
+    const int kh0 = (ph + 1) % 2, kw0 = (pw + 1) % 2, dh0 = (ph + 1 - kh0) / 2, dw0 = (pw + 1 - kw0) / 2;
+    for (int a = 0; a < OH; ++a)
+      for (int c = 0; c < OW; ++c) {
+        int h0, nh, w0, nw;
+        range(a + dh0, -1, 2, OH, h0, nh);
+        range(c + dw0, -1, 2, OW, w0, nw);
+        d[(size_t)a * OW + c] = clip_desc(a * OW + c, h0, nh, w0, nw);
+      }
+    sorted_out(out + (size_t)(1 + py) * npos);
+  }
+}
+
+inline double clip_sched_model(const int* len, int n) {
+  constexpr int SLOTS = 512, CUS = 256;
+  constexpr double SHARED = 3.5, ALONE = 2.2;
+  double rem[SLOTS];
+  bool busy[SLOTS];
+  int next = 0;
+  for (int s = 0; s < SLOTS; ++s) { busy[s] = next < n; rem[s] = busy[s] ? (double)len[next++] : 0.0; }
+  double t = 0.0;
+  int order[SLOTS];
+  for (int c = 0; c < CUS; ++c) { order[2 * c] = c; order[2 * c + 1] = c + CUS; }
+  for (;;) {
+    double dt = -1.0;
+    for (int s = 0; s < SLOTS; ++s)
+      if (busy[s]) {
+        const double d = rem[s] * (busy[s ^ CUS] ? SHARED : ALONE);
+        if (dt < 0.0 || d < dt) dt = d;
+      }
+    if (dt < 0.0) return t;
+    t += dt;
+    bool freed[SLOTS];
+    for (int s = 0; s < SLOTS; ++s) freed[s] = false;
+    for (int s = 0; s < SLOTS; ++s)
+      if (busy[s]) {
+        rem[s] -= dt / (busy[s ^ CUS] ? SHARED : ALONE);
+        freed[s] = rem[s] < 1e-9;
+      }
+    for (int s = 0; s < SLOTS; ++s) if (freed[s]) busy[s] = false;
+    for (int i = 0; i < SLOTS; ++i) {
+      const int s = order[i];
+      if (freed[s] && next < n) { busy[s] = true; rem[s] = (double)len[next++]; }
+    }
+  }
+}
+
+}
diff --git a/promptable-counterfactual-gan_amd/csrc/conv_igemm.hip b/promptable-counterfactual-gan_amd/csrc/conv_igemm.hip
--- a/promptable-counterfactual-gan_amd/csrc/conv_igemm.hip
+++ b/promptable-counterfactual-gan_amd/csrc/conv_igemm.hip
@@ -1,7 +1,10 @@
 #include <string.h>
+#include <array>
+#include <map>
 #include <mutex>
 #include "conv_loaders.h"
 #include "conv_pixtab.h"
+#include "conv_cliptab.h"
 #include "thin_conv.h"
 
 namespace pcg {
@@ -16,10 +19,39 @@
   return p.epi.group_rows > 0 ? __builtin_amdgcn_readfirstlane(m_block / p.epi.group_rows) * p.N : 0;
 }
 
-template <class Cfg, bool XF>
+template <class Cfg, bool XF, bool CLIP = false>
 __global__ void __launch_bounds__(IG_THREADS, Cfg::MINW) conv_fwd_kernel(ConvP p) {
   extern __shared__ __attribute__((aligned(16))) float smem[];
   prio_entry(p);
+  if constexpr (CLIP) {
+    uint32_t nt, idx;
+    clip_block_tile(blockIdx.x, (uint32_t)p.tilesN, gridDim.x / (uint32_t)p.tilesN, p.clip_order, false, 0u, nt, idx);
+    nt = __builtin_amdgcn_readfirstlane(nt); idx = __builtin_amdgcn_readfirstlane(idx);
+    const ClipTile t = clip_tile(p, 0, idx, Cfg::BM);
+    const int n_block = (int)nt * Cfg::BN;
+    const int ktiles = t.nh * t.nw * ((p.Cin + IG_BK - 1) / IG_BK);
+    if (wave_id() >= 4) {
+      const int tid = threadIdx.x - IG_LOADERS;
+      FwdALoader<Cfg::BM, XF, true> la(p, t, tid);
+      FwdBLoader<Cfg::BN, true> lb(p, n_block, tid);
+      lb.it.clip(t.h0, t.nh, t.w0, t.nw);
+      igemm_produce<Cfg>(la, lb, ktiles, smem, tid, ClockStamp{p.stamps, p.stamp_slots});
+      return;
+    }
+    f32x16 acc[Cfg::TM][Cfg::TN];
+    ClockStamp cs{p.stamps, p.stamp_slots};
+    cs.phase(0);
+    igemm_consume<Cfg, true, true>(ktiles, acc, smem, cs);
+    prio_epilogue(p);
+    const size_t npix = (size_t)p.OH * p.OW;
+    igemm_store_tile<Cfg>(acc, smem, n_block, p.N, p.bias, [&](int row) -> float* {
+      const int b = t.img0 + row;
+      return b < p.B ? p.out + ((size_t)b * npix + t.pos) * p.N + n_block : nullptr;
+    }, p.stat_partial ? p.stat_partial + (size_t)t.stat_tile * Cfg::WAVES_M * 2 * p.N : nullptr, p.act, p.slope, &p.epi,
+       p.epi.group_rows > 0 ? t.group * p.N : 0);
+    cs.phase(3);
+    return;
+  }
   const uint32_t tile = xcd_remap(blockIdx.x, gridDim.x);
   const int mt = tile / p.tilesN, nt = tile % p.tilesN;
   const int m_block = mt * Cfg::BM, n_block = nt * Cfg::BN;
@@ -52,11 +84,46 @@
   cs.phase(3);
 }
 
-template <class Cfg, bool XF>
+template <class Cfg, bool XF, bool CLIP = false>
 __global__ void __launch_bounds__(IG_THREADS, Cfg::MINW) conv_dgrad_kernel(ConvP p, DgradPhases phases) {
   extern __shared__ __attribute__((aligned(16))) float smem[];
   __shared__ int rowpix[Cfg::BM];
   prio_entry(p);
+  if constexpr (CLIP) {
+    const uint32_t nil = phases.interleave ? (uint32_t)phases.interleave : 1u, per = nil * (uint32_t)p.tilesN;
+    uint32_t within, idx;
+    clip_block_tile(blockIdx.x, per, gridDim.x / per, p.clip_order, !phases.interleave, blockIdx.y, within, idx);
+    idx = __builtin_amdgcn_readfirstlane(idx);
+    const uint32_t py = __builtin_amdgcn_readfirstlane(phases.interleave ? within % nil : blockIdx.y), nt = __builtin_amdgcn_readfirstlane(within / nil);
+    const PhaseInfo& f = phases.p[py];
+    const ClipTile t = clip_tile(p, 1 + 2 * f.ph + f.pw, idx, Cfg::BM);
+    const int n_block = (int)nt * Cfg::BN;
+    const int ktiles = t.nh * t.nw * ((p.Cout + IG_BK - 1) / IG_BK);
+    if (wave_id() >= 4) {
+      const int tid = threadIdx.x - IG_LOADERS;
+      uint32_t aa, cc;
+      f.dPHw.divmod((uint32_t)t.pos, aa, cc);
+      const int pix0 = ((int)aa * p.stride + f.ph) * p.IW + (int)cc * p.stride + f.pw;
+      for (int r = tid; r < Cfg::BM; r += IG_LOADERS) rowpix[r] = t.img0 + r < p.B ? (t.img0 + r) * p.IH * p.IW + pix0 : -1;
+      DgradALoader<Cfg::BM, XF, true> la(p, f, t, tid);
+      DgradBLoader<Cfg::BN, true> lb(p, f, n_block, tid);
+      lb.it.clip(t.h0, t.nh, t.w0, t.nw);
+      igemm_produce<Cfg>(la, lb, ktiles, smem, tid, ClockStamp{p.stamps, p.stamp_slots});
+      return;
+    }
+    f32x16 acc[Cfg::TM][Cfg::TN];
+    ClockStamp cs{p.stamps, p.stamp_slots};
+    cs.phase(0);
+    igemm_consume<Cfg, true, false>(ktiles, acc, smem, cs);
+    prio_epilogue(p);
+    igemm_store_tile<Cfg>(acc, smem, n_block, p.N, p.bias, [&](int row) -> float* {
+      const int pix = rowpix[row];
+      return pix >= 0 ? p.out + (size_t)pix * p.Cin + n_block : nullptr;
+    }, p.stat_partial ? p.stat_partial + (size_t)(f.prow0 + t.stat_tile * Cfg::WAVES_M) * 2 * p.N : nullptr, p.act, p.slope, &p.epi,
+       p.epi.group_rows > 0 ? t.group * p.N : 0);
+    cs.phase(3);
+    return;
+  }
   uint32_t bx = blockIdx.x, py = blockIdx.y;
   if (phases.interleave) {
     const uint32_t l = xcd_remap(blockIdx.x, gridDim.x);
@@ -484,6 +551,9 @@
 }
 
 using Cfg128x128 = TileCfg<128, 128, 2, 2>;
+#ifndef PCG_PAD_CLIP_DEFAULT
+#define PCG_PAD_CLIP_DEFAULT 1
+#endif
 #ifndef PCG_TILE64_SWZ
 #define PCG_TILE64_SWZ 1
 #endif
@@ -512,7 +582,7 @@
   return PCG_OK;
 }
 
-struct Tune { int edge_prio = -1, dgrad_swz3 = -1, wgrad_rounds = -1, korder = -1, wgrad_order = -1, dgrad_interleave = -1, fwd_splits = -1, stream_k = -1, sk_blocks = -1, dgrad_gemm = -1, t64 = -1, wgrad_pixtab = -1; unsigned long long* stamps = nullptr; int stamp_slots = 0; };
+struct Tune { int edge_prio = -1, dgrad_swz3 = -1, wgrad_rounds = -1, korder = -1, wgrad_order = -1, dgrad_interleave = -1, fwd_splits = -1, stream_k = -1, sk_blocks = -1, dgrad_gemm = -1, t64 = -1, wgrad_pixtab = -1, pad_clip = -1; unsigned long long* stamps = nullptr; int stamp_slots = 0; };
 Tune g_tune;
 
 ConvP make_params(const pcg_conv_geom* g) {
@@ -594,6 +664,76 @@
     if (pixtab_same(g_pixtab[i], dev, g)) return g_pixtab[i].tab;
   return nullptr;
 }
+struct ClipTabReg { int device, OH, OW; const uint32_t* tab; };
+constexpr int CLIPTAB_MAX = 64;
+ClipTabReg g_cliptab[CLIPTAB_MAX];
+int g_cliptab_n = 0;
+std::mutex g_clip_mutex;
+int clip_mode() {
+  static const int env = getenv("PCG_PAD_CLIP") ? atoi(getenv("PCG_PAD_CLIP")) : PCG_PAD_CLIP_DEFAULT;
+  return g_tune.pad_clip >= 0 ? g_tune.pad_clip : env;
+}
+const uint32_t* cliptab_of(const pcg_conv_geom* g) {
+  std::lock_guard<std::mutex> lock(g_clip_mutex);
+  if (g_cliptab_n == 0) return nullptr;
+  const int dev = current_device();
+  for (int i = 0; i < g_cliptab_n; ++i)
+    if (g_cliptab[i].device == dev && g_cliptab[i].OH == g->OH && g_cliptab[i].OW == g->OW) return g_cliptab[i].tab;
+  return nullptr;
+}
+struct ClipShape { int form, OH, OW, B, tilesN, interleave, bm0, alt64; };
+struct ClipPlan { bool take; int order, bm; double ratio; };
+constexpr double CLIP_UNIT64 = 254.0 / (479.0 / 2.0) / 2.0;
+constexpr double CLIP_TAKE = 0.95;
+constexpr double CLIP_DGRAD_COST = 1.21;
+double clip_predict(const ClipShape& c, int bm, int order) {
+  const int npos = c.OH * c.OW, tpp = c.B / bm, tilesM = npos * tpp, nph = c.form ? 4 : 1;
+  const int per = (c.form && c.interleave ? nph : 1) * c.tilesN, gx = tilesM * per, gy = c.form && !c.interleave ? nph : 1;
+  std::vector<uint32_t> tab(cliptab_words(c.OH, c.OW));
+  cliptab_build(c.OH, c.OW, tab.data());
+  std::vector<int> len((size_t)gx * gy);
+  for (int y = 0; y < gy; ++y)
+    for (int b = 0; b < gx; ++b) {
+      uint32_t within, idx;
+      clip_block_tile((uint32_t)b, (uint32_t)per, (uint32_t)tilesM, order < 0 ? 0 : order, gy > 1, (uint32_t)y, within, idx);
+      const int py = c.form ? (c.interleave ? (int)(within % (uint32_t)nph) : y) : 0;
+      len[(size_t)y * gx + b] = order < 0 ? (c.form ? 4 : 16) : clip_desc_taps(tab[(size_t)(c.form ? 1 + py : 0) * npos + idx / (uint32_t)tpp]);
+    }
+  return clip_sched_model(len.data(), (int)len.size()) * (bm == 64 ? CLIP_UNIT64 : 1.0) * (c.form && order >= 0 ? CLIP_DGRAD_COST : 1.0);
+}
+ClipPlan plan_clip(const ClipShape& c) {
+  static std::map<std::array<int, 9>, ClipPlan> cache;
+  const int mode = clip_mode();
+  const std::array<int, 9> key = {c.form, c.OH, c.OW, c.B, c.tilesN, c.interleave, c.bm0, c.alt64, mode};
+  std::lock_guard<std::mutex> lock(g_clip_mutex);
+  auto it = cache.find(key);
+  if (it != cache.end()) return it->second;
+  ClipPlan best{false, 0, c.bm0, 1.0};
+  const double t0 = clip_predict(c, c.B % c.bm0 ? 64 : c.bm0, -1);
+  if (mode >= 2) {
+    const bool rows64 = mode >= 5 && c.alt64 && c.B % 64 == 0 && (c.OH * c.OW * (c.B / 64)) % 8 == 0;
+    best = ClipPlan{true, (mode - 2) % 3, rows64 ? 64 : c.bm0, 0.0};
+    best.ratio = clip_predict(c, best.bm, best.order) / t0;
+  } else {
+    for (int h = 0; h < 2; ++h) {
+      const int bm = h ? 64 : 128;
+      if (bm != c.bm0 && !(bm == 64 && c.alt64)) continue;
+      if (c.B % bm || (c.OH * c.OW * (c.B / bm)) % 8) continue;
+      for (int order = 0; order < 3; ++order) {
+        const double r = clip_predict(c, bm, order) / t0;
+        if (r < best.ratio - 1e-9) best = ClipPlan{false, order, bm, r};
+      }
+    }
+    best.take = best.ratio <= CLIP_TAKE + 1e-9;
+  }
+  cache[key] = best;
+  return best;
+}
+bool clip_shape_ok(const pcg_conv_geom* g, int groups, int bm) {
+  return clip_geom_ok(g->IH, g->IW, g->OH, g->OW, g->stride, g->pad, g->KH, g->KW) && groups >= 1 && g->B % groups == 0 &&
+         (g->B / groups) % bm == 0 && (g->OH * g->OW * (g->B / bm)) % 8 == 0;
+}
+
 int sk_mode() {
   static const int env = getenv("PCG_STREAM_K") ? atoi(getenv("PCG_STREAM_K")) : 1;
   return g_tune.stream_k >= 0 ? g_tune.stream_k : env;
@@ -659,6 +799,18 @@
   return p.in_sc ? launch_fwd_x<Cfg, true>(p, splits, s) : launch_fwd_x<Cfg, false>(p, splits, s);
 }
 
+template <class Cfg, bool XF>
+int launch_fwd_clip_x(ConvP p, hipStream_t s) {
+  p.tilesN = ceil_div(p.N, Cfg::BN);
+  constexpr size_t smem = smem_bytes<Cfg, true, true>();
+  static int once = set_smem(conv_fwd_kernel<Cfg, XF, true>, smem);
+  if (once != PCG_OK) return once;
+  hipLaunchKernelGGL((conv_fwd_kernel<Cfg, XF, true>), dim3((unsigned)(p.clip_npos * p.clip_tpp * p.tilesN)), dim3(IG_THREADS), smem, s, p);
+  return launch_status("conv_fwd_kernel (clipped)");
+}
+template <class Cfg>
+int launch_fwd_clip(const ConvP& p, hipStream_t s) { return p.in_sc ? launch_fwd_clip_x<Cfg, true>(p, s) : launch_fwd_clip_x<Cfg, false>(p, s); }
+
 struct FwdPlan { int splits, ktiles_per_split; };
 FwdPlan plan_fwd(const pcg_conv_geom* g, int have_sk = -1) {
   if (have_sk < 0) have_sk = have_sk_scratch() ? 1 : 0;
@@ -712,11 +864,30 @@
   return ok;
 }
 
+bool dgrad_interleaved(uint32_t w_bytes, const DgradPhases& ph, int nphases) {
+  static const int il_env0 = getenv("PCG_DGRAD_INTERLEAVE") ? atoi(getenv("PCG_DGRAD_INTERLEAVE")) : 1;
+  const int il_env = g_tune.dgrad_interleave >= 0 ? g_tune.dgrad_interleave : il_env0;
+  bool same = nphases > 1 && il_env && w_bytes <= (1u << 20);
+  for (int i = 1; i < nphases; ++i) same = same && ph.p[i].Mp == ph.p[0].Mp;
+  return same;
+}
+
 template <class Cfg, bool XF>
 int launch_dgrad_x(ConvP p, const DgradPhases& ph, int nphases, int maxMp, hipStream_t s) {
   p.tilesN = ceil_div(p.N, Cfg::BN);
   const int tilesM = ceil_div(maxMp, Cfg::BM);
   constexpr size_t smem = smem_bytes<Cfg, true, false>();
+  if constexpr (!Cfg::BF16) {
+    if (p.cliptab) {
+      static int once_c = set_smem(conv_dgrad_kernel<Cfg, XF, true>, smem);
+      if (once_c != PCG_OK) return once_c;
+      DgradPhases phc = ph;
+      phc.interleave = dgrad_interleaved(p.w_bytes, ph, nphases) ? nphases : 0;
+      const unsigned tiles = (unsigned)(p.clip_npos * p.clip_tpp * p.tilesN);
+      hipLaunchKernelGGL((conv_dgrad_kernel<Cfg, XF, true>), phc.interleave ? dim3(tiles * nphases) : dim3(tiles, nphases), dim3(IG_THREADS), smem, s, p, phc);
+      return launch_status("conv_dgrad_kernel (clipped)");
+    }
+  }
   if constexpr (Cfg::BM == 128 && Cfg::BN == 128) {
     bool uniform = true;
     for (int i = 0; i < nphases; ++i)
@@ -747,11 +918,8 @@
   }
   static int once = set_smem(conv_dgrad_kernel<Cfg, XF>, smem);
   if (once != PCG_OK) return once;
-  static const int il_env0 = getenv("PCG_DGRAD_INTERLEAVE") ? atoi(getenv("PCG_DGRAD_INTERLEAVE")) : 1;
-  const int il_env = g_tune.dgrad_interleave >= 0 ? g_tune.dgrad_interleave : il_env0;
   DgradPhases phl = ph;
-  bool same = nphases > 1 && il_env && p.w_bytes <= (1u << 20);
-  for (int i = 1; i < nphases; ++i) same = same && ph.p[i].Mp == ph.p[0].Mp;
+  const bool same = dgrad_interleaved(p.w_bytes, ph, nphases);
   phl.interleave = same ? nphases : 0;
   if (same)
     hipLaunchKernelGGL((conv_dgrad_kernel<Cfg, XF>), dim3((unsigned)tilesM * p.tilesN * nphases), dim3(IG_THREADS), smem, s, p, phl);
@@ -898,6 +1066,40 @@
   return PCG_OK;
 }
 
+extern "C" size_t pcg_conv_cliptab_bytes(const pcg_conv_geom* g) {
+  if (check_geom(g) != PCG_OK || !pcg::clip_geom_ok(g->IH, g->IW, g->OH, g->OW, g->stride, g->pad, g->KH, g->KW)) return 0;
+  return pcg::cliptab_words(g->OH, g->OW) * sizeof(uint32_t);
+}
+extern "C" int pcg_conv_cliptab_register(const pcg_conv_geom* g, void* host_out, size_t bytes, const void* device_table) {
+  using namespace pcg;
+  if (int e = check_geom(g)) return e;
+  const size_t need = pcg_conv_cliptab_bytes(g);
+  PCG_REQUIRE(need > 0, "pcg_conv_cliptab_register: only k4 s2 p1 geometries with IH = 2 OH and IW = 2 OW have a tile table");
+  if (host_out) {
+    PCG_REQUIRE(bytes >= need && (((uintptr_t)host_out) & 3) == 0, "pcg_conv_cliptab_register: host buffer %zu B (need %zu), 4-byte aligned", bytes, need);
+    cliptab_build(g->OH, g->OW, static_cast<uint32_t*>(host_out));
+    if (!device_table) return PCG_OK;
+  }
+  PCG_REQUIRE((((uintptr_t)device_table) & 3) == 0, "pcg_conv_cliptab_register: misaligned table");
+  const int dev = current_device();
+  std::lock_guard<std::mutex> lock(g_clip_mutex);
+  int at = -1;
+  for (int i = 0; i < g_cliptab_n; ++i) if (g_cliptab[i].device == dev && g_cliptab[i].OH == g->OH && g_cliptab[i].OW == g->OW) at = i;
+  if (!device_table) {
+    if (at >= 0) g_cliptab[at] = g_cliptab[--g_cliptab_n];
+    return PCG_OK;
+  }
+  if (at < 0) {
+    PCG_REQUIRE(g_cliptab_n < CLIPTAB_MAX, "pcg_conv_cliptab_register: more than %d geometries with a table", CLIPTAB_MAX);
+    at = g_cliptab_n++;
+  }
+  g_cliptab[at] = ClipTabReg{dev, g->OH, g->OW, static_cast<const uint32_t*>(device_table)};
+  return PCG_OK;
+}
+extern "C" double pcg_conv_sched_model(const int32_t* ktiles, int32_t n) {
+  return ktiles && n > 0 ? pcg::clip_sched_model(ktiles, n) : 0.0;
+}
+
 extern "C" size_t pcg_conv2d_dgrad_workspace_bytes(const pcg_conv_geom* g) {
   if (check_geom(g) != PCG_OK) return 0;
   if (thin_is_cin(g) || thin_is_cout(g)) return thin_conv_dgrad_workspace_bytes(g);
@@ -931,9 +1133,30 @@
   const int tiles128 = ceil_div(M, 128) * ceil_div(N, 128);
   return g_tune.t64 != 0 && N > 64 && splits == 1 && tiles128 > 224 && tiles128 <= 256 && M % 128 == 0;
 }
+static ClipPlan clip_fwd_plan(const pcg_conv_geom* g, int groups, bool t64, bool plain) {
+  const ClipPlan none{false, 0, 0, 1.0};
+  const int bm0 = t64 ? 64 : 128;
+  if (clip_mode() == 0 || conv_bf16() || !plain || !mfma_layer(g) || g->Cin % 4 ||
+      !(clip_shape_ok(g, groups, bm0) || (clip_mode() >= 5 && g->Cout > 64 && clip_shape_ok(g, groups, 64)))) return none;
+  const int N = g->Cout;
+  const ClipShape c{0, g->OH, g->OW, g->B, ceil_div(N, N > 64 ? 128 : 64), 0, bm0, N > 64 && !t64 ? 1 : 0};
+  const ClipPlan cp = plan_clip(c);
+  return cp.take && clip_shape_ok(g, groups, cp.bm) ? cp : ClipPlan{false, cp.order, cp.bm, cp.ratio};
+}
+static ClipPlan clip_dgrad_plan(const pcg_conv_geom* g, int groups, bool interleave, bool plain) {
+  const ClipPlan none{false, 0, 0, 1.0};
+  if (clip_mode() == 0 || conv_bf16() || !plain || !mfma_layer(g) || g->Cin % 4 || g->Cout % 4 || !clip_shape_ok(g, groups, 128)) return none;
+  const int N = g->Cin;
+  const ClipShape c{1, g->OH, g->OW, g->B, ceil_div(N, N > 64 ? 128 : 64), interleave ? 1 : 0, 128, 0};
+  return plan_clip(c);
+}
+static void clip_apply(const pcg_conv_geom* g, const ClipPlan& cp, int groups, const uint32_t* tab, ConvP* p) {
+  p->cliptab = tab; p->clip_order = cp.order; p->clip_tpp = g->B / cp.bm; p->clip_tpg = p->clip_tpp / groups; p->clip_npos = g->OH * g->OW;
+}
+
 static int conv2d_fwd_impl(const pcg_conv_geom* g, const float* x, const float* w, const float* bias, float* y,
                            double* stat_partial, void* workspace, size_t workspace_bytes, pcg_stream_t stream, int act = PCG_ACT_NONE,
-                           float slope = 0.f, const EpiAux* epi = nullptr, const pcg_in_xform* xf = nullptr) {
+                           float slope = 0.f, const EpiAux* epi = nullptr, const pcg_in_xform* xf = nullptr, int groups = 1) {
   if (int e = check_geom(g)) return e;
   PCG_REQUIRE(x && w && y, "pcg_conv2d_fwd: null pointer");
   PCG_REQUIRE(act >= PCG_ACT_NONE && act <= PCG_ACT_SIGMOID, "pcg_conv2d_fwd: unknown activation %d", act);
@@ -958,7 +1181,16 @@
   p.act = fuse ? act : PCG_ACT_NONE; p.slope = act_neg_of(p.act, slope);
   if (f.splits > 1) { p.out = (float*)workspace; p.ktiles_per_split = f.ktiles_per_split; }
   const bool t64 = fwd_use_t64(p.M, p.N, f.splits);
-  if (int e = t64 ? launch_fwd<TileCfg<64, 128, 1, 4>>(p, f.splits, s)
+  int clip_bm = 0;
+  if (const uint32_t* tab = clip_mode() != 0 ? cliptab_of(g) : nullptr) {
+    SkPlan sk{};
+    const bool plain = f.splits == 1 && !(p.N > 64 && !t64 && plan_sk(ceil_div(p.M, 128) * ceil_div(p.N, 128), p.ktiles, s, &sk));
+    const ClipPlan cp = clip_fwd_plan(g, groups, t64, plain);
+    if (cp.take) { clip_apply(g, cp, groups, tab, &p); clip_bm = cp.bm; }
+  }
+  if (int e = clip_bm == 64 ? launch_fwd_clip<TileCfg<64, 128, 1, 4>>(p, s)
+                  : clip_bm ? (p.N > 64 ? launch_fwd_clip<Cfg128x128>(p, s) : launch_fwd_clip<Cfg128x64>(p, s))
+                  : t64 ? launch_fwd<TileCfg<64, 128, 1, 4>>(p, f.splits, s)
                   : p.N > 64 ? launch_fwd<Cfg128x128>(p, f.splits, s)
                        : launch_fwd<Cfg128x64>(p, f.splits, s)) return e;
   if (f.splits > 1) {
@@ -1016,7 +1248,7 @@
   PCG_REQUIRE(groups >= 1 && groups <= 8 && g->B % groups == 0 && ((int64_t)(g->B / groups) * g->OH * g->OW) % 128 == 0,
               "pcg_conv2d_fwd_bn_g: %d images do not split into %d groups of whole 128-row tiles (%d x %d output)", g->B, groups, g->OH, g->OW);
   if (!workspace || workspace_bytes < need) { set_error("pcg_conv2d_fwd_bn_g: workspace %zu B < required %zu B", workspace_bytes, need); return PCG_ERR_WORKSPACE; }
-  if (int e = conv2d_fwd_impl(g, x, w, bias, y, (double*)workspace, nullptr, 0, stream)) return e;
+  if (int e = conv2d_fwd_impl(g, x, w, bias, y, (double*)workspace, nullptr, 0, stream, PCG_ACT_NONE, 0.f, nullptr, nullptr, groups)) return e;
   return launch_bn_stats_finalize_g((const double*)workspace, fwd_stat_rows(g), 1, groups, (int64_t)(g->B / groups) * g->OH * g->OW, g->Cout,
                                     eps, momentum, save_mean, save_invstd, running_mean, running_var, num_batches_tracked, (hipStream_t)stream);
 }
@@ -1095,6 +1327,13 @@
   const int nph = build_phases(g, &ph, &maxMp);
   PCG_REQUIRE(nph > 0, "pcg_conv2d_dgrad: empty problem");
   hipStream_t st = (hipStream_t)stream;
+  if (const uint32_t* tab = clip_mode() != 0 ? cliptab_of(g) : nullptr) {
+    const int groups = p.epi.group_rows > 0 ? maxMp / p.epi.group_rows : 1;
+    SkPlan sk{};
+    const bool plain = nph == 4 && !(p.N > 64 && plan_sk(ceil_div(maxMp, 128) * ceil_div(p.N, 128) * nph, 4 * ceil_div(g->Cout, IG_BK), st, &sk));
+    const ClipPlan cp = clip_dgrad_plan(g, groups, dgrad_interleaved(p.w_bytes, ph, nph), plain);
+    if (cp.take) clip_apply(g, cp, groups, tab, &p);
+  }
   if (int e = p.N > 64 ? launch_dgrad<Cfg128x128>(p, ph, nph, maxMp, st)
                        : (nph > 1 && g_tune.dgrad_swz3 == 0) ? launch_dgrad<Cfg128x64P>(p, ph, nph, maxMp, st)
                                                              : launch_dgrad<Cfg128x64>(p, ph, nph, maxMp, st)) return e;
@@ -1590,6 +1829,35 @@
   return PCG_OK;
 }
 
+extern "C" int pcg_conv_pad_clip_query(const pcg_conv_geom* g, int32_t op, int32_t groups, int32_t assume_scratch, int32_t* taken,
+                                       int32_t* order, int32_t* tile_rows, double* predicted) {
+  if (int e = check_geom(g)) return e;
+  PCG_REQUIRE((op == 0 || op == 1) && groups >= 1, "pcg_conv_pad_clip_query: bad arguments");
+  const int have = assume_scratch && sk_mode() != 0 ? 1 : 0;
+  ClipPlan cp{false, 0, 0, 1.0};
+  if (mfma_layer(g) && op == 0) {
+    const int M = g->B * g->OH * g->OW, N = g->Cout, kt = g->KH * g->KW * ceil_div(g->Cin, IG_BK);
+    const FwdPlan f = plan_fwd(g, have);
+    const bool t64 = fwd_use_t64(M, N, f.splits);
+    SkPlan sk{};
+    const bool plain = f.splits == 1 && !(N > 64 && !t64 && have && plan_sk_shape(ceil_div(M, 128) * ceil_div(N, 128), kt, &sk));
+    cp = clip_fwd_plan(g, groups, t64, plain);
+  } else if (mfma_layer(g) && g->stride <= 2 && !dgrad_as_gemm(g, have)) {
+    DgradPhases ph{};
+    int maxMp = 0;
+    const int nph = build_phases(g, &ph, &maxMp);
+    SkPlan sk{};
+    const bool plain = nph == 4 && !(g->Cin > 64 && have && plan_sk_shape(ceil_div(maxMp, 128) * ceil_div(g->Cin, 128) * nph, 4 * ceil_div(g->Cout, IG_BK), &sk));
+    const uint32_t w_bytes = (uint32_t)((int64_t)g->Cout * g->KH * g->KW * g->Cin * 4);
+    cp = clip_dgrad_plan(g, groups, dgrad_interleaved(w_bytes, ph, nph), plain);
+  }
+  if (taken) *taken = cp.take && cliptab_of(g) ? 1 : 0;
+  if (order) *order = cp.order;
+  if (tile_rows) *tile_rows = cp.bm;
+  if (predicted) *predicted = cp.ratio;
+  return PCG_OK;
+}
+
 extern "C" int pcg_tune_set(const char* name, int32_t value) {
   PCG_REQUIRE(name != nullptr, "pcg_tune_set: null name");
   if (!strcmp(name, "korder")) g_tune.korder = value;
@@ -1604,9 +1872,10 @@
   else if (!strcmp(name, "dgrad_gemm")) g_tune.dgrad_gemm = value;
   else if (!strcmp(name, "t64")) g_tune.t64 = value;
   else if (!strcmp(name, "wgrad_pixtab")) g_tune.wgrad_pixtab = value;
+  else if (!strcmp(name, "pad_clip")) g_tune.pad_clip = value;
   else {
     set_error("pcg_tune_set: unknown switch '%s' (korder, edge_prio, dgrad_swz3, wgrad_rounds, wgrad_order, dgrad_interleave, fwd_splits, "
-              "stream_k, sk_blocks, dgrad_gemm, t64); the loader switch wgrad_pixtab is accepted as well", name);
+              "stream_k, sk_blocks, dgrad_gemm, t64); the loader switches wgrad_pixtab and pad_clip are accepted as well", name);
     return PCG_ERR_INVALID;
   }
   return PCG_OK;
diff --git a/promptable-counterfactual-gan_amd/csrc/conv_loaders.h b/promptable-counterfactual-gan_amd/csrc/conv_loaders.h
--- a/promptable-counterfactual-gan_amd/csrc/conv_loaders.h
+++ b/promptable-counterfactual-gan_amd/csrc/conv_loaders.h
@@ -36,11 +36,33 @@
   FastDiv dOW, dOH;
   const uint32_t* pixtab;
   FastDiv dOHW;
-};
-
-struct FwdKIter {
+  const uint32_t* cliptab; int clip_order, clip_tpp, clip_tpg, clip_npos;
+};
+
+struct ClipTile { int img0, pos, h0, nh, w0, nw, stat_tile, group; };
+__device__ __forceinline__ ClipTile clip_tile(const ConvP& p, int section, uint32_t idx, int BM) {
+  const uint32_t rank = idx / (uint32_t)p.clip_tpp, j = idx - rank * (uint32_t)p.clip_tpp;
+  const uint32_t d = ((const __attribute__((address_space(4))) uint32_t*)p.cliptab)[section * p.clip_npos + (int)rank];
+  const uint32_t g = j / (uint32_t)p.clip_tpg, jj = j - g * (uint32_t)p.clip_tpg;
+  ClipTile t;
+  t.img0 = (int)j * BM; t.pos = (int)(d & 0xFFFFu);
+  t.h0 = (int)((d >> 16) & 15u); t.nh = (int)((d >> 20) & 15u); t.w0 = (int)((d >> 24) & 15u); t.nw = (int)(d >> 28);
+  t.stat_tile = (int)((g * (uint32_t)p.clip_npos + rank) * (uint32_t)p.clip_tpg + jj);
+  t.group = (int)g;
+  return t;
+}
+
+template <bool CLIP = false>
+struct FwdKIterT {
   int KH, KW, Cin, S, mode;
   int ch, cw, jh, jw, ci0;
+  int hlo, wlo;
+  __device__ __forceinline__ int jh0() const { return CLIP && hlo > ch ? (hlo - ch + S - 1) / S : 0; }
+  __device__ __forceinline__ int jw0() const { return CLIP && wlo > cw ? (wlo - cw + S - 1) / S : 0; }
+  __device__ __forceinline__ void clip(int h0, int nh, int w0, int nw) {
+    hlo = h0; wlo = w0; KH = h0 + nh; KW = w0 + nw;
+    jh = jh0(); jw = jw0();
+  }
   __device__ __forceinline__ void init(const ConvP& p) {
     KH = p.KH; KW = p.KW; Cin = p.Cin; mode = p.korder; S = mode ? p.stride : 1;
     ch = cw = jh = jw = ci0 = 0;
@@ -49,13 +71,14 @@
   __device__ __forceinline__ int kw() const { return cw + S * jw; }
   __device__ __forceinline__ bool next_tap_in_class() {
     if (cw + S * (++jw) < KW) return true;
-    jw = 0;
+    jw = jw0();
     if (ch + S * (++jh) < KH) return true;
-    jh = 0;
+    jh = jh0();
     return false;
   }
   __device__ __forceinline__ void next_class() {
     if (++cw >= S || cw >= KW) { cw = 0; ++ch; }
+    if constexpr (CLIP) { jh = jh0(); jw = jw0(); }
   }
   __device__ __forceinline__ void advance() {
     if (mode == 0) {
@@ -93,6 +116,7 @@
     }
   }
 };
+using FwdKIter = FwdKIterT<false>;
 
 struct PhaseInfo {
   int ph, pw;
@@ -125,16 +149,36 @@
   return ok ? t : make_float4(0.f, 0.f, 0.f, 0.f);
 }
 
-template <int ROWS_, bool XF = false>
+template <int ROWS_, bool XF = false, bool CLIP = false>
 struct FwdALoader {
   static constexpr bool KMAJOR = true, XFORM = XF;
   static constexpr int ROWS = ROWS_, NV = ROWS_ / 32;
   rsrc_t rs;
   uint32_t base[NV], mask[NV];
   int IW, Cin, KW, kq4;
-  FwdKIter it;
+  FwdKIterT<CLIP> it;
   XfK xf;
 
+  __device__ __forceinline__ FwdALoader(const ConvP& p, const ClipTile& t, int tid) {
+    if constexpr (XF) xf.init(p);
+    rs = make_rsrc(p.x, p.x_bytes);
+    IW = p.IW; Cin = p.Cin; KW = p.KW;
+    it.init(p);
+    it.clip(t.h0, t.nh, t.w0, t.nw);
+    kq4 = (tid & 7) * 4;
+    const int r0 = tid >> 3;
+    uint32_t oh, ow;
+    p.dOW.divmod((uint32_t)t.pos, oh, ow);
+    const int ih0 = (int)oh * p.stride - p.pad, iw0 = (int)ow * p.stride - p.pad;
+    const uint32_t mk = tap_mask(-ih0, p.IH - ih0, p.KH, -iw0, IW - iw0, KW);
+#pragma unroll
+    for (int i = 0; i < NV; ++i) {
+      const int b = t.img0 + r0 + 32 * i;
+      const bool in = b < p.B;
+      base[i] = in ? (uint32_t)((((b * p.IH + ih0) * IW + iw0) * Cin + kq4) * 4) : OOB_OFF;
+      mask[i] = in ? mk : 0u;
+    }
+  }
   __device__ __forceinline__ FwdALoader(const ConvP& p, int m_block, int tid) {
     if constexpr (XF) xf.init(p);
     rs = make_rsrc(p.x, p.x_bytes);
@@ -181,14 +225,14 @@
   }
 };
 
-template <int ROWS_>
+template <int ROWS_, bool CLIP = false>
 struct FwdBLoader {
   static constexpr bool KMAJOR = true, XFORM = false;
   static constexpr int ROWS = ROWS_, NV = ROWS_ / 32;
   rsrc_t rs;
   uint32_t base[NV];
   int Cin, KW, kq4;
-  FwdKIter it;
+  FwdKIterT<CLIP> it;
 
   __device__ __forceinline__ FwdBLoader(const ConvP& p, int n_block, int tid) {
     rs = make_rsrc(p.w, p.w_bytes);
@@ -214,12 +258,30 @@
   __device__ __forceinline__ void transform(float4 (&)[NV]) {}
 };
 
-struct DgradTapIter {
+template <bool CLIP = false>
+struct DgradTapIterT {
   int Cout, nth, ntw, jw, co0, jh, mode;
+  int hlo, hhi, wlo, whi;
   __device__ __forceinline__ void init(int Cout_, int nth_, int ntw_, int mode_) {
     Cout = Cout_; nth = nth_; ntw = ntw_; mode = mode_; jh = 0; jw = 0; co0 = 0;
   }
+  __device__ __forceinline__ void clip(int h0, int nh, int w0, int nw) {
+    hlo = h0; hhi = h0 + nh; wlo = w0; whi = w0 + nw; jh = hlo; jw = wlo;
+  }
   __device__ __forceinline__ void advance() {
+    if constexpr (CLIP) {
+      if (mode == 0) {
+        co0 += IG_BK;
+        if (co0 >= Cout) { co0 = 0; if (++jw == whi) { jw = wlo; ++jh; } }
+      } else {
+        if (++jw < whi) return;
+        jw = wlo;
+        if (++jh < hhi) return;
+        jh = hlo;
+        co0 += IG_BK;
+      }
+      return;
+    }
     if (mode == 0) {
       co0 += IG_BK;
       if (co0 >= Cout) { co0 = 0; if (++jw == ntw) { jw = 0; ++jh; } }
@@ -246,17 +308,38 @@
     jh = tap / ntw; jw = tap - jh * ntw;
   }
 };
-
-template <int ROWS_, bool XF = false>
+using DgradTapIter = DgradTapIterT<false>;
+
+template <int ROWS_, bool XF = false, bool CLIP = false>
 struct DgradALoader {
   static constexpr bool KMAJOR = true, XFORM = XF;
   static constexpr int ROWS = ROWS_, NV = ROWS_ / 32;
   rsrc_t rs;
   uint32_t base[NV], mask[NV];
   int OW, Cout, kq4;
-  DgradTapIter it;
+  DgradTapIterT<CLIP> it;
   XfK xf;
 
+  __device__ __forceinline__ DgradALoader(const ConvP& p, const PhaseInfo& f, const ClipTile& t, int tid) {
+    if constexpr (XF) xf.init(p);
+    rs = make_rsrc(p.dy, p.dy_bytes);
+    OW = p.OW; Cout = p.Cout;
+    kq4 = (tid & 7) * 4;
+    const int r0 = tid >> 3;
+    uint32_t aa, cc;
+    f.dPHw.divmod((uint32_t)t.pos, aa, cc);
+    const int oh0 = (int)aa + f.dh0, ow0 = (int)cc + f.dw0;
+    const uint32_t mk = tap_mask(oh0 - p.OH + 1, oh0 + 1, f.nth, ow0 - OW + 1, ow0 + 1, f.ntw);
+#pragma unroll
+    for (int i = 0; i < NV; ++i) {
+      const int b = t.img0 + r0 + 32 * i;
+      const bool in = b < p.B;
+      base[i] = in ? (uint32_t)((((b * p.OH + oh0) * OW + ow0) * Cout + kq4) * 4) : OOB_OFF;
+      mask[i] = in ? mk : 0u;
+    }
+    it.init(Cout, f.nth, f.ntw, p.korder);
+    it.clip(t.h0, t.nh, t.w0, t.nw);
+  }
   __device__ __forceinline__ DgradALoader(const ConvP& p, const PhaseInfo& f, int m_block, int tid) {
     if constexpr (XF) xf.init(p);
     rs = make_rsrc(p.dy, p.dy_bytes);
@@ -302,7 +385,7 @@
   }
 };
 
-template <int ROWS_>
+template <int ROWS_, bool CLIP = false>
 struct DgradBLoader {
   static constexpr bool KMAJOR = false, XFORM = false;
   static constexpr int ROWS = ROWS_, NV = ROWS_ / 32;
@@ -310,7 +393,7 @@
   rsrc_t rs;
   uint32_t base[NV];
   int Cin, KHKW, KW, stride, kh0, kw0, kr0;
-  DgradTapIter it;
+  DgradTapIterT<CLIP> it;
 
   __device__ __forceinline__ DgradBLoader(const ConvP& p, const PhaseInfo& f, int n_block, int tid) {
     rs = make_rsrc(p.w, p.w_bytes);
diff --git a/promptable-counterfactual-gan_amd/ops.py b/promptable-counterfactual-gan_amd/ops.py
--- a/promptable-counterfactual-gan_amd/ops.py
+++ b/promptable-counterfactual-gan_amd/ops.py
@@ -38,6 +38,7 @@
 class _Timed:
     def __init__(self, g, op):
         _conv_scratch()
+        _conv_cliptab(g)
         self.on = _conv_hook is not None
         if self.on:
             self.g, self.op = g, op
@@ -135,6 +136,33 @@
     with torch.cuda.device(device):
         check(_lib.load().pcg_conv_pixtab_register(ctypes.byref(g), None, 0, None), "pcg_conv_pixtab_register")
     _pixtabs[_pixtab_key(g, device.index)] = None
+
+
+_cliptabs = {}
+
+
+def _conv_cliptab(g):
+    if g.KH != 4 or g.stride != 2 or g.pad != 1:
+        return
+    key = (torch.cuda.current_device(), g.OH, g.OW)
+    if key in _cliptabs or torch.cuda.is_current_stream_capturing():
+        return
+    lib = _lib.load()
+    n = lib.pcg_conv_cliptab_bytes(ctypes.byref(g))
+    tab = None
+    if n:
+        host = torch.empty(n, dtype=torch.uint8)
+        check(lib.pcg_conv_cliptab_register(ctypes.byref(g), _p(host), n, None), "pcg_conv_cliptab_register")
+        tab = host.cuda()
+        check(lib.pcg_conv_cliptab_register(ctypes.byref(g), None, 0, _p(tab)), "pcg_conv_cliptab_register")
+    _cliptabs[key] = tab
+
+
+def conv_pad_clip_query(g, op, groups=1, assume_scratch=True):
+    taken, order, rows, pred = ctypes.c_int32(0), ctypes.c_int32(0), ctypes.c_int32(0), ctypes.c_double(1.0)
+    check(_lib.load().pcg_conv_pad_clip_query(ctypes.byref(g), int(op), int(groups), int(bool(assume_scratch)), ctypes.byref(taken),
+                                              ctypes.byref(order), ctypes.byref(rows), ctypes.byref(pred)), "pcg_conv_pad_clip_query")
+    return bool(taken.value), order.value, rows.value, pred.value
 
 
 def _p(t):
```
